# curioloop/rafting

Measured on AMD Instinct MI355X. Metric: raft-group decisions/sec (AppendEntries+vote), higher is better.
Workload: dtype int64

## Files before the change

### include/raftgpu.h

```cpp
#ifndef RAFTGPU_H
#define RAFTGPU_H

#include <stdint.h>
#include <stddef.h>

#ifdef __cplusplus
extern "C" {
#endif

#define RG_ABI_VERSION      6
#define RG_MIN_CLUSTER      2
#define RG_MAX_CLUSTER      15
#define RG_MAX_COMPACT_CLUSTER 7
#define RG_TERM_RUNS        4
#define RG_NO_NODE          (-1)

enum { RG_FOLLOWER = 0, RG_CANDIDATE = 1, RG_LEADER = 2 };

enum {
    RG_EV_NONE          = 0,
    RG_EV_AE_REQ        = 1,
    RG_EV_AE_ACK        = 2,
    RG_EV_IS_ACK        = 3,
    RG_EV_RV_REQ        = 4,
// ... 123 lines not shown
    uint32_t *elected_epoch;
    int64_t  *elected_term;
    int64_t  *commit_index;
    int64_t  *epoch_index;
    int64_t  *epoch_term;
    int64_t  *first_index;
    int64_t  *last_index;
    uint32_t *run_count;
    uint32_t *run_offset;
    int64_t  *run_start;
    int64_t  *run_term;
    int64_t  *peer_last_epoch;
    int64_t  *peer_next_index;
    int64_t  *peer_match_index;
    int32_t  *peer_rejection;
    uint8_t  *peer_pending;
} rg_group_state_t;

typedef struct rg_table rg_table_t;

int         rg_abi_version(void);
int         rg_table_create(int device, uint32_t groups, uint32_t cluster, uint32_t self_slot,
                            int pre_vote, rg_table_t **out);
int         rg_table_destroy(rg_table_t *t);
const char *rg_last_error(const rg_table_t *t);
enum { RG_OPT_REQUIRE_FENCED_TIMEOUTS = 1,
       RG_OPT_AUTO_INDEX_BASE = 2,
       RG_OPT_COMPACT_ANY_CLUSTER = 3,
       RG_OPT_DEVICE_IN_FLIGHT = 4 };
int         rg_table_option(rg_table_t *t, int option, int value);
uint32_t    rg_table_groups(const rg_table_t *t);
uint32_t    rg_table_cluster(const rg_table_t *t);

int rg_load_state(rg_table_t *t, uint32_t first, uint32_t count, const rg_group_state_t *src);
int rg_read_state(rg_table_t *t, uint32_t first, uint32_t count, rg_group_state_t *dst);

int rg_submit(rg_table_t *t, const rg_batch_t *in, const rg_outcome_t *out, int memspace);
int rg_sync(rg_table_t *t);

#define RG_PIPELINE_DEPTH 2
int rg_submit_async(rg_table_t *t, const rg_batch_t *in, const rg_outcome_t *out);
int rg_submit_wait(rg_table_t *t);

typedef struct { int32_t a, b, c, d; } rg_ev_quad32_t;
typedef struct {
    uint32_t              rounds, count;
    const uint32_t       *gid;
    const rg_ev_head_t   *head;
    const rg_ev_quad32_t *abcd;
    const int32_t        *entry_terms;
    uint64_t              entry_count;
} rg_batch32_t;
typedef struct {
    rg_reply_t   *reply;
    rg_logfx_t   *logfx;
    rg_persist_t *persist;
    uint32_t     *counts;
    uint32_t      logfx_cap, persist_cap;
} rg_outcome_packed_t;
int rg_submit_async_packed(rg_table_t *t, const rg_batch32_t *in, const rg_outcome_packed_t *out);

typedef struct rg_tick rg_tick_t;
int rg_tick_create(rg_table_t *t, const rg_batch32_t *in, const rg_outcome_packed_t *out, rg_tick_t **tick);
int rg_tick_launch(rg_tick_t *tick);
int rg_tick_wait(rg_tick_t *tick);
int rg_tick_destroy(rg_tick_t *tick);

int rg_submit32(rg_table_t *t, const rg_batch32_t *in, const rg_outcome_t *out, int memspace);
int64_t rg_batch32_pack(const rg_batch_t *in, rg_ev_head_t *head, rg_ev_quad32_t *abcd, int32_t *entry_terms);

int rg_index_base_set(rg_table_t *t, uint32_t first, uint32_t count, const int64_t *base);
int rg_index_base_get(rg_table_t *t, uint32_t first, uint32_t count, int64_t *base);
int rg_index_base_advance(const rg_batch_t *in, int32_t window, uint32_t groups, int64_t *index_base);
int rg_index_base_advance32(const rg_batch32_t *in, int32_t window, uint32_t groups, int64_t *index_base);
int64_t rg_batch32_pack_rel(const rg_batch_t *in, const int64_t *index_base, rg_ev_head_t *head, rg_ev_quad32_t *abcd, int32_t *entry_terms);
typedef struct { int32_t resp_term; uint32_t flags; int32_t commit_index; int32_t log_from; } rg_out32_t;
typedef struct { int32_t term; int32_t voted_for; uint32_t role_epoch; int32_t role; } rg_persist32_t;
typedef struct {
    rg_out32_t     *row;
    rg_persist32_t *persist;
    rg_outcome_t    wide;
} rg_outcome32_t;
int rg_submit32c(rg_table_t *t, const rg_batch32_t *in, const rg_outcome32_t *out, int memspace);
int rg_submit32c_sparse(rg_table_t *t, const rg_batch32_t *in, const rg_outcome32_t *out, int memspace);
int rg_submit32c_sparse_rounds(rg_table_t *t, const rg_batch32_t *in, const rg_outcome32_t *out, int memspace);
int rg_outcome32_unpack(const rg_outcome32_t *in, uint32_t rounds, uint32_t count, uint32_t *role_epoch, const rg_outcome_t *out);
int rg_outcome32_unpack_rel(const rg_outcome32_t *in, uint32_t rounds, uint32_t count, uint32_t *role_epoch, const int64_t *index_base, const rg_outcome_t *out);
const char *rg_step_kernel(rg_table_t *t, uint32_t count);

enum {
    RG_SEND_NONE      = 0,
    RG_SEND_APPEND    = 1,
    RG_SEND_SNAPSHOT  = 2,
    RG_SEND_GATED     = 3,
    RG_SEND_NEED_HOST = 4
};
#define RG_REPLICATE_LIMIT 50
#define RG_IN_FLIGHT_LIMIT 20

typedef struct {
    int64_t  term;
    int64_t  leader_commit;
    int64_t  epoch_index;
    int64_t  epoch_term;
    uint32_t role_epoch;
    uint32_t is_leader;
    uint64_t reserved;
} rg_send_head_t;

#define RG_SENT_TRIGGERED  1u
#define RG_SENT_HEARTBEAT  2u

typedef struct {
    int64_t  prev_index;
    int64_t  prev_term;
    int64_t  last_index;
    uint32_t count;
    uint32_t kind;
} rg_send_t;

int rg_replicate(rg_table_t *t, uint32_t count, const uint32_t *gid, const uint8_t *heartbeat, const uint16_t *in_flight,
                 rg_send_head_t *head, rg_send_t *send, int memspace);

int rg_timers_configure(rg_table_t *t, int64_t election_ms, int64_t heartbeat_ms, uint64_t seed);
int rg_timers_update(rg_table_t *t, uint32_t rounds, uint32_t count, const uint32_t *gid, const rg_reply_t *reply,
                     const int64_t *now, int memspace);
int rg_timers_expired(rg_table_t *t, int64_t now, uint32_t *out_gid, uint32_t capacity, uint32_t *out_count, int memspace);
int rg_timers_expired_epochs(rg_table_t *t, int64_t now, uint32_t *out_gid, uint32_t *out_epoch, uint32_t capacity, uint32_t *out_count,
                             int memspace);
int rg_timers_update32(rg_table_t *t, uint32_t rounds, const rg_out32_t *row, const rg_persist32_t *persist32, const int64_t *now, int memspace);
int rg_timers_arm(rg_table_t *t, int64_t now);
int rg_timers_read(rg_table_t *t, uint32_t first, uint32_t count, int64_t *deadline);

int rg_health_update(rg_table_t *t, uint32_t rounds, uint32_t count, const uint32_t *gid, const rg_ev_head_t *head,
                     const rg_reply_t *reply, const int64_t *now, int memspace);
int rg_health_update32(rg_table_t *t, uint32_t rounds, const rg_ev_head_t *head, const rg_out32_t *row, const int64_t *now, int memspace);
#define RG_HEALTH_NO_REQUEST 4u
int rg_health_failure(rg_table_t *t, uint32_t n, const uint32_t *gid, const uint8_t *slot, const uint8_t *flags, int64_t now);
int rg_ready(rg_table_t *t, int64_t now, int32_t critical_point, int64_t cool_down_ms, uint8_t *ready, int memspace);
int rg_health_read(rg_table_t *t, uint32_t first, uint32_t count, int64_t *request_success, int64_t *request_failure,
                   int32_t *recent_failure);
int rg_in_flight_read(rg_table_t *t, uint32_t first, uint32_t count, uint16_t *in_flight);
int rg_in_flight_set(rg_table_t *t, uint32_t first, uint32_t count, const uint16_t *in_flight);

typedef struct {
    uint32_t              rounds;
    const rg_ev_head_t   *head;
    const rg_ev_quad32_t *abcd;
    const int32_t        *entry_terms;
    uint64_t              entry_capacity;
    const int64_t        *now;
    const uint8_t        *heartbeat;
    const uint16_t       *in_flight;
    int32_t               critical_point;
    int64_t               cool_down_ms;
    rg_out32_t           *row;
    rg_persist32_t       *persist32;
    uint32_t             *expired_gid;
    uint32_t             *expired_epoch;
    uint32_t             *expired_count;
    uint32_t              expired_capacity;
    rg_send_head_t       *send_head;
    rg_send_t            *send;
    uint8_t              *ready;
} rg_tick2_io_t;
typedef struct rg_tick2 rg_tick2_t;
// ... 65 lines not shown
```

### rafting_amd/csrc/raftgpu.cpp

```cpp
#include <hip/hip_runtime.h>

#include <algorithm>
#include <cstdarg>
#include <cstdint>
#include <cstdio>
#include <cstdlib>
#include <cstring>
#include <string>
#include <unordered_map>
#include <vector>

#include "rg_device.hpp"
#include "rg_assemble.hpp"

using rg::DevTable;
using rg::I64x2;

struct Staging {
    void *ptr = nullptr;
    size_t cap = 0;
};

struct PipeSlot {
    Staging gid, head, ab, cd, hint, terms, reply, logfx, persist;
    Staging abcd32, terms32, counts;
    hipEvent_t up = nullptr, done = nullptr, down = nullptr;
};

struct rg_table {
    int device = 0;
    uint32_t G = 0, P = 0, self = 0, F = 0;
    int pre_vote = 0;
    hipStream_t stream = nullptr;
    DevTable dt{};
    unsigned long long *counters = nullptr;
    unsigned long long *wide_bodies = nullptr;
    size_t counter_slots = 0;
    int fast_paths = 1;
    int force_wide = 0;
    int require_fence = 0;
    int has_bases = 0;
    int auto_window = 0;
    int compact_any_cluster = 0;
    Staging st_abcd32, st_terms32, st_out32, st_persist32;
    int lanes = -1;
    uint32_t simds = 1024;
    Staging st_gid, st_head, st_ab, st_cd, st_hint, st_terms, st_reply, st_logfx, st_persist, st_hb, st_fl, st_sh, st_ss;
    bool timing = false;
    std::vector<std::pair<hipEvent_t, hipEvent_t>> ev_pool;
    size_t ev_used = 0;
    uint64_t t_launches = 0;
    double t_total_ms = 0.0;
    hipEvent_t region0 = nullptr, region1 = nullptr;
    int64_t *timer_deadline = nullptr;
    uint32_t *timer_epoch = nullptr;
    unsigned long long *tick_masks = nullptr;
    uint32_t *tick_ticket = nullptr;
    uint64_t config_gen = 0;
    std::vector<struct rg_tick *> ticks;
    std::vector<struct rg_tick2 *> ticks2;
    std::vector<struct rg_assembler *> assemblers;
    uint32_t *timer_counts = nullptr;
    int64_t election_ms = 900, heartbeat_ms = 300;
    uint64_t timer_seed = 0;
    Staging st_tgid, st_hgid, st_hslot, st_hflag, st_ready;
    int64_t *health_ok = nullptr, *health_fail = nullptr;
    int32_t *health_recent = nullptr;
    uint16_t *in_flight = nullptr;
    Staging st_hdone;
    hipStream_t s_in = nullptr, s_out = nullptr;
    PipeSlot pipe[RG_PIPELINE_DEPTH];
    uint64_t pipe_head = 0, pipe_tail = 0;
    std::string err;
};

static thread_local std::string g_create_err;

static int fail(rg_table *t, int code, const char *fmt, ...)
{
    char buf[512];
    va_list ap;
    va_start(ap, fmt);
    vsnprintf(buf, sizeof buf, fmt, ap);
    va_end(ap);
    if (t) t->err = buf; else g_create_err = buf;
    return code;
}

#define HIP_TRY(t, expr)                                                                              \
    do {                                                                                              \
        hipError_t e_ = (expr);                                                                       \
        if (e_ != hipSuccess) return fail((t), -2, "%s failed: %s", #expr, hipGetErrorString(e_));    \
    } while (0)

static int wait_oldest(rg_table *t)
{
    if (t->pipe_tail == t->pipe_head) return 1;
    HIP_TRY(t, hipEventSynchronize(t->pipe[t->pipe_tail % RG_PIPELINE_DEPTH].down));
    t->pipe_tail += 1;
    return 0;
}

static int bind(rg_table *t, bool drain = true)
{
    HIP_TRY(t, hipSetDevice(t->device));
    while (drain && t->pipe_tail != t->pipe_head)
        if (int rc = wait_oldest(t); rc < 0) return rc;
    return 0;
}

static int reserve(rg_table *t, Staging &s, size_t bytes)
{
    if (bytes <= s.cap) return 0;
    if (s.ptr) HIP_TRY(t, hipFree(s.ptr));
    s.ptr = nullptr; s.cap = 0;
    size_t cap = bytes + bytes / 4 + 4096;
    HIP_TRY(t, hipMalloc(&s.ptr, cap));
    s.cap = cap;
    return 0;
}

static int drain_timing(rg_table *t)
{
    if (t->ev_used == 0) return 0;
    HIP_TRY(t, hipStreamSynchronize(t->stream));
    for (size_t i = 0; i < t->ev_used; i++) {
        float ms = 0.f;
        HIP_TRY(t, hipEventElapsedTime(&ms, t->ev_pool[i].first, t->ev_pool[i].second));
        t->t_total_ms += ms;
        t->t_launches += 1;
    }
    t->ev_used = 0;
    return 0;
}

extern "C" {

int rg_abi_version(void) { return RG_ABI_VERSION; }

const char *rg_last_error(const rg_table_t *t) { return t ? t->err.c_str() : g_create_err.c_str(); }
uint32_t rg_table_groups(const rg_table_t *t) { return t ? t->G : 0; }
uint32_t rg_table_cluster(const rg_table_t *t) { return t ? t->P : 0; }

int rg_table_option(rg_table_t *t, int option, int value)
{
    if (!t) return -1;
    switch (option) {
    case RG_OPT_REQUIRE_FENCED_TIMEOUTS:
        if (t->require_fence != (value != 0)) t->config_gen += 1;
        t->require_fence = value != 0;
        return 0;
    case RG_OPT_AUTO_INDEX_BASE:
        if (value < 0 || value >= (1 << 30)) return fail(t, -1, "rg_table_option: RG_OPT_AUTO_INDEX_BASE window %d outside [0, 2^30)", value);
        if (t->auto_window != value) t->config_gen += 1;
        if (value != 0 && !t->has_bases) t->has_bases = 1;
        t->auto_window = value;
        return 0;
    case RG_OPT_COMPACT_ANY_CLUSTER:
        if (value != 0 && value != 1) return fail(t, -1, "rg_table_option: RG_OPT_COMPACT_ANY_CLUSTER takes 0 or 1 (%d given)", value);
        if (t->compact_any_cluster != value) t->config_gen += 1;
        t->compact_any_cluster = value;
        return 0;
    case RG_OPT_DEVICE_IN_FLIGHT: {
        if (value != 0 && value != 1) return fail(t, -1, "rg_table_option: RG_OPT_DEVICE_IN_FLIGHT takes 0 or 1 (%d given)", value);
        if ((t->in_flight != nullptr) == (value == 1)) return 0;
        if (bind(t)) return -2;
        HIP_TRY(t, hipStreamSynchronize(t->stream));
        if (value == 1) {
            const size_t bytes = (size_t)t->G * t->F * sizeof(uint16_t);
            uint16_t *c = nullptr;
            HIP_TRY(t, hipMalloc((void **)&c, bytes));
            if (hipError_t e = hipMemsetAsync(c, 0, bytes, t->stream); e != hipSuccess || (e = hipStreamSynchronize(t->stream)) != hipSuccess) {
                (void)hipFree(c);
                return fail(t, -2, "rg_table_option: RG_OPT_DEVICE_IN_FLIGHT: %s", hipGetErrorString(e));
            }
            t->in_flight = c;
        } else {
            HIP_TRY(t, hipFree(t->in_flight));
            t->in_flight = nullptr;
        }
        t->config_gen += 1;
        return 0;
    }
    default: return fail(t, -1, "rg_table_option: unknown option %d", option);
    }
}

static void tick_release(struct rg_tick *k);
static void tick2_release(struct rg_tick2 *k);
static void assembler_release(struct rg_assembler *a);

int rg_table_destroy(rg_table_t *t)
{
    if (!t) return 0;
    (void)hipSetDevice(t->device);
    if (t->stream) (void)hipStreamSynchronize(t->stream);
    for (struct rg_tick *k : t->ticks) tick_release(k);
    for (struct rg_tick2 *k : t->ticks2) tick2_release(k);
    for (struct rg_assembler *a : t->assemblers) assembler_release(a);
    t->ticks.clear(); t->ticks2.clear(); t->assemblers.clear();
    void *cols[] = {t->dt.term_commit, t->dt.epoch, t->dt.window, t->dt.ident, t->dt.elect, t->dt.runs,
                    t->dt.peer_en, t->dt.peer_m, t->dt.ibase, t->wide_bodies, t->counters, t->st_gid.ptr, t->st_head.ptr, t->st_ab.ptr,
                    t->st_cd.ptr, t->st_hint.ptr, t->st_terms.ptr, t->st_reply.ptr, t->st_logfx.ptr,
                    t->st_persist.ptr, t->st_hb.ptr, t->st_fl.ptr, t->st_sh.ptr, t->st_ss.ptr, t->timer_deadline, t->timer_epoch, t->tick_masks, t->tick_ticket,
                    t->timer_counts, t->st_tgid.ptr, t->st_hgid.ptr, t->st_hslot.ptr, t->st_hflag.ptr, t->st_ready.ptr, t->health_ok,
                    t->health_fail, t->health_recent, t->in_flight, t->st_hdone.ptr, t->st_abcd32.ptr, t->st_terms32.ptr, t->st_out32.ptr, t->st_persist32.ptr};
    for (void *c : cols) if (c) (void)hipFree(c);
    for (PipeSlot &sl : t->pipe) {
        if (sl.down) (void)hipEventSynchronize(sl.down);
        for (Staging *st : {&sl.gid, &sl.head, &sl.ab, &sl.cd, &sl.hint, &sl.terms, &sl.reply, &sl.logfx, &sl.persist, &sl.abcd32, &sl.terms32, &sl.counts})
            if (st->ptr) (void)hipFree(st->ptr);
        for (hipEvent_t ev : {sl.up, sl.done, sl.down}) if (ev) (void)hipEventDestroy(ev);
    }
    if (t->s_in) (void)hipStreamDestroy(t->s_in);
    if (t->s_out) (void)hipStreamDestroy(t->s_out);
    for (auto &e : t->ev_pool) { (void)hipEventDestroy(e.first); (void)hipEventDestroy(e.second); }
    if (t->region0) { (void)hipEventDestroy(t->region0); (void)hipEventDestroy(t->region1); }
    if (t->stream) (void)hipStreamDestroy(t->stream);
    delete t;
    return 0;
}

int rg_table_create(int device, uint32_t groups, uint32_t cluster, uint32_t self_slot, int pre_vote, rg_table_t **out)
{
    if (!out) return fail(nullptr, -1, "rg_table_create: out is NULL");
    *out = nullptr;
    if (groups == 0) return fail(nullptr, -1, "rg_table_create: groups must be > 0");
    if (cluster < RG_MIN_CLUSTER || cluster > RG_MAX_CLUSTER)
        return fail(nullptr, -1, "rg_table_create: cluster size %u outside [%d, %d]", cluster, RG_MIN_CLUSTER, RG_MAX_CLUSTER);
    if (self_slot >= cluster) return fail(nullptr, -1, "rg_table_create: self_slot %u >= cluster %u", self_slot, cluster);
    int ndev = 0;
    hipError_t e = hipGetDeviceCount(&ndev);
    if (e != hipSuccess || ndev == 0)
        return fail(nullptr, -2, "rg_table_create: no HIP device (%s) — libraftgpu has no CPU path", hipGetErrorString(e));
    if (device < 0 || device >= ndev) return fail(nullptr, -1, "rg_table_create: device %d of %d", device, ndev);

    rg_table *t = new rg_table();
    t->device = device; t->G = groups; t->P = cluster; t->self = self_slot; t->F = cluster - 1;
    t->pre_vote = pre_vote != 0;
#define CREATE_TRY(expr)                                                                   \
    do {                                                                                   \
        hipError_t e2_ = (expr);                                                           \
        if (e2_ != hipSuccess) {                                                           \
            fail(nullptr, -2, "%s failed: %s", #expr, hipGetErrorString(e2_));             \
            rg_table_destroy(t);                                                           \
            return -2;                                                                     \
        }                                                                                  \
    } while (0)
    CREATE_TRY(hipSetDevice(device));
    CREATE_TRY(hipStreamCreateWithFlags(&t->stream, hipStreamNonBlocking));
    const size_t G = groups, F = t->F;
    CREATE_TRY(hipMalloc((void **)&t->dt.term_commit, G * sizeof(I64x2)));
    CREATE_TRY(hipMalloc((void **)&t->dt.epoch, G * sizeof(I64x2)));
    CREATE_TRY(hipMalloc((void **)&t->dt.window, G * sizeof(I64x2)));
    CREATE_TRY(hipMalloc((void **)&t->dt.ident, G * sizeof(rg::Ident)));
    CREATE_TRY(hipMalloc((void **)&t->dt.elect, G * sizeof(rg::Elect)));
    CREATE_TRY(hipMalloc((void **)&t->dt.runs, G * rg::K * sizeof(I64x2)));
    CREATE_TRY(hipMalloc((void **)&t->dt.peer_en, G * F * sizeof(I64x2)));
    CREATE_TRY(hipMalloc((void **)&t->dt.peer_m, G * F * sizeof(rg::Match)));
    CREATE_TRY(hipMalloc((void **)&t->dt.ibase, G * sizeof(int64_t)));
    CREATE_TRY(hipMalloc((void **)&t->wide_bodies, sizeof(unsigned long long)));
    CREATE_TRY(hipMemsetAsync(t->wide_bodies, 0, sizeof(unsigned long long), t->stream));
    {
        hipDeviceProp_t prop;
        CREATE_TRY(hipGetDeviceProperties(&prop, device));
        t->simds = (uint32_t)prop.multiProcessorCount * 4u;
    }
    t->lanes = -1;
    if (const char *e = getenv("RG_SPLIT")) t->lanes = atoi(e) != 0 ? 0 : 64;
    if (const char *e = getenv("RG_FAST")) t->fast_paths = atoi(e) != 0;
    if (const char *e = getenv("RG_FORCE_WIDE")) t->force_wide = atoi(e) != 0;
    t->counter_slots = (G + 63) / 64 + 1;
    CREATE_TRY(hipMalloc((void **)&t->counters, t->counter_slots * RG_NUM_COUNTERS * sizeof(unsigned long long)));
    t->dt.groups = groups;
    CREATE_TRY(hipMalloc((void **)&t->timer_deadline, G * sizeof(int64_t)));
    CREATE_TRY(hipMalloc((void **)&t->timer_counts, ((G + 255) / 256 * 4 + 1) * sizeof(uint32_t)));
    CREATE_TRY(hipMemsetAsync(t->timer_deadline, 0, G * sizeof(int64_t), t->stream));
    CREATE_TRY(hipMalloc((void **)&t->tick_masks, ((G + 255) / 256 * 4) * sizeof(unsigned long long)));
    CREATE_TRY(hipMemsetAsync(t->tick_masks, 0, ((G + 255) / 256 * 4) * sizeof(unsigned long long), t->stream));
    CREATE_TRY(hipMalloc((void **)&t->tick_ticket, sizeof(uint32_t)));
    CREATE_TRY(hipMemsetAsync(t->tick_ticket, 0, sizeof(uint32_t), t->stream));
    CREATE_TRY(hipMalloc((void **)&t->timer_epoch, G * sizeof(uint32_t)));
    CREATE_TRY(hipMemsetAsync(t->timer_epoch, 0, G * sizeof(uint32_t), t->stream));
    CREATE_TRY(hipMalloc((void **)&t->health_ok, G * F * sizeof(int64_t)));
    CREATE_TRY(hipMalloc((void **)&t->health_fail, G * F * sizeof(int64_t)));
    CREATE_TRY(hipMalloc((void **)&t->health_recent, G * F * sizeof(int32_t)));
    CREATE_TRY(hipMemsetAsync(t->health_ok, 0, G * F * sizeof(int64_t), t->stream));
    CREATE_TRY(hipMemsetAsync(t->health_fail, 0, G * F * sizeof(int64_t), t->stream));
    CREATE_TRY(hipMemsetAsync(t->health_recent, 0, G * F * sizeof(int32_t), t->stream));
    CREATE_TRY(hipMemsetAsync(t->dt.term_commit, 0, G * sizeof(I64x2), t->stream));
    CREATE_TRY(hipMemsetAsync(t->dt.epoch, 0, G * sizeof(I64x2), t->stream));
    CREATE_TRY(hipMemsetAsync(t->dt.window, 0, G * sizeof(I64x2), t->stream));
    CREATE_TRY(hipMemsetAsync(t->dt.runs, 0, G * rg::K * sizeof(I64x2), t->stream));
    CREATE_TRY(hipMemsetAsync(t->dt.peer_en, 0, G * F * sizeof(I64x2), t->stream));
    CREATE_TRY(hipMemsetAsync(t->dt.peer_m, 0, G * F * sizeof(rg::Match), t->stream));
    CREATE_TRY(hipMemsetAsync(t->dt.ibase, 0, G * sizeof(int64_t), t->stream));
    CREATE_TRY(hipMemsetAsync(t->counters, 0, t->counter_slots * RG_NUM_COUNTERS * sizeof(unsigned long long), t->stream));
    {
        std::vector<rg::Ident> id(G, rg::Ident{RG_NO_NODE, RG_NO_NODE, 1u, 0u});
        std::vector<rg::Elect> el(G, rg::Elect{0, 0u, 1});
        CREATE_TRY(hipMemcpyAsync(t->dt.ident, id.data(), G * sizeof(rg::Ident), hipMemcpyHostToDevice, t->stream));
        CREATE_TRY(hipMemcpyAsync(t->dt.elect, el.data(), G * sizeof(rg::Elect), hipMemcpyHostToDevice, t->stream));
        CREATE_TRY(hipStreamSynchronize(t->stream));
    }
#undef CREATE_TRY
    *out = t;
    return 0;
}


static int step_lanes(const rg_table *t, uint32_t count)
{
    if (t->lanes >= 0) return t->lanes;
    const uint32_t wavefronts = (count + 63u) / 64u;
    return wavefronts <= t->simds ? 0 : 64;
}

static bool state_complete(const rg_group_state_t *s)
{
    return s->current_term && s->voted_for && s->role && s->current_leader && s->timeout_detected && s->repl_prepared &&
           s->role_epoch && s->votes && s->elected_epoch && s->elected_term && s->commit_index && s->epoch_index &&
           s->epoch_term && s->first_index && s->last_index && s->run_count && s->run_offset && s->run_start && s->run_term &&
           s->peer_last_epoch && s->peer_next_index && s->peer_match_index && s->peer_rejection && s->peer_pending;
}

int rg_load_state(rg_table_t *t, uint32_t first, uint32_t count, const rg_group_state_t *s)
{
    if (!t) return -1;
    if (!s || !state_complete(s)) return fail(t, -1, "rg_load_state: src or one of its columns is NULL");
    if ((uint64_t)first + count > t->G) return fail(t, -1, "rg_load_state: range [%u, %u) exceeds %u groups", first, first + count, t->G);
    if (count == 0) return 0;
    if (bind(t)) return -2;
    const size_t n = count, F = t->F, G = t->G;
    std::vector<I64x2> tc(n), ep(n), win(n), runs(n * rg::K), en(n * F);
    std::vector<rg::Ident> id(n);
    std::vector<rg::Elect> el(n);
    std::vector<rg::Match> pm(n * F);
    for (size_t i = 0; i < n; i++) {
        const int32_t role = s->role[i];
        if (role < RG_FOLLOWER || role > RG_LEADER) return fail(t, -1, "rg_load_state: group %zu role %d", first + i, role);
        if (s->voted_for[i] < RG_NO_NODE || s->voted_for[i] >= (int32_t)t->P || s->current_leader[i] < RG_NO_NODE ||
            s->current_leader[i] >= (int32_t)t->P)
            return fail(t, -1, "rg_load_state: group %zu node slot out of range", first + i);
        const uint32_t total = s->run_count[i], off = s->run_offset[i];
        const uint32_t rc = total > (uint32_t)rg::K ? (uint32_t)rg::K : total;
        int64_t fi = 0, la = 0;
        if (total) {
            fi = s->first_index[i]; la = s->last_index[i];
            if (s->run_start[off] != fi || la < s->run_start[off + total - 1])
                return fail(t, -1, "rg_load_state: group %zu runs do not span [first,last]", first + i);
            if (fi != s->epoch_index[i] && fi != s->epoch_index[i] + 1)
                return fail(t, -1, "rg_load_state: group %zu first index %lld is neither epoch.index nor epoch.index+1",
                            first + i, (long long)fi);
            for (uint32_t k = 1; k < total; k++)
// ... 247 lines not shown
    rg_batch_t wide{};
    wide.rounds = in->rounds; wide.count = in->count; wide.gid = in->gid; wide.head = in->head;
    wide.ab = wide.cd = reinterpret_cast<const rg_ev_pair_t *>(in->abcd);
    wide.entry_terms = reinterpret_cast<const int64_t *>(in->entry_terms); wide.entry_count = in->entry_count;
    rg_logfx_t dummy_l; rg_persist_t dummy_p;
    const rg_outcome_t shape{out->reply, &dummy_l, &dummy_p};
    if (int rc = check_batch(t, &wide, &shape, true)) return rc;
    if (in->count == 0) { out->counts[0] = out->counts[1] = 0; return 0; }
    const size_t rows64 = (size_t)in->rounds * in->count;
    if (rows64 >= (1ull << 31)) return fail(t, -1, "rg_submit_async_packed: %zu rows in one batch (limit 2^31 - 1)", rows64);
    if (bind(t, false)) return -2;
    void *d_logfx = nullptr, *d_persist = nullptr, *d_counts = nullptr;
    if (hipHostGetDevicePointer(&d_counts, out->counts, 0) != hipSuccess ||
        (out->logfx_cap && hipHostGetDevicePointer(&d_logfx, out->logfx, 0) != hipSuccess) ||
        (out->persist_cap && hipHostGetDevicePointer(&d_persist, out->persist, 0) != hipSuccess)) {
        (void)hipGetLastError();
        return fail(t, -1, "rg_submit_async_packed: counts / logfx / persist must be page-locked memory from rg_host_alloc");
    }
    if (int rc = pipeline_ready(t)) return rc;
    PipeSlot &sl = t->pipe[t->pipe_head % RG_PIPELINE_DEPTH];
    const bool sparse = in->gid != nullptr;
    const uint32_t rows = (uint32_t)rows64, waves = (rows + 63u) / 64u;
    rg::StepParams p = step_params(t, &wide);
    if (reserve(t, sl.head, rows64 * sizeof(rg_ev_head_t)) || reserve(t, sl.abcd32, rows64 * sizeof(rg_ev_quad32_t)) ||
        reserve(t, sl.reply, rows64 * sizeof(rg_reply_t)) || reserve(t, sl.logfx, rows64 * sizeof(I64x2)) ||
        reserve(t, sl.persist, rows64 * sizeof(rg_persist_t)) || reserve(t, sl.counts, (size_t)2 * waves * sizeof(uint32_t)))
        return -2;
    hipStream_t si = t->s_in, so = t->s_out;
    HIP_TRY(t, hipMemcpyAsync(sl.head.ptr, in->head, rows64 * sizeof(rg_ev_head_t), hipMemcpyHostToDevice, si));
    HIP_TRY(t, hipMemcpyAsync(sl.abcd32.ptr, in->abcd, rows64 * sizeof(rg_ev_quad32_t), hipMemcpyHostToDevice, si));
    if (sparse) {
        if (reserve(t, sl.gid, in->count * sizeof(uint32_t))) return -2;
        HIP_TRY(t, hipMemcpyAsync(sl.gid.ptr, in->gid, in->count * sizeof(uint32_t), hipMemcpyHostToDevice, si));
        p.gid = (const uint32_t *)sl.gid.ptr;
    }
    if (in->entry_count) {
        if (reserve(t, sl.terms32, in->entry_count * sizeof(int32_t))) return -2;
        HIP_TRY(t, hipMemcpyAsync(sl.terms32.ptr, in->entry_terms, in->entry_count * sizeof(int32_t), hipMemcpyHostToDevice, si));
    }
    HIP_TRY(t, hipEventRecord(sl.up, si));
    HIP_TRY(t, hipStreamWaitEvent(t->stream, sl.up, 0));
    p.head = (const rg_ev_head_t *)sl.head.ptr; p.abcd32 = (const rg::I32x4 *)sl.abcd32.ptr;
    p.hint = nullptr;
    p.entry_terms32 = in->entry_count ? (const int32_t *)sl.terms32.ptr : nullptr;
    p.reply = (rg_reply_t *)sl.reply.ptr; p.logfx = (I64x2 *)sl.logfx.ptr; p.persist = (rg_persist_t *)sl.persist.ptr;
    if (int rc = launch(t, p, sparse)) return rc;
    HIP_TRY(t, rg::launch_outcome_count(p.reply, rows, (uint32_t *)sl.counts.ptr, (uint32_t *)d_counts, t->stream));
    HIP_TRY(t, hipEventRecord(sl.done, t->stream));
    HIP_TRY(t, hipStreamWaitEvent(so, sl.done, 0));
    HIP_TRY(t, rg::launch_outcome_emit(p.reply, p.logfx, p.persist, rows, (const uint32_t *)sl.counts.ptr, (I64x2 *)d_logfx, out->logfx_cap,
                                       (rg_persist_t *)d_persist, out->persist_cap, so));
    HIP_TRY(t, hipMemcpyAsync(out->reply, sl.reply.ptr, rows64 * sizeof(rg_reply_t), hipMemcpyDeviceToHost, so));
    HIP_TRY(t, hipEventRecord(sl.down, so));
    t->pipe_head += 1;
    return 0;
}

struct rg_tick {
    rg_table *t = nullptr;
    hipGraph_t graph = nullptr;
    hipGraphExec_t exec = nullptr;
    Staging head, abcd, gid, terms, reply, logfx, persist, counts;
    uint64_t config_gen = 0;
    bool in_flight = false;
};

static void tick_release(struct rg_tick *k)
{
    if (k->exec) (void)hipGraphExecDestroy(k->exec);
    if (k->graph) (void)hipGraphDestroy(k->graph);
    k->exec = nullptr; k->graph = nullptr;
    for (Staging *st : {&k->head, &k->abcd, &k->gid, &k->terms, &k->reply, &k->logfx, &k->persist, &k->counts}) {
        if (st->ptr) (void)hipFree(st->ptr);
        st->ptr = nullptr; st->cap = 0;
    }
    k->t = nullptr;
}

int rg_tick_destroy(rg_tick_t *k)
{
    if (!k) return 0;
    if (rg_table *t = k->t) {
        (void)hipSetDevice(t->device);
        if (t->stream) (void)hipStreamSynchronize(t->stream);
        t->ticks.erase(std::remove(t->ticks.begin(), t->ticks.end(), k), t->ticks.end());
        tick_release(k);
    }
    delete k;
    return 0;
}

static bool page_locked(const void *p)
{
    void *d = nullptr;
    if (hipHostGetDevicePointer(&d, const_cast<void *>(p), 0) == hipSuccess) return true;
    (void)hipGetLastError();
    return false;
}

int rg_tick_create(rg_table_t *t, const rg_batch32_t *in, const rg_outcome_packed_t *out, rg_tick_t **tick)
{
    if (!t) return -1;
    if (int rc = compact_ok(t, "rg_tick_create")) return rc;
    if (!tick) return fail(t, -1, "rg_tick_create: tick is NULL");
    *tick = nullptr;
    if (!in || !out) return fail(t, -1, "rg_tick_create: null batch or outcome");
    if (!in->head || !in->abcd || !out->reply || !out->counts || (out->logfx_cap && !out->logfx) || (out->persist_cap && !out->persist))
        return fail(t, -1, "rg_tick_create: head, abcd, reply, counts and every list with a capacity are required");
    if (in->entry_count && !in->entry_terms) return fail(t, -1, "rg_tick_create: entry_count %llu without entry_terms", (unsigned long long)in->entry_count);
    rg_batch_t wide{};
    wide.rounds = in->rounds; wide.count = in->count; wide.gid = nullptr; wide.head = in->head;
    wide.ab = wide.cd = reinterpret_cast<const rg_ev_pair_t *>(in->abcd);
    wide.entry_terms = reinterpret_cast<const int64_t *>(in->entry_terms); wide.entry_count = in->entry_count;
    rg_logfx_t dummy_l; rg_persist_t dummy_p;
    const rg_outcome_t shape{out->reply, &dummy_l, &dummy_p};
    if (in->gid) {
        if (in->rounds != 1) return fail(t, -1, "rg_tick_create: sparse batches carry exactly one round");
        if (in->count > t->G || in->count == 0) return fail(t, -1, "rg_tick_create: %u rows for %u groups", in->count, t->G);
    } else if (int rc = check_batch(t, &wide, &shape, true)) return rc;
    if (in->rounds == 0 || in->count == 0) return fail(t, -1, "rg_tick_create: an empty shape");
    const size_t rows64 = (size_t)in->rounds * in->count;
    if (rows64 >= (1ull << 31)) return fail(t, -1, "rg_tick_create: %zu rows in one batch (limit 2^31 - 1)", rows64);
    if (bind(t)) return -2;
    void *d_logfx = nullptr, *d_persist = nullptr, *d_counts = nullptr;
    if (hipHostGetDevicePointer(&d_counts, out->counts, 0) != hipSuccess ||
        (out->logfx_cap && hipHostGetDevicePointer(&d_logfx, out->logfx, 0) != hipSuccess) ||
        (out->persist_cap && hipHostGetDevicePointer(&d_persist, out->persist, 0) != hipSuccess)) {
        (void)hipGetLastError();
        return fail(t, -1, "rg_tick_create: counts / logfx / persist must be page-locked memory from rg_host_alloc");
    }
    if (!page_locked(in->head) || !page_locked(in->abcd) || !page_locked(out->reply) || (in->gid && !page_locked(in->gid)) ||
        (in->entry_count && !page_locked(in->entry_terms)))
        return fail(t, -1, "rg_tick_create: head / abcd / gid / entry_terms / reply must be page-locked memory from rg_host_alloc (the recorded copies replay from them)");
    rg_tick *k = new rg_tick();
    k->t = t;
    k->config_gen = t->config_gen;
    const uint32_t rows = (uint32_t)rows64, waves = (rows + 63u) / 64u;
    const bool sparse = in->gid != nullptr;
    if (reserve(t, k->head, rows64 * sizeof(rg_ev_head_t)) || reserve(t, k->abcd, rows64 * sizeof(rg_ev_quad32_t)) || reserve(t, k->reply, rows64 * sizeof(rg_reply_t)) ||
        reserve(t, k->logfx, rows64 * sizeof(I64x2)) || reserve(t, k->persist, rows64 * sizeof(rg_persist_t)) || reserve(t, k->counts, (size_t)2 * waves * sizeof(uint32_t)) ||
        (sparse && reserve(t, k->gid, in->count * sizeof(uint32_t))) || (in->entry_count && reserve(t, k->terms, in->entry_count * sizeof(int32_t)))) {
        rg_tick_destroy(k);
        return -2;
    }
    rg::StepParams p = step_params(t, &wide);
    p.head = (const rg_ev_head_t *)k->head.ptr; p.abcd32 = (const rg::I32x4 *)k->abcd.ptr;
    p.gid = sparse ? (const uint32_t *)k->gid.ptr : nullptr;
    p.entry_terms32 = in->entry_count ? (const int32_t *)k->terms.ptr : nullptr;
    p.reply = (rg_reply_t *)k->reply.ptr; p.logfx = (I64x2 *)k->logfx.ptr; p.persist = (rg_persist_t *)k->persist.ptr;
    hipStream_t s = t->stream;
    hipError_t e = hipStreamBeginCapture(s, hipStreamCaptureModeThreadLocal);
    if (e == hipSuccess) e = hipMemcpyAsync(k->head.ptr, in->head, rows64 * sizeof(rg_ev_head_t), hipMemcpyHostToDevice, s);
    if (e == hipSuccess) e = hipMemcpyAsync(k->abcd.ptr, in->abcd, rows64 * sizeof(rg_ev_quad32_t), hipMemcpyHostToDevice, s);
    if (e == hipSuccess && sparse) e = hipMemcpyAsync(k->gid.ptr, in->gid, in->count * sizeof(uint32_t), hipMemcpyHostToDevice, s);
    if (e == hipSuccess && in->entry_count) e = hipMemcpyAsync(k->terms.ptr, in->entry_terms, in->entry_count * sizeof(int32_t), hipMemcpyHostToDevice, s);
    if (e == hipSuccess) e = rg::launch_step(p, (int)t->F, sparse, 32, s);
    if (e == hipSuccess) e = rg::launch_outcome_count(p.reply, rows, (uint32_t *)k->counts.ptr, (uint32_t *)d_counts, s);
    if (e == hipSuccess) e = rg::launch_outcome_emit(p.reply, p.logfx, p.persist, rows, (const uint32_t *)k->counts.ptr, (I64x2 *)d_logfx, out->logfx_cap,
                                                     (rg_persist_t *)d_persist, out->persist_cap, s);
    if (e == hipSuccess) e = hipMemcpyAsync(out->reply, k->reply.ptr, rows64 * sizeof(rg_reply_t), hipMemcpyDeviceToHost, s);
    hipGraph_t g = nullptr;
    const hipError_t e2 = hipStreamEndCapture(s, &g);
    k->graph = g;
    if (e == hipSuccess) e = e2;
    if (e == hipSuccess) e = hipGraphInstantiate(&k->exec, k->graph, nullptr, nullptr, 0);
    if (e != hipSuccess) {
        (void)hipGetLastError();
        rg_tick_destroy(k);
        return fail(t, -2, "rg_tick_create: %s", hipGetErrorString(e));
    }
    t->ticks.push_back(k);
    *tick = k;
    return 0;
}

int rg_tick_launch(rg_tick_t *k)
{
    if (!k || !k->t) return -1;
    rg_table *t = k->t;
    if (k->config_gen != t->config_gen)
        return fail(t, -1, "rg_tick_launch: the table's options or index bases changed after rg_tick_create (they are part of the recording): create the tick again");
    if (bind(t)) return -2;
    if (k->in_flight) { HIP_TRY(t, hipStreamSynchronize(t->stream)); k->in_flight = false; }
    HIP_TRY(t, hipGraphLaunch(k->exec, t->stream));
    k->in_flight = true;
    return 0;
}

int rg_tick_wait(rg_tick_t *k)
{
    if (!k || !k->t) return -1;
    rg_table *t = k->t;
    HIP_TRY(t, hipSetDevice(t->device));
    HIP_TRY(t, hipStreamSynchronize(t->stream));
    k->in_flight = false;
    return 0;
}

static rg::TimerParams timer_params(rg_table *t);
static rg::HealthParams health_params(rg_table *t);

struct rg_tick2 {
    rg_table *t = nullptr;
    hipGraph_t graph = nullptr;
    hipGraphExec_t exec = nullptr;
    uint64_t config_gen = 0;
    bool in_flight = false;
};

static void tick2_release(struct rg_tick2 *k)
{
    if (k->exec) (void)hipGraphExecDestroy(k->exec);
    if (k->graph) (void)hipGraphDestroy(k->graph);
    k->exec = nullptr; k->graph = nullptr;
    k->t = nullptr;
}

int rg_tick2_destroy(rg_tick2_t *k)
{
    if (!k) return 0;
    if (rg_table *t = k->t) {
        (void)hipSetDevice(t->device);
        if (t->stream) (void)hipStreamSynchronize(t->stream);
        t->ticks2.erase(std::remove(t->ticks2.begin(), t->ticks2.end(), k), t->ticks2.end());
        tick2_release(k);
    }
    delete k;
    return 0;
}

static int device_visible(rg_table *t, const char *who, const void *p, const char *what, void **out)
{
    *out = nullptr;
    if (!p) return 0;
    hipPointerAttribute_t a{};
    if (hipPointerGetAttributes(&a, p) != hipSuccess || a.type == hipMemoryTypeUnregistered) {
        (void)hipGetLastError();
        return fail(t, -1, "%s: %s is neither device memory (rg_dev_alloc) nor page-locked host memory (rg_host_alloc)", who, what);
    }
    if (a.type == hipMemoryTypeHost) {
        if (hipHostGetDevicePointer(out, const_cast<void *>(p), 0) != hipSuccess) {
            (void)hipGetLastError();
            return fail(t, -1, "%s: %s is host memory the device cannot address", who, what);
        }
        return 0;
    }
    *out = const_cast<void *>(p);
    return 0;
}

static int tick2_create(rg_table_t *t, const rg_tick2_io_t *io, const rg_tick2_rows_t *rows, rg_tick2_t **tick, const char *who, bool deep = false,
                        const uint32_t *depth_now = nullptr)
{
    if (!t) return -1;
    if (int rc = compact_ok(t, who)) return rc;
    if (!tick) return fail(t, -1, "%s: tick is NULL", who);
    *tick = nullptr;
    if (!io) return fail(t, -1, "%s: io is NULL", who);
    if (io->rounds == 0 || io->rounds > 64) return fail(t, -1, "%s: %u rounds (1 .. 64: one clock per round travels with the tick)", who, io->rounds);
    if (!io->head || !io->abcd || !io->now || !io->row || !io->persist32) return fail(t, -1, "%s: head, abcd, now, row and persist32 are required", who);
    if (io->entry_capacity && !io->entry_terms) return fail(t, -1, "%s: entry_capacity %llu without entry_terms", who, (unsigned long long)io->entry_capacity);
    if (io->expired_gid && (!io->expired_count || io->expired_capacity == 0)) return fail(t, -1, "%s: the expiry step needs expired_count and a capacity", who);
    if ((io->send_head == nullptr) != (io->send == nullptr)) return fail(t, -1, "%s: send_head and send come together", who);
    if (t->in_flight && (io->heartbeat || io->in_flight))
        return fail(t, -1, "%s: the table has RG_OPT_DEVICE_IN_FLIGHT: the send step derives heartbeat and in_flight from the tick's own rows, both columns must be NULL", who);
    if (rows) {
        if (io->rounds != 1 && !deep) return fail(t, -1, "%s: %u rounds (a list of groups carries exactly one round)", who, io->rounds);
        if (!rows->gid || !rows->count) return fail(t, -1, "%s: gid and count are required", who);
        if (rows->capacity == 0 || rows->capacity > t->G) return fail(t, -1, "%s: a capacity of %u rows for %u groups (1 .. groups)", who, rows->capacity, t->G);
    }
    const uint32_t R = rows ? rows->capacity : t->G;
    rg_batch_t wide{};
    wide.rounds = io->rounds; wide.count = R; wide.gid = rows ? rows->gid : nullptr; wide.head = io->head;
    wide.ab = wide.cd = reinterpret_cast<const rg_ev_pair_t *>(io->abcd);
    wide.entry_terms = reinterpret_cast<const int64_t *>(io->entry_terms); wide.entry_count = io->entry_capacity;
    rg_reply_t dummy_r; rg_logfx_t dummy_l; rg_persist_t dummy_p;
    const rg_outcome_t shape{&dummy_r, &dummy_l, &dummy_p};
    if (int rc = check_batch(t, &wide, &shape, false, deep)) return rc;
    if (bind(t)) return -2;
    const auto visible = [t](const void *p, const char *what, void **out) { return device_visible(t, "rg_tick2_create", p, what, out); };
    void *d_head, *d_abcd, *d_terms, *d_now, *d_hb, *d_fl, *d_row, *d_per, *d_egid, *d_eep, *d_ecnt, *d_sh, *d_ss, *d_ready, *d_gid = nullptr, *d_cnt = nullptr, *d_depth = nullptr;
    if ((rows && (visible(rows->gid, "gid", &d_gid) || visible(rows->count, "count", &d_cnt) || visible(depth_now, "rounds", &d_depth))) ||
        visible(io->head, "head", &d_head) || visible(io->abcd, "abcd", &d_abcd) || visible(io->entry_terms, "entry_terms", &d_terms) ||
        visible(io->now, "now", &d_now) || visible(io->heartbeat, "heartbeat", &d_hb) || visible(io->in_flight, "in_flight", &d_fl) ||
        visible(io->row, "row", &d_row) || visible(io->persist32, "persist32", &d_per) || visible(io->expired_gid, "expired_gid", &d_egid) ||
        visible(io->expired_epoch, "expired_epoch", &d_eep) || visible(io->expired_count, "expired_count", &d_ecnt) ||
        visible(io->send_head, "send_head", &d_sh) || visible(io->send, "send", &d_ss) || visible(io->ready, "ready", &d_ready))
        return -1;
    rg_tick2 *k = new rg_tick2();
    k->t = t;
    k->config_gen = t->config_gen;
    rg::StepParams sp = step_params(t, &wide);
    sp.gid = (const uint32_t *)d_gid;
    sp.head = (const rg_ev_head_t *)d_head; sp.abcd32 = (const rg::I32x4 *)d_abcd;
    sp.entry_terms32 = io->entry_capacity ? (const int32_t *)d_terms : nullptr;
    sp.out32 = (rg::I32x4 *)d_row; sp.persist32 = (rg::I32x4 *)d_per;
    rg::TimerParams tp = timer_params(t);
    tp.rounds = io->rounds; tp.count = R; tp.out32 = (const rg::I32x4 *)d_row; tp.persist32 = (const rg::I32x4 *)d_per; tp.now_mem = (const int64_t *)d_now;
    rg::HealthParams hp = health_params(t);
    hp.rounds = io->rounds; hp.count = R; hp.head = (const rg_ev_head_t *)d_head; hp.out32 = (const rg::I32x4 *)d_row; hp.now_mem = (const int64_t *)d_now;
    const int64_t *now_last = (const int64_t *)d_now + (io->rounds - 1);
    rg::HealthParams rp = health_params(t);
    rp.now_mem = now_last;
    rg::ReplicateParams qp{};
    qp.t = t->dt; qp.count = R; qp.gid = (const uint32_t *)d_gid; qp.heartbeat = (const uint8_t *)d_hb; qp.in_flight = (const uint16_t *)d_fl; qp.head = (rg_send_head_t *)d_sh; qp.send = (rg_send_t *)d_ss;
    if (t->in_flight) {
        qp.counts = t->in_flight; qp.ev_head = (const rg_ev_head_t *)d_head; qp.ev_out32 = (const rg::I32x4 *)d_row; qp.ev_stride = R; qp.self = t->self;
    }
    hipStream_t s = t->stream;
    rg::TickFoldParams fp{};
    fp.tp = tp; fp.hp = hp; fp.now_last = now_last;
    fp.masks = (unsigned long long *)t->tick_masks; fp.ticket = t->tick_ticket;
    fp.out_gid = (uint32_t *)d_egid; fp.out_epoch = (uint32_t *)d_eep; fp.out_count = (uint32_t *)d_ecnt; fp.capacity = io->expired_capacity;
    fp.expire = io->expired_gid != nullptr;
    fp.rounds_now = (const uint32_t *)d_depth;
    rg::TickTailParams tt{};
    tt.fp = fp; tt.qp = qp; tt.rp = rp; tt.critical_point = io->critical_point; tt.cool_down = io->cool_down_ms; tt.ready = (uint8_t *)d_ready;
    const char *nodes_env = getenv("RG_TICK_NODES");
    int nodes = (nodes_env && (nodes_env[0] == '2' || nodes_env[0] == '4')) ? nodes_env[0] - '0' : (sp.force_wide != 0 ? 2 : 1);
    if (nodes == 4 && t->in_flight) nodes = 2;
    hipError_t e = hipStreamBeginCapture(s, hipStreamCaptureModeThreadLocal);
    if (rows) {
        if (e == hipSuccess) e = rg::launch_tick_sparse(sp, tt, (const uint32_t *)d_cnt, (int)t->F, s);
        if (e == hipSuccess && fp.expire) e = rg::launch_tick_expire(fp, s);
    } else if (nodes == 1) {
        if (e == hipSuccess) e = rg::launch_tick(sp, tt, (int)t->F, s);
    } else {
        if (e == hipSuccess) e = rg::launch_step(sp, (int)t->F, false, 32, s);
        if (nodes == 2) {
            if (e == hipSuccess) e = rg::launch_tick_tail(tt, (int)t->F, s);
        } else {
            if (e == hipSuccess) e = rg::launch_tick_fold(fp, s);
            if (e == hipSuccess && io->send_head) e = rg::launch_replicate(qp, (int)t->F, s);
            if (e == hipSuccess && io->ready) e = rg::launch_ready(rp, 0, io->critical_point, io->cool_down_ms, (uint8_t *)d_ready, s);
        }
    }
    hipGraph_t g = nullptr;
    const hipError_t e2 = hipStreamEndCapture(s, &g);
    k->graph = g;
    if (e == hipSuccess) e = e2;
    if (e == hipSuccess) e = hipGraphInstantiate(&k->exec, k->graph, nullptr, nullptr, 0);
    if (e != hipSuccess) {
        (void)hipGetLastError();
        rg_tick2_destroy(k);
        return fail(t, -2, "%s: %s", who, hipGetErrorString(e));
    }
    t->ticks2.push_back(k);
    *tick = k;
    return 0;
}

int rg_tick2_create(rg_table_t *t, const rg_tick2_io_t *io, rg_tick2_t **tick)
{
    return tick2_create(t, io, nullptr, tick, "rg_tick2_create");
}

int rg_tick2_create_sparse(rg_table_t *t, const rg_tick2_io_t *io, const rg_tick2_rows_t *rows, rg_tick2_t **tick)
{
    if (t && !rows) return fail(t, -1, "rg_tick2_create_sparse: rows is NULL");
    return tick2_create(t, io, rows, tick, "rg_tick2_create_sparse");
}

int rg_tick2_create_sparse_rounds(rg_table_t *t, const rg_tick2_io_t *io, const rg_tick2_rounds_t *rows, rg_tick2_t **tick)
{
    if (t && !rows) return fail(t, -1, "rg_tick2_create_sparse_rounds: rows is NULL");
    if (!t) return -1;
    const rg_tick2_rows_t list{rows->gid, rows->count, rows->capacity};
    return tick2_create(t, io, &list, tick, "rg_tick2_create_sparse_rounds", true, rows->rounds);
}

int rg_tick2_launch(rg_tick2_t *k)
{
    if (!k || !k->t) return -1;
    rg_table *t = k->t;
    if (k->config_gen != t->config_gen)
        return fail(t, -1, "rg_tick2_launch: the table's options or index bases changed after rg_tick2_create (they are part of the recording): create the tick again");
    if (bind(t)) return -2;
    HIP_TRY(t, hipGraphLaunch(k->exec, t->stream));
    k->in_flight = true;
    return 0;
}

int rg_tick2_wait(rg_tick2_t *k)
{
    if (!k || !k->t) return -1;
    rg_table *t = k->t;
    HIP_TRY(t, hipSetDevice(t->device));
    HIP_TRY(t, hipStreamSynchronize(t->stream));
    k->in_flight = false;
    return 0;
}

struct rg_assembler {
    rg_table *t = nullptr;
    uint32_t max_events = 0, max_expired = 0;
    rg::AsmParams sc{};
    Staging in_words, in_gid, in_head, in_abcd, ex_gid, ex_epoch;
    Staging out_gid, out_words, out_head, out_abcd, out_origin, out_deferred;
};

static void assembler_release(struct rg_assembler *a)
{
    void *cols[] = {a->sc.cnt, a->sc.bitmap, a->sc.rowof, a->sc.wordoff, a->sc.rowcnt, a->sc.segoff, a->sc.seg, a->sc.flag, a->sc.dcounts, a->sc.big, a->sc.scalars,
                    a->in_words.ptr, a->in_gid.ptr, a->in_head.ptr, a->in_abcd.ptr, a->ex_gid.ptr, a->ex_epoch.ptr,
                    a->out_gid.ptr, a->out_words.ptr, a->out_head.ptr, a->out_abcd.ptr, a->out_origin.ptr, a->out_deferred.ptr};
    for (void *c : cols) if (c) (void)hipFree(c);
    *a = rg_assembler{};
}

int rg_assembler_destroy(rg_assembler_t *a)
{
    if (!a) return 0;
    if (rg_table *t = a->t) {
        (void)hipSetDevice(t->device);
        if (t->stream) (void)hipStreamSynchronize(t->stream);
        t->assemblers.erase(std::remove(t->assemblers.begin(), t->assemblers.end(), a), t->assemblers.end());
        assembler_release(a);
    }
    delete a;
    return 0;
}

int rg_assembler_create(rg_table_t *t, uint32_t max_events, uint32_t max_expired, rg_assembler_t **out)
{
    if (!t) return -1;
    if (!out) return fail(t, -1, "rg_assembler_create: a is NULL");
    *out = nullptr;
    if ((uint64_t)max_events + max_expired >= (1ull << 31))
        return fail(t, -1, "rg_assembler_create: %u + %u events: a run holds fewer than 2^31 (the ids of the expired source carry bit 31)", max_events, max_expired);
    if (bind(t)) return -2;
    rg_assembler *a = new rg_assembler();
    a->t = t; a->max_events = max_events; a->max_expired = max_expired;
    rg::AsmParams &p = a->sc;
    const size_t G = t->G, words = (G + 63) / 64, events = (size_t)max_events + max_expired, eb = events ? (events + 255) / 256 : 1;
    p.groups = t->G; p.words = (uint32_t)words;
    p.seg_cap = (uint32_t)events;
    p.rows_cap = (uint32_t)(G < events ? G : events);
    p.big_cap = (uint32_t)(events / (rg::ASM_SMALL + 1) + 1);
    struct { void **ptr; size_t bytes; bool zero; } cols[] = {
        {(void **)&p.cnt, G * sizeof(uint32_t), true}, {(void **)&p.bitmap, words * sizeof(unsigned long long), true}, {(void **)&p.rowof, G * sizeof(uint32_t), true},
        {(void **)&p.wordoff, (words + 1) * sizeof(uint32_t), false}, {(void **)&p.rowcnt, ((size_t)p.rows_cap + 1) * sizeof(uint32_t), false},
        {(void **)&p.segoff, ((size_t)p.rows_cap + 1) * sizeof(uint32_t), false}, {(void **)&p.seg, (events + 1) * sizeof(uint32_t), false},
        {(void **)&p.flag, events + 1, false}, {(void **)&p.dcounts, (eb * 4 + 1) * sizeof(uint32_t), false}, {(void **)&p.big, (size_t)p.big_cap * sizeof(uint32_t), false},
        {(void **)&p.scalars, rg::ASM_SCALARS * sizeof(uint32_t), true}};
    for (auto &c : cols) {
        hipError_t e = hipMalloc(c.ptr, c.bytes);
        if (e == hipSuccess && c.zero) e = hipMemsetAsync(*c.ptr, 0, c.bytes, t->stream);
        if (e != hipSuccess) {
            assembler_release(a);
            delete a;
            return fail(t, -2, "rg_assembler_create: %zu bytes of scratch: %s", c.bytes, hipGetErrorString(e));
        }
    }
    if (hipStreamSynchronize(t->stream) != hipSuccess) { assembler_release(a); delete a; return fail(t, -2, "rg_assembler_create: hipStreamSynchronize failed"); }
    t->assemblers.push_back(a);
    *out = a;
    return 0;
}

int rg_assemble32(rg_assembler_t *a, const rg_arrivals_t *in, const rg_assembled_t *out, int memspace)
{
    if (!a || !a->t) return -1;
    rg_table *t = a->t;
    const char *who = "rg_assemble32";
    if (!in || !out) return fail(t, -1, "%s: NULL arrivals or batch", who);
    if (!in->count || (in->capacity && (!in->gid || !in->head || !in->abcd))) return fail(t, -1, "%s: count, gid, head and abcd of the arrival log are required", who);
    if (!out->gid || !out->count || !out->rounds || !out->head || !out->abcd || !out->origin || !out->stats || (out->deferred_capacity && !out->deferred))
        return fail(t, -1, "%s: gid, count, rounds, head, abcd, origin and stats of the batch are required (and deferred, unless deferred_capacity is 0)", who);
    if (out->capacity == 0 || out->capacity > t->G) return fail(t, -1, "%s: capacity %u outside 1 .. %u groups", who, out->capacity, t->G);
    if (out->max_rounds < 1 || out->max_rounds > 64) return fail(t, -1, "%s: max_rounds %u outside 1 .. 64", who, out->max_rounds);
    if (in->capacity > a->max_events) return fail(t, -1, "%s: an arrival log of %u events, the assembler was created for %u", who, in->capacity, a->max_events);
    const int sources = (in->expired_gid != nullptr) + (in->expired_epoch != nullptr) + (in->expired_count != nullptr);
    if (sources != 0 && sources != 3) return fail(t, -1, "%s: the expired source comes as all three columns or none", who);
    const bool expired = sources == 3;
    if (expired && in->expired_capacity > a->max_expired)
        return fail(t, -1, "%s: an expired source of %u entries, the assembler was created for %u", who, in->expired_capacity, a->max_expired);
    if (memspace != RG_MEM_DEVICE && memspace != RG_MEM_HOST) return fail(t, -1, "%s: unknown memspace %d", who, memspace);
    const uint32_t C = out->capacity, D = out->max_rounds, ex_cap = expired ? in->expired_capacity : 0u;
    const size_t cells = (size_t)C * D;
    rg::AsmParams p = a->sc;
    p.in_cap = in->capacity; p.ex_cap = ex_cap; p.C = C; p.D = D; p.deferred_cap = out->deferred_capacity;
    if (memspace == RG_MEM_DEVICE) {
        void *v[16] = {};
        const struct { const void *ptr; const char *what; } cols[] = {
            {in->count, "count"}, {in->gid, "gid"}, {in->head, "head"}, {in->abcd, "abcd"}, {in->expired_gid, "expired_gid"}, {in->expired_epoch, "expired_epoch"},
            {in->expired_count, "expired_count"}, {out->gid, "the batch's gid"}, {out->count, "the batch's count"}, {out->rounds, "rounds"}, {out->head, "the batch's head"},
            {out->abcd, "the batch's abcd"}, {out->origin, "origin"}, {out->deferred, "deferred"}, {out->stats, "stats"}};
        int k = 0;
        for (const auto &c : cols) if (int rc = device_visible(t, "rg_assemble32", c.ptr, c.what, &v[k++])) return rc;
        p.in_count = (const uint32_t *)v[0]; p.in_gid = (const uint32_t *)v[1]; p.in_head = (const rg::U32x2 *)v[2]; p.in_abcd = (const rg::I32x4 *)v[3];
        p.ex_gid = (const uint32_t *)v[4]; p.ex_epoch = (const uint32_t *)v[5]; p.ex_count = (const uint32_t *)v[6];
        p.gid = (uint32_t *)v[7]; p.count = (uint32_t *)v[8]; p.rounds = (uint32_t *)v[9]; p.head = (rg::U32x2 *)v[10]; p.abcd = (rg::I32x4 *)v[11];
        p.origin = (uint32_t *)v[12]; p.deferred = (uint32_t *)v[13]; p.stats = (uint32_t *)v[14];
        if (bind(t)) return -2;
        HIP_TRY(t, rg::launch_assemble(p, t->stream));
        return 0;
    }
// ... 100 lines not shown
    }
    p.reply = (rg_reply_t *)t->st_reply.ptr; p.logfx = (I64x2 *)t->st_logfx.ptr; p.persist = (rg_persist_t *)t->st_persist.ptr;
    HIP_TRY(t, hipMemsetAsync(t->st_logfx.ptr, 0, rows * sizeof(I64x2), s));
    HIP_TRY(t, hipMemsetAsync(t->st_persist.ptr, 0, rows * sizeof(rg_persist_t), s));
    if (int rc = launch(t, p, sparse)) return rc;
    HIP_TRY(t, hipMemcpyAsync(out->reply, t->st_reply.ptr, rows * sizeof(rg_reply_t), hipMemcpyDeviceToHost, s));
    HIP_TRY(t, hipMemcpyAsync(out->logfx, t->st_logfx.ptr, rows * sizeof(I64x2), hipMemcpyDeviceToHost, s));
    HIP_TRY(t, hipMemcpyAsync(out->persist, t->st_persist.ptr, rows * sizeof(rg_persist_t), hipMemcpyDeviceToHost, s));
    HIP_TRY(t, hipStreamSynchronize(s));
    return 0;
}

int rg_submit32(rg_table_t *t, const rg_batch32_t *in, const rg_outcome_t *out, int memspace)
{
    if (!t) return -1;
    if (int rc = compact_ok(t, "rg_submit32")) return rc;
    if (!in || !out) return fail(t, -1, "rg_submit32: NULL batch or outcome");
    if (!in->head || !in->abcd) return fail(t, -1, "rg_submit32: head and abcd are required");
    rg_batch_t wide{};
    wide.rounds = in->rounds; wide.count = in->count; wide.gid = in->gid; wide.head = in->head;
    wide.ab = wide.cd = reinterpret_cast<const rg_ev_pair_t *>(in->abcd);
    wide.entry_terms = reinterpret_cast<const int64_t *>(in->entry_terms); wide.entry_count = in->entry_count;
    if (int rc = check_batch(t, &wide, out, memspace == RG_MEM_HOST)) return rc;
    if (in->count == 0) return 0;
    if (bind(t)) return -2;
    const bool sparse = in->gid != nullptr;
    const size_t rows = (size_t)in->rounds * in->count;
    rg::StepParams p = step_params(t, &wide);
    if (memspace == RG_MEM_DEVICE) {
        p.gid = in->gid; p.head = in->head; p.abcd32 = (const rg::I32x4 *)in->abcd;
        p.entry_terms32 = in->entry_count ? in->entry_terms : nullptr;
        p.reply = out->reply; p.logfx = (I64x2 *)out->logfx; p.persist = out->persist;
        return launch(t, p, sparse);
    }
    if (memspace != RG_MEM_HOST) return fail(t, -1, "rg_submit32: unknown memspace %d", memspace);
    hipStream_t s = t->stream;
    if (reserve(t, t->st_head, rows * sizeof(rg_ev_head_t)) || reserve(t, t->st_abcd32, rows * sizeof(rg_ev_quad32_t)) ||
        reserve(t, t->st_reply, rows * sizeof(rg_reply_t)) || reserve(t, t->st_logfx, rows * sizeof(I64x2)) ||
        reserve(t, t->st_persist, rows * sizeof(rg_persist_t)))
        return -2;
    HIP_TRY(t, hipMemcpyAsync(t->st_head.ptr, in->head, rows * sizeof(rg_ev_head_t), hipMemcpyHostToDevice, s));
    HIP_TRY(t, hipMemcpyAsync(t->st_abcd32.ptr, in->abcd, rows * sizeof(rg_ev_quad32_t), hipMemcpyHostToDevice, s));
    p.head = (const rg_ev_head_t *)t->st_head.ptr; p.abcd32 = (const rg::I32x4 *)t->st_abcd32.ptr;
    if (sparse) {
        if (reserve(t, t->st_gid, in->count * sizeof(uint32_t))) return -2;
        HIP_TRY(t, hipMemcpyAsync(t->st_gid.ptr, in->gid, in->count * sizeof(uint32_t), hipMemcpyHostToDevice, s));
        p.gid = (const uint32_t *)t->st_gid.ptr;
    }
    if (in->entry_count) {
        if (reserve(t, t->st_terms32, in->entry_count * sizeof(int32_t))) return -2;
        HIP_TRY(t, hipMemcpyAsync(t->st_terms32.ptr, in->entry_terms, in->entry_count * sizeof(int32_t), hipMemcpyHostToDevice, s));
        p.entry_terms32 = (const int32_t *)t->st_terms32.ptr;
    }
    p.reply = (rg_reply_t *)t->st_reply.ptr; p.logfx = (I64x2 *)t->st_logfx.ptr; p.persist = (rg_persist_t *)t->st_persist.ptr;
    HIP_TRY(t, hipMemsetAsync(t->st_logfx.ptr, 0, rows * sizeof(I64x2), s));
    HIP_TRY(t, hipMemsetAsync(t->st_persist.ptr, 0, rows * sizeof(rg_persist_t), s));
    if (int rc = launch(t, p, sparse)) return rc;
    HIP_TRY(t, hipMemcpyAsync(out->reply, t->st_reply.ptr, rows * sizeof(rg_reply_t), hipMemcpyDeviceToHost, s));
    HIP_TRY(t, hipMemcpyAsync(out->logfx, t->st_logfx.ptr, rows * sizeof(I64x2), hipMemcpyDeviceToHost, s));
    HIP_TRY(t, hipMemcpyAsync(out->persist, t->st_persist.ptr, rows * sizeof(rg_persist_t), hipMemcpyDeviceToHost, s));
    HIP_TRY(t, hipStreamSynchronize(s));
    return 0;
}

int rg_wide_body_workgroups(rg_table_t *t, uint64_t *count, int reset)
{
    if (!t || !count) return -1;
    if (bind(t)) return -2;
    unsigned long long v = 0;
    HIP_TRY(t, hipMemcpyAsync(&v, t->wide_bodies, sizeof v, hipMemcpyDeviceToHost, t->stream));
    if (reset) HIP_TRY(t, hipMemsetAsync(t->wide_bodies, 0, sizeof v, t->stream));
    HIP_TRY(t, hipStreamSynchronize(t->stream));
    *count = v;
    return 0;
}

int rg_index_base_set(rg_table_t *t, uint32_t first, uint32_t count, const int64_t *base)
{
    if (!t) return -1;
    if (!base) return fail(t, -1, "rg_index_base_set: NULL base");
    if ((uint64_t)first + count > t->G) return fail(t, -1, "rg_index_base_set: groups [%u, %u) of %u", first, first + count, t->G);
    for (uint32_t i = 0; i < count; i++)
        if (base[i] < 0) return fail(t, -1, "rg_index_base_set: base[%u] = %lld is negative", i, (long long)base[i]);
    for (uint32_t i = 0; i < count; i++)
        if (base[i] != 0 && !t->has_bases) { t->has_bases = 1; t->config_gen += 1; }
    if (count == 0) return 0;
    if (bind(t)) return -2;
    HIP_TRY(t, hipMemcpyAsync(t->dt.ibase + first, base, (size_t)count * sizeof(int64_t), hipMemcpyHostToDevice, t->stream));
    HIP_TRY(t, hipStreamSynchronize(t->stream));
    return 0;
}

int rg_index_base_get(rg_table_t *t, uint32_t first, uint32_t count, int64_t *base)
{
    if (!t) return -1;
    if (!base) return fail(t, -1, "rg_index_base_get: NULL base");
    if ((uint64_t)first + count > t->G) return fail(t, -1, "rg_index_base_get: groups [%u, %u) of %u", first, first + count, t->G);
    if (count == 0) return 0;
    if (bind(t)) return -2;
    HIP_TRY(t, hipMemcpyAsync(base, t->dt.ibase + first, (size_t)count * sizeof(int64_t), hipMemcpyDeviceToHost, t->stream));
    HIP_TRY(t, hipStreamSynchronize(t->stream));
    return 0;
}

extern "C++" template <class Flush>
int advance_bases(uint32_t rounds, uint32_t count, const uint32_t *gid, const rg_ev_head_t *head, int32_t window, uint32_t groups, int64_t *index_base,
                         Flush flush)
{
    if (!head || !index_base || window < 1 || window >= (1 << 30)) return -1;
    if (gid ? count > groups : count != groups) return -2;
    if (gid)
        for (uint32_t i = 0; i < count; i++)
            if (gid[i] >= groups) return -2;
    std::vector<int64_t> top(gid ? count : groups, 0);
    for (uint32_t r = 0; r < rounds; r++)
        for (uint32_t i = 0; i < count; i++) {
            const size_t row = (size_t)r * count + i;
            if (RG_HDR_KIND(head[row].hdr) != RG_EV_LOG_FLUSH) continue;
            const int64_t a = flush(row, gid ? gid[i] : i);
            if (a > top[i]) top[i] = a;
        }
    for (uint32_t i = 0; i < (uint32_t)top.size(); i++) {
        int64_t &base = index_base[gid ? gid[i] : i];
        if (top[i] - window > base) base = top[i] - window;
    }
    return 0;
}

int rg_index_base_advance(const rg_batch_t *in, int32_t window, uint32_t groups, int64_t *index_base)
{
    if (!in || !in->ab) return -1;
    return advance_bases(in->rounds, in->count, in->gid, in->head, window, groups, index_base, [&](size_t row, uint32_t) { return (int64_t)in->ab[row].x; });
}

int rg_index_base_advance32(const rg_batch32_t *in, int32_t window, uint32_t groups, int64_t *index_base)
{
    if (!in || !in->abcd) return -1;
    return advance_bases(in->rounds, in->count, in->gid, in->head, window, groups, index_base, [&](size_t row, uint32_t g) {
        const int32_t a = in->abcd[row].a;
        return a <= 0 ? (int64_t)0 : (int64_t)a + index_base[g];
    });
}

static uint32_t host_index_fields(uint32_t kind)
{
    switch (kind) {
    case RG_EV_AE_REQ: return 0xAu;
    case RG_EV_AE_ACK: return 0x6u;
    case RG_EV_IS_ACK: case RG_EV_RV_REQ: case RG_EV_PV_REQ: case RG_EV_IS_REQ: return 0x2u;
    case RG_EV_LOG_FLUSH: return 0x1u;
    default: return 0u;
    }
}

static int submit32c(rg_table_t *t, const rg_batch32_t *in, const rg_outcome32_t *out, int memspace, bool sparse, const char *who, bool list_rounds = false)
{
    if (!t) return -1;
    if (int rc = compact_ok(t, who)) return rc;
    if (!in || !out) return fail(t, -1, "%s: NULL batch or outcome", who);
    if (!in->head || !in->abcd || !out->row || !out->persist) return fail(t, -1, "%s: head, abcd, row and persist are required", who);
    if (!sparse && in->gid) return fail(t, -1, "rg_submit32c: dense batches only (gid must be NULL); a list of groups goes through rg_submit32c_sparse");
    if (sparse && !in->gid) return fail(t, -1, "%s: gid is required (dense batches go through rg_submit32c)", who);
    const int wides = (out->wide.reply != nullptr) + (out->wide.logfx != nullptr) + (out->wide.persist != nullptr);
    if (wides != 0 && wides != 3) return fail(t, -1, "%s: the overflow columns come as all three or none", who);
    rg_batch_t wide{};
    wide.rounds = in->rounds; wide.count = in->count; wide.gid = in->gid; wide.head = in->head;
    wide.ab = wide.cd = reinterpret_cast<const rg_ev_pair_t *>(in->abcd);
    wide.entry_terms = reinterpret_cast<const int64_t *>(in->entry_terms); wide.entry_count = in->entry_count;
    rg_reply_t dummy_r; rg_logfx_t dummy_l; rg_persist_t dummy_p;
    const rg_outcome_t shape{&dummy_r, &dummy_l, &dummy_p};
    if (int rc = check_batch(t, &wide, &shape, memspace == RG_MEM_HOST, list_rounds)) return rc;
    if (in->count == 0) return 0;
    if (bind(t)) return -2;
    const size_t rows = (size_t)in->rounds * in->count;
    rg::StepParams p = step_params(t, &wide);
    if (memspace == RG_MEM_DEVICE) {
        p.gid = in->gid; p.head = in->head; p.abcd32 = (const rg::I32x4 *)in->abcd;
        p.entry_terms32 = in->entry_count ? in->entry_terms : nullptr;
        p.out32 = (rg::I32x4 *)out->row; p.persist32 = (rg::I32x4 *)out->persist;
        p.reply = out->wide.reply; p.logfx = (I64x2 *)out->wide.logfx; p.persist = out->wide.persist;
        return launch(t, p, sparse);
    }
    if (memspace != RG_MEM_HOST) return fail(t, -1, "%s: unknown memspace %d", who, memspace);
    hipStream_t s = t->stream;
    if (reserve(t, t->st_head, rows * sizeof(rg_ev_head_t)) || reserve(t, t->st_abcd32, rows * sizeof(rg_ev_quad32_t)) ||
        reserve(t, t->st_out32, rows * sizeof(rg_out32_t)) || reserve(t, t->st_persist32, rows * sizeof(rg_persist32_t)))
        return -2;
    if (wides && (reserve(t, t->st_reply, rows * sizeof(rg_reply_t)) || reserve(t, t->st_logfx, rows * sizeof(I64x2)) ||
                  reserve(t, t->st_persist, rows * sizeof(rg_persist_t))))
        return -2;
    HIP_TRY(t, hipMemcpyAsync(t->st_head.ptr, in->head, rows * sizeof(rg_ev_head_t), hipMemcpyHostToDevice, s));
    HIP_TRY(t, hipMemcpyAsync(t->st_abcd32.ptr, in->abcd, rows * sizeof(rg_ev_quad32_t), hipMemcpyHostToDevice, s));
    p.head = (const rg_ev_head_t *)t->st_head.ptr; p.abcd32 = (const rg::I32x4 *)t->st_abcd32.ptr;
    if (sparse) {
        if (reserve(t, t->st_gid, in->count * sizeof(uint32_t))) return -2;
        HIP_TRY(t, hipMemcpyAsync(t->st_gid.ptr, in->gid, in->count * sizeof(uint32_t), hipMemcpyHostToDevice, s));
        p.gid = (const uint32_t *)t->st_gid.ptr;
    }
    if (in->entry_count) {
        if (reserve(t, t->st_terms32, in->entry_count * sizeof(int32_t))) return -2;
        HIP_TRY(t, hipMemcpyAsync(t->st_terms32.ptr, in->entry_terms, in->entry_count * sizeof(int32_t), hipMemcpyHostToDevice, s));
        p.entry_terms32 = (const int32_t *)t->st_terms32.ptr;
    }
    p.out32 = (rg::I32x4 *)t->st_out32.ptr; p.persist32 = (rg::I32x4 *)t->st_persist32.ptr;
    HIP_TRY(t, hipMemsetAsync(t->st_persist32.ptr, 0, rows * sizeof(rg_persist32_t), s));
    if (wides) {
        p.reply = (rg_reply_t *)t->st_reply.ptr; p.logfx = (I64x2 *)t->st_logfx.ptr; p.persist = (rg_persist_t *)t->st_persist.ptr;
        HIP_TRY(t, hipMemsetAsync(t->st_reply.ptr, 0, rows * sizeof(rg_reply_t), s));
        HIP_TRY(t, hipMemsetAsync(t->st_logfx.ptr, 0, rows * sizeof(I64x2), s));
        HIP_TRY(t, hipMemsetAsync(t->st_persist.ptr, 0, rows * sizeof(rg_persist_t), s));
    }
    if (int rc = launch(t, p, sparse)) return rc;
    HIP_TRY(t, hipMemcpyAsync(out->row, t->st_out32.ptr, rows * sizeof(rg_out32_t), hipMemcpyDeviceToHost, s));
    HIP_TRY(t, hipMemcpyAsync(out->persist, t->st_persist32.ptr, rows * sizeof(rg_persist32_t), hipMemcpyDeviceToHost, s));
    if (wides) {
        HIP_TRY(t, hipMemcpyAsync(out->wide.reply, t->st_reply.ptr, rows * sizeof(rg_reply_t), hipMemcpyDeviceToHost, s));
        HIP_TRY(t, hipMemcpyAsync(out->wide.logfx, t->st_logfx.ptr, rows * sizeof(I64x2), hipMemcpyDeviceToHost, s));
        HIP_TRY(t, hipMemcpyAsync(out->wide.persist, t->st_persist.ptr, rows * sizeof(rg_persist_t), hipMemcpyDeviceToHost, s));
    }
    HIP_TRY(t, hipStreamSynchronize(s));
    return 0;
}

int rg_submit32c(rg_table_t *t, const rg_batch32_t *in, const rg_outcome32_t *out, int memspace)
{
    return submit32c(t, in, out, memspace, false, "rg_submit32c");
}

int rg_submit32c_sparse(rg_table_t *t, const rg_batch32_t *in, const rg_outcome32_t *out, int memspace)
{
    return submit32c(t, in, out, memspace, true, "rg_submit32c_sparse");
}

int rg_submit32c_sparse_rounds(rg_table_t *t, const rg_batch32_t *in, const rg_outcome32_t *out, int memspace)
{
    return submit32c(t, in, out, memspace, true, "rg_submit32c_sparse_rounds", true);
}

int rg_outcome32_unpack(const rg_outcome32_t *in, uint32_t rounds, uint32_t count, uint32_t *role_epoch, const rg_outcome_t *out)
{
    return rg_outcome32_unpack_rel(in, rounds, count, role_epoch, nullptr, out);
}

int rg_outcome32_unpack_rel(const rg_outcome32_t *in, uint32_t rounds, uint32_t count, uint32_t *role_epoch, const int64_t *index_base, const rg_outcome_t *out)
{
    if (!in || !in->row || !in->persist || !role_epoch || !out || !out->reply || !out->logfx || !out->persist) return -1;
    auto absolute = [&](int32_t v, uint32_t i) { return v == 0 ? (int64_t)0 : (int64_t)v + (index_base ? index_base[i] : 0); };
    for (uint32_t r = 0; r < rounds; r++) {
        for (uint32_t i = 0; i < count; i++) {
            const size_t row = (size_t)r * count + i;
            const rg_out32_t c = in->row[row];
            const uint32_t flags = c.flags & ~RG_F_WIDE_VALUES;
            const bool has_lfx = (flags & (RG_F_COMMIT | RG_F_LOG_APPEND | RG_F_LOG_TRUNC)) != 0 || RG_F_STATUS(flags) == RG_NEED_HOST;
            const bool has_from = (flags & (RG_F_LOG_APPEND | RG_F_LOG_TRUNC)) != 0 || RG_F_STATUS(flags) == RG_NEED_HOST;
            const bool has_per = (flags & RG_F_PERSIST) != 0;
// ... 417 lines not shown
    if (out)
        for (size_t i = 0; i < n; i++)
            for (size_t j = 0; j < F; j++) out[i * F + j] = col[j * n + i];
    return 0;
}

int rg_in_flight_read(rg_table_t *t, uint32_t first, uint32_t count, uint16_t *in_flight)
{
    return in_flight_copy(t, first, count, in_flight, nullptr, "rg_in_flight_read");
}

int rg_in_flight_set(rg_table_t *t, uint32_t first, uint32_t count, const uint16_t *in_flight)
{
    return in_flight_copy(t, first, count, nullptr, in_flight, "rg_in_flight_set");
}

const char *rg_step_kernel(rg_table_t *t, uint32_t count)
{
    if (!t) return "";
    return step_lanes(t, count) == 0 ? "rg::step_split_kernel" : "rg::step_kernel";
}

int rg_sync(rg_table_t *t)
{
    if (!t) return -1;
    if (bind(t)) return -2;
    HIP_TRY(t, hipStreamSynchronize(t->stream));
    return 0;
}


int rg_host_alloc(rg_table_t *t, size_t bytes, void **hptr)
{
    if (!t || !hptr) return -1;
    if (bind(t)) return -2;
    HIP_TRY(t, hipHostMalloc(hptr, bytes ? bytes : 16, hipHostMallocDefault));
    return 0;
}

int rg_host_free(rg_table_t *t, void *hptr)
{
    if (!t) return -1;
    if (bind(t)) return -2;
    HIP_TRY(t, hipStreamSynchronize(t->stream));
    HIP_TRY(t, hipHostFree(hptr));
    return 0;
}

int rg_dev_alloc(rg_table_t *t, size_t bytes, void **dptr)
{
    if (!t || !dptr) return -1;
    if (bind(t)) return -2;
    HIP_TRY(t, hipMalloc(dptr, bytes ? bytes : 16));
    return 0;
}

int rg_dev_free(rg_table_t *t, void *dptr)
{
    if (!t) return -1;
    if (bind(t)) return -2;
    HIP_TRY(t, hipStreamSynchronize(t->stream));
    HIP_TRY(t, hipFree(dptr));
    return 0;
}

int rg_copy_to_device(rg_table_t *t, void *dst, const void *src, size_t bytes)
{
    if (!t) return -1;
    if (bind(t)) return -2;
    HIP_TRY(t, hipMemcpyAsync(dst, src, bytes, hipMemcpyHostToDevice, t->stream));
    HIP_TRY(t, hipStreamSynchronize(t->stream));
    return 0;
}

int rg_copy_to_host(rg_table_t *t, void *dst, const void *src, size_t bytes)
{
    if (!t) return -1;
    if (bind(t)) return -2;
    HIP_TRY(t, hipMemcpyAsync(dst, src, bytes, hipMemcpyDeviceToHost, t->stream));
    HIP_TRY(t, hipStreamSynchronize(t->stream));
    return 0;
}

void *rg_stream(rg_table_t *t) { return t ? (void *)t->stream : nullptr; }


int rg_timing_enable(rg_table_t *t, int on)
{
    if (!t) return -1;
    if (bind(t)) return -2;
    if (drain_timing(t)) return -2;
    t->timing = on != 0;
    return 0;
}

int rg_timing_read(rg_table_t *t, uint64_t *launches, double *total_ms, int reset)
{
    if (!t) return -1;
    if (bind(t)) return -2;
    if (drain_timing(t)) return -2;
    if (launches) *launches = t->t_launches;
    if (total_ms) *total_ms = t->t_total_ms;
    if (reset) { t->t_launches = 0; t->t_total_ms = 0.0; }
    return 0;
}

int rg_timing_begin(rg_table_t *t)
{
    if (!t) return -1;
    if (bind(t)) return -2;
    if (!t->region0) { HIP_TRY(t, hipEventCreate(&t->region0)); HIP_TRY(t, hipEventCreate(&t->region1)); }
    HIP_TRY(t, hipEventRecord(t->region0, t->stream));
    return 0;
}

int rg_timing_end(rg_table_t *t, double *elapsed_ms)
{
    if (!t || !elapsed_ms) return -1;
    if (bind(t)) return -2;
    if (!t->region0) return fail(t, -1, "rg_timing_end without rg_timing_begin");
    HIP_TRY(t, hipEventRecord(t->region1, t->stream));
    HIP_TRY(t, hipEventSynchronize(t->region1));
    float ms = 0.f;
    HIP_TRY(t, hipEventElapsedTime(&ms, t->region0, t->region1));
    *elapsed_ms = ms;
    return 0;
}

int rg_counters_read(rg_table_t *t, uint64_t counters[RG_NUM_COUNTERS], int reset)
{
    if (!t || !counters) return -1;
    if (bind(t)) return -2;
    const size_t n = t->counter_slots * RG_NUM_COUNTERS;
    std::vector<unsigned long long> host(n);
    HIP_TRY(t, hipMemcpyAsync(host.data(), t->counters, n * sizeof(unsigned long long), hipMemcpyDeviceToHost, t->stream));
    if (reset) HIP_TRY(t, hipMemsetAsync(t->counters, 0, n * sizeof(unsigned long long), t->stream));
    HIP_TRY(t, hipStreamSynchronize(t->stream));
#ifdef RG_PROBE_HWID
    if (const char *path = getenv("RG_DUMP_COUNTERS")) {
        if (FILE *f = fopen(path, "wb")) { fwrite(host.data(), sizeof(unsigned long long), n, f); fclose(f); }
    }
#endif
    for (int i = 0; i < RG_NUM_COUNTERS; i++) counters[i] = 0;
    for (size_t s = 0; s < t->counter_slots; s++)
        for (int i = 0; i < RG_NUM_COUNTERS; i++) counters[i] += host[s * RG_NUM_COUNTERS + i];
    return 0;
}

int rg_copy_bandwidth(rg_table_t *t, size_t bytes, int iters, double *gbps)
{
    if (!t || !gbps || iters < 1) return -1;
    if (bind(t)) return -2;
    bytes &= ~(size_t)15;
    if (bytes == 0) return fail(t, -1, "rg_copy_bandwidth: bytes must be >= 16");
    void *src = nullptr, *dst = nullptr;
    HIP_TRY(t, hipMalloc(&src, bytes));
    HIP_TRY(t, hipMalloc(&dst, bytes));
    HIP_TRY(t, hipMemsetAsync(src, 1, bytes, t->stream));
    hipEvent_t a, b;
    HIP_TRY(t, hipEventCreate(&a));
    HIP_TRY(t, hipEventCreate(&b));
    HIP_TRY(t, rg::launch_copy(src, dst, bytes, t->stream));
    HIP_TRY(t, hipEventRecord(a, t->stream));
    for (int i = 0; i < iters; i++) HIP_TRY(t, rg::launch_copy(src, dst, bytes, t->stream));
    HIP_TRY(t, hipEventRecord(b, t->stream));
    HIP_TRY(t, hipStreamSynchronize(t->stream));
    float ms = 0.f;
// ... 9 lines not shown
```

### rafting_amd/csrc/rg_device.hpp

```cpp
#pragma once

#include <hip/hip_runtime.h>
#include <stdint.h>
#include <type_traits>

#include "../../include/raftgpu.h"

namespace rg {

constexpr int K = RG_TERM_RUNS;
constexpr int BLOCK = 64;

struct alignas(16) I64x2 { int64_t x, y; };
struct alignas(16) I32x4 { int32_t x, y, z, w; };
struct alignas(8) U32x2 { uint32_t x, y; };
struct alignas(16) Ident { int32_t voted_for, leader; uint32_t role_epoch, meta; };
struct alignas(16) Elect { int64_t elected_term; uint32_t elected_epoch; int32_t votes; };
struct alignas(16) Match { int64_t match_index; int32_t rejection; int32_t pad; };

constexpr uint32_t META_ROLE = 3u, META_TD = 1u << 2, META_PREP = 1u << 3;
constexpr int META_RC_SHIFT = 4, META_PEND_SHIFT = 8;
constexpr uint32_t META_PEND_MASK = (1u << (RG_MAX_CLUSTER - 1)) - 1u;

struct DevTable {
    I64x2 *term_commit;
    I64x2 *epoch;
    I64x2 *window;
    Ident *ident;
    Elect *elect;
    I64x2 *runs;
    I64x2 *peer_en;
    Match *peer_m;
    int64_t *ibase;
    uint32_t groups;
};

struct StepParams {
    DevTable t;
    uint32_t rounds, count;
    const uint32_t *gid;
    const rg_ev_head_t *head;
    const I64x2 *ab, *cd, *hint;
    const int64_t *entry_terms;
    const I32x4 *abcd32;
    const int32_t *entry_terms32;
    uint64_t entry_count;
    rg_reply_t *reply;
    I64x2 *logfx;
    rg_persist_t *persist;
    I32x4 *out32, *persist32;
    unsigned long long *counters;
    unsigned long long *wide_bodies;
    int32_t self, cluster, majority, pre_vote;
    int32_t fast_paths;
    int32_t force_wide;
    int32_t require_fence;
    int32_t has_bases;
    int32_t auto_window;
    uint32_t stride;
};

struct ReplicateParams {
    DevTable t;
    uint32_t count;
    const uint32_t *gid;
    const uint8_t *heartbeat;
    const uint16_t *in_flight;
    rg_send_head_t *head;
    rg_send_t *send;
    uint16_t *counts;
    const rg_ev_head_t *ev_head;
    const I32x4 *ev_out32;
    uint32_t ev_stride, self;
};

struct TimerParams {
    int64_t *deadline;
    uint32_t *epoch;
    const Ident *ident;
    uint32_t groups, rounds, count;
    const uint32_t *gid;
    const rg_reply_t *reply;
    const I32x4 *out32, *persist32;
    const int64_t *now_mem;
    int64_t now[64];
    int64_t election_ms, heartbeat_ms;
    uint64_t seed;
};

struct HealthParams {
    int64_t *ok, *fail;
    int32_t *recent;
    DevTable t;
    uint32_t rounds, count, followers, self;
    const uint32_t *gid;
    const rg_ev_head_t *head;
    const rg_reply_t *reply;
    const I32x4 *out32;
    const int64_t *now_mem;
    int64_t now[64];
    uint16_t *counts;
};

struct TickFoldParams {
    TimerParams tp;
    HealthParams hp;
    const int64_t *now_last;
    unsigned long long *masks;
    uint32_t *ticket;
    uint32_t *out_gid, *out_epoch, *out_count;
    uint32_t capacity;
    int expire;
    const uint32_t *rounds_now;
};
struct TickTailParams {
    TickFoldParams fp;
    ReplicateParams qp;
    HealthParams rp;
    int32_t critical_point;
    int64_t cool_down;
    uint8_t *ready;
};

hipError_t launch_step(const StepParams &p, int followers, bool sparse, int shape, hipStream_t s);
hipError_t launch_copy(const void *src, void *dst, size_t bytes, hipStream_t s);
hipError_t launch_replicate(const ReplicateParams &p, int followers, hipStream_t s);
hipError_t launch_health_update(const HealthParams &p, hipStream_t s);
hipError_t launch_health_failure(const HealthParams &p, uint32_t n, const uint32_t *gid, const uint8_t *slot, const uint8_t *flags, const uint16_t *done, hipStream_t s);
hipError_t launch_ready(const HealthParams &p, int64_t now, int32_t cp, int64_t cd, uint8_t *ready, hipStream_t s);
hipError_t launch_timers_update(const TimerParams &p, hipStream_t s);
hipError_t launch_tick_fold(const TickFoldParams &p, hipStream_t s);
hipError_t launch_tick_tail(const TickTailParams &p, int followers, hipStream_t s);
hipError_t launch_tick(const StepParams &p, const TickTailParams &tp, int followers, hipStream_t s);
hipError_t launch_tick_sparse(const StepParams &p, const TickTailParams &tp, const uint32_t *rows_now, int followers, hipStream_t s);
hipError_t launch_tick_expire(const TickFoldParams &p, hipStream_t s);
hipError_t launch_timers_arm(const TimerParams &p, hipStream_t s);
hipError_t launch_timers_expired(int64_t *deadline, const Ident *ident, uint32_t groups, int64_t now, const int64_t *now_mem, uint32_t *counts, uint32_t *total,
                                 uint32_t *out_gid, uint32_t *out_epoch, uint32_t capacity, hipStream_t s);
hipError_t launch_outcome_count(const rg_reply_t *reply, uint32_t rows, uint32_t *counts, uint32_t *totals, hipStream_t s);
hipError_t launch_outcome_emit(const rg_reply_t *reply, const I64x2 *logfx, const rg_persist_t *persist, uint32_t rows, const uint32_t *counts,
                               I64x2 *out_logfx, uint32_t cap_logfx, rg_persist_t *out_persist, uint32_t cap_persist, hipStream_t s);

__device__ __forceinline__ int64_t wadd(int64_t a, int64_t b) { return (int64_t)((uint64_t)a + (uint64_t)b); }
__device__ __forceinline__ int64_t wsub(int64_t a, int64_t b) { return (int64_t)((uint64_t)a - (uint64_t)b); }
__device__ __forceinline__ int64_t max64(int64_t a, int64_t b) { return a > b ? a : b; }
__device__ __forceinline__ int64_t min64(int64_t a, int64_t b) { return a < b ? a : b; }
template <class V> __device__ __forceinline__ V vadd(V x, V y) { typedef typename std::make_unsigned<V>::type U; return (V)((U)x + (U)y); }
template <class V> __device__ __forceinline__ V vmin(V x, V y) { return x < y ? x : y; }
template <class V> __device__ __forceinline__ V vmax(V x, V y) { return x > y ? x : y; }

constexpr uint32_t EV_LIMIT = 1u << 30;
constexpr uint32_t STATE_LIMIT = (1u << 30) + (1u << 29);

template <class V>
__device__ __forceinline__ void cmp_exchange(V &a, V &b)
{
    const bool sw = a > b;
    const V lo = sw ? b : a, hi = sw ? a : b;
    a = lo; b = hi;
}
template <int F, class V>
__device__ __forceinline__ void major_indices(V (&m)[F], V &full, V &major)
{
    if constexpr (F == 4 && sizeof(V) == 4) {
        const V lo1 = vmin(m[0], m[1]), hi1 = vmax(m[0], m[1]), lo2 = vmin(m[2], m[3]), hi2 = vmax(m[2], m[3]);
        full = vmin(lo1, lo2);
        major = vmax(vmax(lo1, lo2), vmin(hi1, hi2));
    } else if constexpr (F == 4) {
        cmp_exchange(m[0], m[1]); cmp_exchange(m[2], m[3]);
        cmp_exchange(m[0], m[2]); cmp_exchange(m[1], m[3]);
        full = m[0]; major = m[1] > m[2] ? m[1] : m[2];
    } else {
#pragma unroll
        for (int a = 1; a < F; a++) {
#pragma unroll
            for (int b = a; b > 0; b--) cmp_exchange(m[b - 1], m[b]);
        }
        full = m[0]; major = m[F / 2];
    }
}

__device__ __forceinline__ int64_t rejection_step(int32_t r)
{
    if (r < 0) return r == -1 ? 1 : 0;
    int64_t s = 1;
    s += r >= 2; s += r >= 10; s += r >= 31; s += r >= 88; s += r >= 242; s += r >= 663; s += r >= 1806;
    s += r >= 4913; s += r >= 13358; s += r >= 36313; s += r >= 98714; s += r >= 268335; s += r >= 729414;
    s += r >= 1982757; s += r >= 5389696; s += r >= 14650717; s += r >= 39824782; s += r >= 108254986;
    s += r >= 294267564; s += r >= 799902175;
    return s;
}

template <class V>
struct FxT {
    uint32_t flags;
    uint32_t status;
    V resp_term;
    V log_from;
};
typedef FxT<int64_t> Fx;

constexpr uint32_t HDR_AE_OK = 1u << 10, HDR_PEER_OK = 1u << 11, HDR_WIDE = 1u << 9;

template <class V>
struct GroupT {
    V term, commit, epoch_index, epoch_term, first, last, elected_term;
    V s0, s1, s2, s3;
// ... 897 lines not shown
```

### rafting_amd/csrc/rg_kernels.hip

```cpp
#include "rg_device.hpp"
#include "rg_step.hpp"

namespace rg {

__device__ __forceinline__ void wave_lds_sync()
{
    __builtin_amdgcn_s_waitcnt(0xC07F);
    __builtin_amdgcn_wave_barrier();
}
__device__ __forceinline__ void stream_store(uint4 *dst, const uint4 v)
{
    const u32x4 q = {v.x, v.y, v.z, v.w};
    __builtin_nontemporal_store(q, reinterpret_cast<u32x4 *>(dst));
}

template <int F>
__device__ __forceinline__ void replicate_wave(const ReplicateParams &p, uint4 *st, const uint32_t i0, const uint32_t lane, const uint32_t stride, const uint32_t rounds)
{
    const uint32_t i = i0 + lane;
    const bool active = i < p.count;
    const uint32_t ir = active ? i : p.count - 1u;
    const uint32_t gi = p.gid ? p.gid[ir] : ir;
    const uint32_t G = p.t.groups;
    const I64x2 tc = p.t.term_commit[gi], ep = p.t.epoch[gi], w = p.t.window[gi];
// ... 664 lines not shown
{
    if (n == 0) return hipSuccess;
    hipLaunchKernelGGL(health_failure_kernel, dim3((n + 255) / 256), dim3(256), 0, s, p, n, gid, slot, flags, done);
    return hipGetLastError();
}
hipError_t launch_ready(const HealthParams &p, int64_t now, int32_t cp, int64_t cd, uint8_t *ready, hipStream_t s)
{
    hipLaunchKernelGGL(ready_kernel, dim3((p.t.groups + 255) / 256), dim3(256), 0, s, p, now, cp, cd, ready);
    return hipGetLastError();
}

constexpr int COPY_UNROLL = 4;
__global__ __launch_bounds__(256) void copy_kernel(const u32x4 *__restrict__ src, u32x4 *__restrict__ dst, size_t n)
{
    const size_t per = (n + gridDim.x - 1) / gridDim.x;
    const size_t lo = (size_t)blockIdx.x * per, hi = lo + per < n ? lo + per : n;
    size_t i = lo + threadIdx.x;
    for (; i + (COPY_UNROLL - 1) * 256 < hi; i += COPY_UNROLL * 256) {
        u32x4 v[COPY_UNROLL];
#pragma unroll
        for (int k = 0; k < COPY_UNROLL; k++) v[k] = __builtin_nontemporal_load(src + i + k * 256);
#pragma unroll
        for (int k = 0; k < COPY_UNROLL; k++) __builtin_nontemporal_store(v[k], dst + i + k * 256);
    }
    for (; i < hi; i += 256) dst[i] = src[i];
}

__device__ __forceinline__ bool row_has_logfx(uint32_t fa)
{
    return ((fa & (RG_F_COMMIT | RG_F_LOG_APPEND | RG_F_LOG_TRUNC)) != 0u) | (RG_F_STATUS(fa) == (uint32_t)RG_NEED_HOST);
}
__global__ __launch_bounds__(256) void outcome_count_kernel(const rg_reply_t *__restrict__ reply, uint32_t rows, uint32_t *n_logfx, uint32_t *n_persist)
{
    const uint32_t i = blockIdx.x * 256u + threadIdx.x;
    const uint32_t fa = i < rows ? reply[i].flags : 0u;
    const unsigned long long ml = __ballot(row_has_logfx(fa)), mp = __ballot((fa & RG_F_PERSIST) != 0u);
    if ((threadIdx.x & 63u) == 0u && i < rows) { n_logfx[i >> 6] = (uint32_t)__popcll(ml); n_persist[i >> 6] = (uint32_t)__popcll(mp); }
}
__global__ __launch_bounds__(256) void outcome_emit_kernel(const rg_reply_t *__restrict__ reply, const I64x2 *__restrict__ logfx,
                                                           const rg_persist_t *__restrict__ persist, uint32_t rows, const uint32_t *off_logfx,
                                                           const uint32_t *off_persist, I64x2 *out_logfx, uint32_t cap_logfx,
                                                           rg_persist_t *out_persist, uint32_t cap_persist)
{
    const uint32_t i = blockIdx.x * 256u + threadIdx.x;
    const uint32_t fa = i < rows ? reply[i].flags : 0u;
    const bool hl = row_has_logfx(fa), hp = (fa & RG_F_PERSIST) != 0u;
    const unsigned long long ml = __ballot(hl), mp = __ballot(hp);
    const unsigned long long below = (1ull << (threadIdx.x & 63u)) - 1ull;
    if (hl) {
        const uint32_t pos = off_logfx[i >> 6] + (uint32_t)__popcll(ml & below);
        if (pos < cap_logfx) out_logfx[pos] = logfx[i];
    }
    if (hp) {
        const uint32_t pos = off_persist[i >> 6] + (uint32_t)__popcll(mp & below);
        if (pos < cap_persist) out_persist[pos] = persist[i];
    }
}

hipError_t launch_outcome_count(const rg_reply_t *reply, uint32_t rows, uint32_t *counts, uint32_t *totals, hipStream_t s)
{
    const uint32_t blocks = (rows + 255u) / 256u, waves = (rows + 63u) / 64u;
    hipLaunchKernelGGL(outcome_count_kernel, dim3(blocks), dim3(256), 0, s, reply, rows, counts, counts + waves);
    hipLaunchKernelGGL(timers_scan_kernel, dim3(1), dim3(1024), 0, s, counts, waves, totals);
    hipLaunchKernelGGL(timers_scan_kernel, dim3(1), dim3(1024), 0, s, counts + waves, waves, totals + 1);
    return hipGetLastError();
}
hipError_t launch_outcome_emit(const rg_reply_t *reply, const I64x2 *logfx, const rg_persist_t *persist, uint32_t rows, const uint32_t *counts,
                               I64x2 *out_logfx, uint32_t cap_logfx, rg_persist_t *out_persist, uint32_t cap_persist, hipStream_t s)
{
    const uint32_t blocks = (rows + 255u) / 256u, waves = (rows + 63u) / 64u;
    hipLaunchKernelGGL(outcome_emit_kernel, dim3(blocks), dim3(256), 0, s, reply, logfx, persist, rows, counts, counts + waves, out_logfx, cap_logfx,
                       out_persist, cap_persist);
    return hipGetLastError();
}

hipError_t launch_copy(const void *src, void *dst, size_t bytes, hipStream_t s)
{
    hipLaunchKernelGGL(copy_kernel, dim3(2048), dim3(256), 0, s, (const u32x4 *)src, (u32x4 *)dst, bytes / 16);
    return hipGetLastError();
}

#endif

#define RG_FOLLOWER_LAUNCHERS(X) X(StepLaunch) X(TickLaunch) X(TickSparseLaunch) X(TickTailLaunch)
#if defined(RG_TU) && RG_TU == 1
#define RG_PER_UNIT(L) extern template hipError_t launch_range<L, 7>(const L &, int); extern template hipError_t launch_range<L, 11>(const L &, int);
#elif defined(RG_TU)
#define RG_PER_UNIT(L) template hipError_t launch_range<L, RG_TU>(const L &, int);
#else
#define RG_PER_UNIT(L)
#endif
RG_FOLLOWER_LAUNCHERS(RG_PER_UNIT)
#undef RG_PER_UNIT
#ifdef RG_TU_MAIN
hipError_t launch_step(const StepParams &p, int followers, bool sparse, int shape, hipStream_t s) { return launch_followers(StepLaunch{p, sparse, shape, s}, followers); }
hipError_t launch_replicate(const ReplicateParams &p, int followers, hipStream_t s) { return launch_followers(ReplicateLaunch{p, s}, followers); }
hipError_t launch_tick(const StepParams &p, const TickTailParams &tp, int followers, hipStream_t s) { return launch_followers(TickLaunch{p, tp, s}, followers); }
hipError_t launch_tick_sparse(const StepParams &p, const TickTailParams &tp, const uint32_t *rows_now, int followers, hipStream_t s)
{
    return launch_followers(TickSparseLaunch{p, tp, rows_now, s}, followers);
}
hipError_t launch_tick_tail(const TickTailParams &p, int followers, hipStream_t s) { return launch_followers(TickTailLaunch{p, s}, followers); }
#endif

}

#ifdef RG_TU_MAIN
#define RG_ASSEMBLE_KERNELS 1
#endif
#include "rg_assemble.hpp"
```

### rafting_amd/csrc/rg_step.hpp

```cpp
#pragma once
#include "rg_device.hpp"
#include "rg_tier1n.hpp"

namespace rg {

typedef uint32_t u32x2 __attribute__((vector_size(8)));
typedef uint32_t u32x4 __attribute__((vector_size(16)));

template <class T> __device__ __forceinline__ T nt_load16(const T *p)
{
    static_assert(sizeof(T) == 16, "16-byte row");
    const u32x4 v = __builtin_nontemporal_load(reinterpret_cast<const u32x4 *>(p));
    T r; __builtin_memcpy(&r, &v, 16); return r;
}
template <class T> __device__ __forceinline__ T nt_load8(const T *p)
{
    static_assert(sizeof(T) == 8, "8-byte row");
    const u32x2 v = __builtin_nontemporal_load(reinterpret_cast<const u32x2 *>(p));
    T r; __builtin_memcpy(&r, &v, 8); return r;
}
template <class T> __device__ __forceinline__ void nt_store16(T *p, const T &x)
{
    static_assert(sizeof(T) == 16, "16-byte row");
    u32x4 v; __builtin_memcpy(&v, &x, 16);
// ... 61 lines not shown
    e.hdr = h.hdr; e.aux = h.aux;
    if constexpr (EV32) {
        const I32x4 q = nt_load16(p.abcd32 + row);
        e.a = q.x; e.b = q.y; e.c = q.z; e.d = q.w;
    } else {
        const I64x2 ab = nt_load16(p.ab + row), cd = nt_load16(p.cd + row);
        e.a = ab.x; e.b = ab.y; e.c = cd.x; e.d = cd.y;
    }
}

template <bool EV32>
__device__ __forceinline__ void load_event_tail(const StepParams &p, size_t row, const EventRow &e, EventTail &t)
{
    if constexpr (EV32) {
        t.hx = 0; t.hy = 0;
        t.e0 = (int64_t)(int32_t)e.aux; t.e1 = t.e0; t.e2 = t.e0; t.e3 = t.e0;
    } else {
        if (p.hint != nullptr && RG_HDR_HINT(e.hdr)) { const I64x2 hh = p.hint[row]; t.hx = hh.x; t.hy = hh.y; }
        const uint32_t n = RG_HDR_N(e.hdr);
        const bool have_terms = (p.entry_terms != nullptr) & (p.entry_count != 0);
        const char *base = have_terms ? reinterpret_cast<const char *>(p.entry_terms) : reinterpret_cast<const char *>(p.head);
        const bool ae = (RG_HDR_KIND(e.hdr) == RG_EV_AE_REQ) & (n > 0) & have_terms & ((uint64_t)e.aux + n <= p.entry_count);
        const uint32_t o = e.aux * 8u;
        const uint32_t o0 = ae ? o : 0u, o1 = (ae & (n > 1u)) ? o + 8u : 0u, o2 = (ae & (n > 2u)) ? o + 16u : 0u,
                       o3 = (ae & (n > 3u)) ? o + 24u : 0u;
        t.e0 = *reinterpret_cast<const int64_t *>(base + o0); t.e1 = *reinterpret_cast<const int64_t *>(base + o1);
        t.e2 = *reinterpret_cast<const int64_t *>(base + o2); t.e3 = *reinterpret_cast<const int64_t *>(base + o3);
    }
}

template <bool EV32>
__device__ __forceinline__ uint32_t decorate(const StepParams &p, const EventRow &e, const EventTail &t, bool mark_out_of_domain)
{
    const uint32_t hdr = e.hdr, kind = RG_HDR_KIND(hdr), slot = RG_HDR_SLOT(hdr), n = RG_HDR_N(hdr);
    const uint32_t P = (uint32_t)p.cluster, self = (uint32_t)p.self;
    const bool peer_ok = (slot < P) & (slot != self);
    bool one_term;
    uint32_t keep;
    if constexpr (EV32) {
        const bool same = (hdr & RG_HDR_SAME_TERM) != 0;
        one_term = (n == 0) | same;
        keep = (hdr & ~(7u << 9)) | (same ? HDR_SAME_IN : 0u);
    } else {
        const bool readable = (n <= 4u) & (p.entry_terms != nullptr) & ((uint64_t)e.aux + n <= p.entry_count);
        const bool same = ((n < 2u) | (t.e1 == t.e0)) & ((n < 3u) | (t.e2 == t.e0)) & ((n < 4u) | (t.e3 == t.e0));
        one_term = (n == 0) | (readable & same);
        keep = hdr & ~(3u << 10);
    }
    const bool ae_ok = (kind == RG_EV_AE_REQ) & (slot < P) & (e.c != 0) & (n <= RG_MAX_AE_ENTRIES) & one_term;
    uint32_t out = keep | (ae_ok ? HDR_AE_OK : 0u) | (peer_ok ? HDR_PEER_OK : 0u);
    if constexpr (EV32) {
        if (mark_out_of_domain) {
            const uint32_t w = (uint32_t)(int32_t)e.a | (uint32_t)(int32_t)e.b | (uint32_t)(int32_t)e.c | (uint32_t)(int32_t)e.d |
                               (((kind == RG_EV_AE_REQ) & ((hdr & RG_HDR_SAME_TERM) != 0)) ? e.aux : 0u);
            out = (w >= EV_LIMIT) ? (out | KIND_OUT_OF_DOMAIN) : out;
        }
    }
    return out;
}

template <bool EV32>
__device__ __forceinline__ Entries entries_of(const StepParams &p, uint32_t hdr_in, uint32_t aux, int64_t e0, int64_t e1, int64_t e2, int64_t e3)
{
    Entries en;
    if constexpr (EV32) {
        en.t64 = nullptr;
        en.t32 = p.entry_terms32 ? p.entry_terms32 + aux : nullptr;
        en.same = ((hdr_in & HDR_SAME_IN) != 0) & (RG_HDR_KIND(hdr_in) == RG_EV_AE_REQ);
        en.prefetched = false;
        en.e0 = (int64_t)(int32_t)aux; en.e1 = en.e0; en.e2 = en.e0; en.e3 = en.e0;
    } else {
        en.t64 = p.entry_terms ? p.entry_terms + aux : nullptr;
        en.t32 = nullptr;
        en.same = false;
        en.prefetched = true;
        en.e0 = e0; en.e1 = e1; en.e2 = e2; en.e3 = e3;
    }
    return en;
}
__device__ __forceinline__ bool entries_readable(const StepParams &p, const Entries &en, uint32_t aux, uint32_t n)
{
    return en.same | (((en.t64 != nullptr) | (en.t32 != nullptr)) & ((uint64_t)aux + n <= p.entry_count));
}

__device__ __forceinline__ void load_group(const DevTable &t, uint32_t gi, Group &g)
{
    const uint32_t G = t.groups;
    const I64x2 tc = t.term_commit[gi], ep = t.epoch[gi], w = t.window[gi];
    const Ident id = t.ident[gi];
    const Elect el = t.elect[gi];
    g.term = tc.x; g.commit = tc.y; g.epoch_index = ep.x; g.epoch_term = ep.y; g.first = w.x; g.last = w.y;
    g.voted_for = id.voted_for; g.leader = id.leader; g.role_epoch = id.role_epoch;
    g.role = (int32_t)(id.meta & META_ROLE);
    g.td = (id.meta & META_TD) != 0; g.prepared = (id.meta & META_PREP) != 0;
    g.rc = (int32_t)((id.meta >> META_RC_SHIFT) & 7u);
    g.pending = (id.meta >> META_PEND_SHIFT) & META_PEND_MASK;
    g.elected_term = el.elected_term; g.elected_epoch = el.elected_epoch; g.votes = el.votes;
    const I64x2 r0 = t.runs[gi], r1 = t.runs[(size_t)G + gi], r2 = t.runs[(size_t)2 * G + gi], r3 = t.runs[(size_t)3 * G + gi];
    g.s0 = r0.x; g.t0 = r0.y; g.s1 = r1.x; g.t1 = r1.y; g.s2 = r2.x; g.t2 = r2.y; g.s3 = r3.x; g.t3 = r3.y;
    g.log_dirty = false; g.peers_dirty = false;
    g.refresh_tail();
}

template <int F>
__device__ __forceinline__ void stage_peers(const DevTable &t, uint32_t gi, const Group &g, PeersWide<F> &pe)
{
    if (!g.prepared) return;
    const uint32_t G = t.groups;
#pragma unroll
    for (int j = 0; j < F; j++) {
        const I64x2 en = t.peer_en[(size_t)j * G + gi];
        const Match m = t.peer_m[(size_t)j * G + gi];
        pe.set_last_epoch(j, en.x); pe.set_next_index(j, en.y);
        pe.set_match_index(j, m.match_index); pe.set_rejection(j, m.rejection);
    }
}
template <int F>
__device__ __forceinline__ bool stage_peers(const DevTable &t, uint32_t gi, bool prepared, PeersNarrow<F> &pe)
{
    if (!prepared) return true;
    const uint32_t G = t.groups;
    const int64_t base = pe.base;
    uint64_t w = 0;
#pragma unroll
    for (int j = 0; j < F; j++) {
        const I64x2 en = t.peer_en[(size_t)j * G + gi];
        const Match m = t.peer_m[(size_t)j * G + gi];
        const int64_t ep = to_rel(en.x, base), nx = to_rel(en.y, base), mt = to_rel(m.match_index, base);
        w |= (uint64_t)ep | (uint64_t)nx | (uint64_t)mt;
        pe.rec[j * BLOCK] = I32x4{(int32_t)ep, (int32_t)nx, (int32_t)mt, m.rejection};
        *pe.mslot(j) = (int32_t)mt;
    }
    return w < (uint64_t)EV_LIMIT;
}

template <class PE>
__device__ __forceinline__ void store_group(const DevTable &t, uint32_t gi, const Group &g, const PE &pe, int followers)
{
    const uint32_t G = t.groups;
    t.term_commit[gi] = I64x2{g.term, g.commit};
    t.epoch[gi] = I64x2{g.epoch_index, g.epoch_term};
    t.window[gi] = I64x2{g.first, g.last};
    Ident id;
    id.voted_for = g.voted_for; id.leader = g.leader; id.role_epoch = g.role_epoch;
    id.meta = (uint32_t)g.role | (g.td ? META_TD : 0u) | (g.prepared ? META_PREP : 0u) |
              ((uint32_t)g.rc << META_RC_SHIFT) | (g.pending << META_PEND_SHIFT);
    t.ident[gi] = id;
    Elect el;
    el.elected_term = g.elected_term; el.elected_epoch = g.elected_epoch; el.votes = g.votes;
    t.elect[gi] = el;
    if (g.log_dirty) {
        t.runs[gi] = I64x2{g.s0, g.t0};
        t.runs[(size_t)G + gi] = I64x2{g.s1, g.t1};
        t.runs[(size_t)2 * G + gi] = I64x2{g.s2, g.t2};
        t.runs[(size_t)3 * G + gi] = I64x2{g.s3, g.t3};
    }
    if (g.peers_dirty) {
        for (int j = 0; j < followers; j++) {
            t.peer_en[(size_t)j * G + gi] = I64x2{pe.last_epoch(j), pe.next_index(j)};
            Match m;
            m.match_index = pe.match_index(j); m.rejection = pe.rejection(j); m.pad = 0;
            t.peer_m[(size_t)j * G + gi] = m;
        }
    }
}

// ... 96 lines not shown
    load_event_tail<false>(p, ir, cur, cur_t);
    for (uint32_t r = 0; r < p.rounds; r++) {
        const size_t row = (size_t)r * round_rows + ir;
        __builtin_amdgcn_s_waitcnt(0x0F70);
        if (r > 0) {
            if (active) nt_store16(p.reply + (row - round_rows), pend_rep);
            if (pend_w_lfx) nt_store16(p.logfx + (row - round_rows), pend_lfx);
            if (pend_w_per) nt_store16(p.persist + (row - round_rows), pend_per);
        }
        const uint32_t r1 = r + 1u < p.rounds ? r + 1u : last_round, r2 = r + 2u < p.rounds ? r + 2u : last_round;
        load_event<false>(p, (size_t)r2 * round_rows + ir, far);
        load_event_tail<false>(p, (size_t)r1 * round_rows + ir, near, near_t);

        {
            const uint32_t kind = RG_HDR_KIND(cur.hdr);
            const bool skip = blocked & (kind != RG_EV_NONE);
            flush_max = ((kind == RG_EV_LOG_FLUSH) & (cur.a > flush_max)) ? cur.a : flush_max;
            const uint32_t hdr = decorate<false>(p, cur, cur_t, false);
            const bool done = tier1<F, int64_t, PeersWide<F>>(p, g, pe, st.fx, FAST & !skip, hdr, cur.aux, cur.a, cur.b, cur.c, cur.d, cur_t.e0);
            bool slow = !done & !skip;
            if (skip) st.fx = Fx{0u, RG_SKIPPED_AFTER_NEED_HOST, 0, 0};
            if (__builtin_amdgcn_ballot_w64(slow) != 0) {
                if (slow) slow = !tier15w<F, int64_t, PeersWide<F>>(p, g, pe, st.fx, FAST, hdr, cur.aux, (RG_HDR_HINT(cur.hdr) != 0) & (p.hint != nullptr), cur.a, cur.b, cur.c, cur.d, cur_t.e0);
                if (slow) {
                    const Entries en = entries_of<false>(p, cur.hdr, cur.aux, cur_t.e0, cur_t.e1, cur_t.e2, cur_t.e3);
                    st.run(cur.hdr, cur.aux, cur.a, cur.b, cur.c, cur.d, (RG_HDR_HINT(cur.hdr) != 0) & (p.hint != nullptr), cur_t.hx, cur_t.hy, en,
                           entries_readable(p, en, cur.aux, RG_HDR_N(cur.hdr)));
                }
            }
            const uint32_t status = st.fx.status, flags = st.fx.flags;
            if (status == RG_NEED_HOST) blocked = true;
            pend_rep.resp_term = (flags & RG_F_REPLIED) ? st.fx.resp_term : 0;
            pend_rep.flags = flags | ((uint32_t)g.role << RG_F_ROLE_SHIFT) | (status << RG_F_STATUS_SHIFT);
            pend_rep.role_epoch = g.role_epoch;
            pend_w_lfx = active & (((flags & (RG_F_COMMIT | RG_F_LOG_APPEND | RG_F_LOG_TRUNC)) != 0) | (status == RG_NEED_HOST));
            pend_lfx = I64x2{g.commit, st.fx.log_from};
            pend_w_per = active & ((flags & RG_F_PERSIST) != 0);
            pend_per.term = g.term; pend_per.voted_for = g.voted_for; pend_per.role = g.role;
            tally.add(kind, flags, status);
        }
        cur = near; cur_t = near_t;
        near = far;
    }
    if (active) {
        const size_t row = (size_t)(p.rounds - 1) * round_rows + ir;
        nt_store16(p.reply + row, pend_rep);
        if (pend_w_lfx) nt_store16(p.logfx + row, pend_lfx);
        if (pend_w_per) nt_store16(p.persist + row, pend_per);
    }

    if (active) {
        store_group(p.t, gi, g, pe, F);
        if (p.auto_window != 0) advance_base(p, gi, p.t.ibase[gi], flush_max);
    }
    tally.flush(p, lane, active);
}

enum { EV_HEAD = 0, EV_A, EV_B, EV_C, EV_D, EV_E0, EV_HX, EV_HY, EV_E1, EV_E2, EV_E3, EV_FIELDS };
enum { OUT_RESP = 0, OUT_FLAGS, OUT_COMMIT, OUT_FROM, OUT_TERM, OUT_VOTE, OUT_FIELDS };

__device__ __forceinline__ void lds_barrier()
{
    __builtin_amdgcn_s_waitcnt(0xC07F);
    __builtin_amdgcn_s_barrier();
    asm volatile("" ::: "memory");
}

template <int F, bool EV32, int NO = 2>
struct SplitLds {
    static constexpr int EVF = EV32 ? (int)EV_D + 1 : (int)EV_FIELDS;
    static constexpr size_t W_EPOCH = 0, W_NEXT = W_EPOCH + F * BLOCK * 8, W_MATCH = W_NEXT + F * BLOCK * 8, W_REJ = W_MATCH + F * BLOCK * 8,
                            W_EV = W_REJ + F * BLOCK * 4, W_OUT = W_EV + 2 * EVF * BLOCK * 8, W_AUTO = W_OUT + 2 * OUT_FIELDS * BLOCK * 8,
                            W_END = W_AUTO + BLOCK * 24;
    static constexpr int MV = (F + 3) / 4;
    static constexpr int NEV = 4;
    static constexpr size_t N_REC = 0, N_MV = N_REC + F * BLOCK * 16, N_EVH = N_MV + MV * BLOCK * 16, N_EVQ = N_EVH + NEV * BLOCK * 16,
                            N_O0 = N_EVQ + NEV * BLOCK * 16, N_O1 = N_O0 + NO * BLOCK * 16, N_BAIL = N_O1 + NO * BLOCK * 16,
                            N_LUTC = N_BAIL + 16, N_LUTM = N_LUTC + 256 * 4, N_LUTE = N_LUTM + 128 * 4,
                            N_BASE = N_LUTE + 128 * 2, N_LUTS = N_BASE + BLOCK * 8,
                            N_END = N_LUTS + 64 * 4;
    static constexpr size_t BYTES = EV32 ? (W_END > N_END ? W_END : N_END) : W_END;
};

template <int F, bool SPARSE, bool EV32, bool OUT32 = false>
__device__ __forceinline__ void split_body(const StepParams &p, unsigned char *smem)
{
    static_assert(EV32 || !OUT32, "compact outcome rows belong to the compact-row kernels");
    typedef SplitLds<F, EV32> L;
    int64_t *sh_epoch = reinterpret_cast<int64_t *>(smem + L::W_EPOCH), *sh_next = reinterpret_cast<int64_t *>(smem + L::W_NEXT),
            *sh_match = reinterpret_cast<int64_t *>(smem + L::W_MATCH);
    int32_t *sh_rej = reinterpret_cast<int32_t *>(smem + L::W_REJ);
    uint64_t (*sh_ev)[L::EVF][BLOCK] = reinterpret_cast<uint64_t (*)[L::EVF][BLOCK]>(smem + L::W_EV);
    uint64_t (*sh_out)[OUT_FIELDS][BLOCK] = reinterpret_cast<uint64_t (*)[OUT_FIELDS][BLOCK]>(smem + L::W_OUT);

    const uint32_t lane = threadIdx.x & (BLOCK - 1);
    const bool io_wave = __builtin_amdgcn_readfirstlane(threadIdx.x) >= (uint32_t)BLOCK;
    const uint32_t i = blockIdx.x * BLOCK + lane;
    const bool active = i < p.count;
    const uint32_t ir = active ? i : p.count - 1u;
    const uint32_t last_round = p.rounds - 1u;
    const uint32_t round_rows = SPARSE ? p.stride : p.count;

    if (io_wave) {
        auto row_of = [&](uint32_t r) { return (size_t)(r < p.rounds ? r : last_round) * round_rows + ir; };
        int64_t io_base = 0;
        if constexpr (EV32) io_base = (p.has_bases != 0) ? p.t.ibase[SPARSE ? p.gid[ir] : ir] : 0;
        const bool io_rel = EV32 && __builtin_amdgcn_ballot_w64(io_base != 0) != 0;
        auto publish = [&](uint32_t slot, const EventRow &e, const EventTail &t) {
            sh_ev[slot][EV_HEAD][lane] = (uint64_t)decorate<EV32>(p, e, t, false) | ((uint64_t)e.aux << 32);
            if (io_rel) {
                const uint32_t ix = index_fields(RG_HDR_KIND(e.hdr));
                sh_ev[slot][EV_A][lane] = (uint64_t)((ix & 1u) ? to_abs(e.a, io_base) : e.a); sh_ev[slot][EV_B][lane] = (uint64_t)((ix & 2u) ? to_abs(e.b, io_base) : e.b);
                sh_ev[slot][EV_C][lane] = (uint64_t)((ix & 4u) ? to_abs(e.c, io_base) : e.c); sh_ev[slot][EV_D][lane] = (uint64_t)((ix & 8u) ? to_abs(e.d, io_base) : e.d);
            } else {
                sh_ev[slot][EV_A][lane] = (uint64_t)e.a; sh_ev[slot][EV_B][lane] = (uint64_t)e.b; sh_ev[slot][EV_C][lane] = (uint64_t)e.c; sh_ev[slot][EV_D][lane] = (uint64_t)e.d;
            }
            if constexpr (!EV32) {
                sh_ev[slot][EV_E0][lane] = (uint64_t)t.e0;
                sh_ev[slot][EV_HX][lane] = (uint64_t)t.hx; sh_ev[slot][EV_HY][lane] = (uint64_t)t.hy;
                sh_ev[slot][EV_E1][lane] = (uint64_t)t.e1;
                sh_ev[slot][EV_E2][lane] = (uint64_t)t.e2; sh_ev[slot][EV_E3][lane] = (uint64_t)t.e3;
            }
        };
        Tally tally;
        auto retire = [&](uint32_t r, uint32_t hdr) {
            const uint32_t slot = r & 1u;
            const size_t row = (size_t)r * round_rows + ir;
            const uint64_t fe = sh_out[slot][OUT_FLAGS][lane];
            const uint32_t flags_all = (uint32_t)fe, flags = flags_all & 0xFFFFu, status = RG_F_STATUS(flags_all);
            rg_reply_t rep;
            rep.resp_term = (int64_t)sh_out[slot][OUT_RESP][lane]; rep.flags = flags_all; rep.role_epoch = (uint32_t)(fe >> 32);
            const bool w_lfx = active & (((flags & (RG_F_COMMIT | RG_F_LOG_APPEND | RG_F_LOG_TRUNC)) != 0) | (status == RG_NEED_HOST));
            const bool w_per = active & ((flags & RG_F_PERSIST) != 0);
            const I64x2 lfx{(int64_t)sh_out[slot][OUT_COMMIT][lane], (int64_t)sh_out[slot][OUT_FROM][lane]};
            const uint64_t v = sh_out[slot][OUT_VOTE][lane];
            rg_persist_t per;
            per.term = (int64_t)sh_out[slot][OUT_TERM][lane]; per.voted_for = (int32_t)(uint32_t)v; per.role = (int32_t)(uint32_t)(v >> 32);
            if constexpr (OUT32) {
                const int64_t commit_r = io_rel ? to_rel(lfx.x, io_base) : lfx.x, from_r = io_rel ? to_rel(lfx.y, io_base) : lfx.y;
                const uint64_t bits = (uint64_t)rep.resp_term | (uint64_t)commit_r | (w_lfx ? (uint64_t)from_r : 0ull) | (w_per ? (uint64_t)per.term : 0ull);
                const bool wide = bits >= (1ull << 31);
                if (active) {
                    nt_store16(p.out32 + row, I32x4{(int32_t)rep.resp_term, (int32_t)(flags_all | (wide ? RG_F_WIDE_VALUES : 0u)), (int32_t)commit_r, (int32_t)from_r});
                    if (w_per) nt_store16(p.persist32 + row, I32x4{(int32_t)per.term, per.voted_for, (int32_t)rep.role_epoch, per.role});
                    if (wide & (p.reply != nullptr)) {
                        nt_store16(p.reply + row, rep);
                        if (w_lfx) nt_store16(p.logfx + row, lfx);
                        if (w_per) nt_store16(p.persist + row, per);
                    }
                }
            } else {
                if (active) nt_store16(p.reply + row, rep);
                if (w_lfx) nt_store16(p.logfx + row, lfx);
                if (w_per) nt_store16(p.persist + row, per);
            }
            tally.add(RG_HDR_KIND(hdr), flags, status);
        };

        EventRow n1{}, n2{}, n3{}, n4{};
        EventTail t1{}, t2{};
        uint32_t hdr_cur, hdr_prev = 0u;
        {
            EventRow first{};
            EventTail first_t{};
            load_event<EV32>(p, row_of(0), first);
            load_event<EV32>(p, row_of(1), n1);
            load_event<EV32>(p, row_of(2), n2);
            load_event<EV32>(p, row_of(3), n3);
            load_event<EV32>(p, row_of(4), n4);
            load_event_tail<EV32>(p, row_of(0), first, first_t);
            load_event_tail<EV32>(p, row_of(1), n1, t1);
            load_event_tail<EV32>(p, row_of(2), n2, t2);
            publish(0u, first, first_t);
            hdr_cur = first.hdr;
        }
        lds_barrier();
        for (uint32_t r = 0; r < p.rounds; r++) {
            publish((r + 1u) & 1u, n1, t1);
            if (r > 0) retire(r - 1u, hdr_prev);
            hdr_prev = hdr_cur; hdr_cur = n1.hdr;
            n1 = n2; t1 = t2;
            n2 = n3;
            n3 = n4;
            load_event_tail<EV32>(p, row_of(r + 3u), n2, t2);
            load_event<EV32>(p, row_of(r + 5u), n4);
            lds_barrier();
        }
        retire(last_round, hdr_prev);
        tally.flush(p, lane, active);
        return;
    }

    __builtin_amdgcn_s_setprio(3);
    const uint32_t gi = SPARSE ? p.gid[ir] : ir;
    Group g;
    load_group(p.t, gi, g);
    PeersWide<F> pe;
    pe.e = sh_epoch + lane; pe.n = sh_next + lane; pe.m = sh_match + lane; pe.r = sh_rej + lane; pe.overflow = false;
    stage_peers<F>(p.t, gi, g, pe);
    Stepper<F, PeersWide<F>> st(p, g, pe);
    const bool FAST = p.fast_paths != 0;
    bool blocked = false;
    int64_t *sh_flush = reinterpret_cast<int64_t *>(smem + L::W_AUTO) + 3 * lane;
    sh_flush[0] = 0;
    sh_flush[1] = (active & (p.auto_window != 0)) ? (int64_t)reinterpret_cast<uint64_t>(p.t.ibase + gi) : 0;
    sh_flush[2] = p.auto_window;
    lds_barrier();
    for (uint32_t r = 0; r < p.rounds; r++) {
        const uint32_t slot = r & 1u;
        const uint64_t head = sh_ev[slot][EV_HEAD][lane];
        const uint32_t hdr = (uint32_t)head, aux = (uint32_t)(head >> 32);
        const int64_t a = (int64_t)sh_ev[slot][EV_A][lane], b = (int64_t)sh_ev[slot][EV_B][lane],
                      c = (int64_t)sh_ev[slot][EV_C][lane], d = (int64_t)sh_ev[slot][EV_D][lane];
        int64_t e0 = (int64_t)(int32_t)aux;
        if constexpr (!EV32) e0 = (int64_t)sh_ev[slot][EV_E0][lane];
        const uint32_t kind = RG_HDR_KIND(hdr);
        { const int64_t top = *sh_flush; *sh_flush = ((kind == RG_EV_LOG_FLUSH) & (a > top)) ? a : top; }
        const bool skip = blocked & (kind != RG_EV_NONE);
        const bool done = tier1<F, int64_t, PeersWide<F>>(p, g, pe, st.fx, FAST & !skip, hdr, aux, a, b, c, d, e0);
        bool slow = !done & !skip;
        if (skip) st.fx = Fx{0u, RG_SKIPPED_AFTER_NEED_HOST, 0, 0};
        if (__builtin_amdgcn_ballot_w64(slow) != 0) {
            if (slow) slow = !tier15w<F, int64_t, PeersWide<F>>(p, g, pe, st.fx, FAST, hdr, aux, EV32 ? false : ((RG_HDR_HINT(hdr) != 0) & (p.hint != nullptr)), a, b, c, d, e0);
            if (slow) {
                int64_t hx = 0, hy = 0, e1 = e0, e2 = e0, e3 = e0;
                if constexpr (!EV32) {
                    hx = (int64_t)sh_ev[slot][EV_HX][lane]; hy = (int64_t)sh_ev[slot][EV_HY][lane];
                    e1 = (int64_t)sh_ev[slot][EV_E1][lane]; e2 = (int64_t)sh_ev[slot][EV_E2][lane]; e3 = (int64_t)sh_ev[slot][EV_E3][lane];
                }
                const Entries en = entries_of<EV32>(p, hdr, aux, e0, e1, e2, e3);
                const bool hinted = EV32 ? false : ((RG_HDR_HINT(hdr) != 0) & (p.hint != nullptr));
                st.run(hdr, aux, a, b, c, d, hinted, hx, hy, en, entries_readable(p, en, aux, RG_HDR_N(hdr)));
            }
        }
        const uint32_t status = st.fx.status, flags = st.fx.flags;
        if (status == RG_NEED_HOST) blocked = true;
        const uint32_t flags_all = flags | ((uint32_t)g.role << RG_F_ROLE_SHIFT) | (status << RG_F_STATUS_SHIFT);
        sh_out[slot][OUT_RESP][lane] = (flags & RG_F_REPLIED) ? (uint64_t)st.fx.resp_term : 0ull;
        sh_out[slot][OUT_FLAGS][lane] = (uint64_t)flags_all | ((uint64_t)g.role_epoch << 32);
        sh_out[slot][OUT_COMMIT][lane] = (uint64_t)g.commit;
        sh_out[slot][OUT_FROM][lane] = (uint64_t)st.fx.log_from;
        sh_out[slot][OUT_TERM][lane] = (uint64_t)g.term;
        sh_out[slot][OUT_VOTE][lane] = (uint64_t)(uint32_t)g.voted_for | ((uint64_t)(uint32_t)g.role << 32);
        lds_barrier();
    }
    uint32_t gi_out = gi;
    RG_FRESH_VGPR(gi_out);
    if (active) store_group(p.t, gi_out, g, pe, F);
    if (const int64_t at = sh_flush[1]; at != 0) {
        RG_GLOBAL_AS int64_t *slot = reinterpret_cast<RG_GLOBAL_AS int64_t *>((uint64_t)at);
        const int64_t top = sh_flush[0], window = sh_flush[2];
        if (top - window > *slot) *slot = top - window;
    }
}

template <int F, bool SPARSE>
__global__ __launch_bounds__(2 * BLOCK) void step_split_kernel(const StepParams p)
{
    __shared__ alignas(16) unsigned char smem[SplitLds<F, false>::BYTES];
    split_body<F, SPARSE, false>(p, smem);
}

struct Row32 { U32x2 h; I32x4 q; };

constexpr int CW_AUXC = 18;
template <int F = 0>
__device__ __forceinline__ uint32_t class_entry(const StepParams &p, uint32_t idx)
{
    const uint32_t kind = idx & 15u, slot = idx >> 4;
    const uint32_t P = (uint32_t)p.cluster, self = (uint32_t)p.self;
    const bool peer_ok = (slot < P) & (slot != self);
    const bool ack = (kind == RG_EV_AE_ACK) & peer_ok, vreq = (kind == RG_EV_RV_REQ) | (kind == RG_EV_PV_REQ),
               vrep = (kind == RG_EV_RV_REPLY) | (kind == RG_EV_PV_REPLY);
    const uint32_t j = ack ? (slot < self ? slot : slot - 1u) : 0u;
    const uint32_t cls = (ack ? 1u << CW_ACK : 0u) | (((kind == RG_EV_AE_REQ) & (slot < P)) ? 1u << CW_AE : 0u) | ((kind == RG_EV_CLIENT_APPEND) ? 1u << CW_CLIENT : 0u) |
                         (((ack | (kind == RG_EV_IS_ACK)) & peer_ok) ? 1u << CW_ACKANY : 0u) |
                         ((kind - (uint32_t)RG_EV_RV_REQ <= (uint32_t)(RG_EV_TIMEOUT - RG_EV_RV_REQ)) ? 1u << CW_ELK : 0u) |
                         ((vrep & peer_ok) ? 1u << CW_VR : 0u) | ((kind == RG_EV_PV_REPLY) ? 1u << CW_PV : 0u) | ((kind == RG_EV_TIMEOUT) ? 1u << CW_TO : 0u) |
                         ((vreq & (slot < P)) ? 1u << CW_VQ : 0u) | ((kind == RG_EV_PV_REQ) ? 1u << CW_PVQ : 0u) | ((kind == RG_EV_NONE) ? 1u << CW_NONE : 0u) |
                         ((((0x1CCu >> kind) & 1u) != 0) ? 1u << CW_AUXC : 0u);
    const uint32_t j4 = F > 6 ? (j & 15u) : j;
    return cls | (j4 << 10) | (slot << 5) | (31u - j);
}
__device__ __forceinline__ I32x4 class_word(const uint32_t *lutc, const Row32 &x)
{
    const uint32_t hdr = x.h.x, aux = x.h.y;
    const uint32_t e = lutc[hdr & 0xFFu];
    const int32_t n = (int32_t)(hdr >> 12);
    const sw same = (int32_t)(hdr << (31 - 10));
    const int32_t n_lim = (same >> 31) & (int32_t)RG_MAX_AE_ENTRIES;
    const sw ae_bad = ~s_pos(x.q.z) | s_lt(n_lim, n), cli_bad = s_lt(n, 1);
    const uint32_t auxm = (uint32_t)(((int32_t)(e << (31 - CW_AUXC)) | ((int32_t)(e << (31 - CW_AE)) & same)) >> 31);
    const uint32_t w = (uint32_t)x.q.x | (uint32_t)x.q.y | (uint32_t)x.q.z | (uint32_t)x.q.w | (aux & auxm);
    const uint32_t ood = (uint32_t)((int32_t)(w | (w << 1)) >> 31);
    const uint32_t off = (((uint32_t)ae_bad & 0x80000000u) >> (31 - CW_AE)) | (((uint32_t)cli_bad & 0x80000000u) >> (31 - CW_CLIENT)) | (1u << CW_AUXC) |
                         (ood & 0xFFF80000u);
    const uint32_t cw = (e & ~off) | ((hdr & 0x100u) << (CW_FLAG - 8));
    return I32x4{(int32_t)cw, (int32_t)aux, n, (int32_t)(hdr | (ood & KIND_OUT_OF_DOMAIN))};
}
__device__ __forceinline__ uint32_t expand_by_table(const uint32_t *lutm, const uint16_t *lute, uint32_t w)
{
    const uint32_t fast = lutm[w & 127u] | (uint32_t)lute[(w >> 7) & 127u];
    return ((int32_t)w < 0) ? (w & 0x00FFFFFFu) : fast;
}

template <int F, bool SPARSE, bool OUT32, int IOW = 1, int RPB = 1>
__device__ __forceinline__ bool narrow_body(const StepParams &p, unsigned char *smem)
{
    static_assert(RPB == 1 || (RPB == 2 && IOW == 1), "two rounds per hand-over: the two-wavefront workgroup only");
    constexpr int NO = 2 * RPB;
    typedef SplitLds<F, true, NO> L;
    I32x4 *sh_rec = reinterpret_cast<I32x4 *>(smem + L::N_REC);
    int32_t *sh_mv = reinterpret_cast<int32_t *>(smem + L::N_MV);
    I32x4 (*sh_evh)[BLOCK] = reinterpret_cast<I32x4 (*)[BLOCK]>(smem + L::N_EVH);
    I32x4 (*sh_evq)[BLOCK] = reinterpret_cast<I32x4 (*)[BLOCK]>(smem + L::N_EVQ);
    I32x4 (*sh_o0)[BLOCK] = reinterpret_cast<I32x4 (*)[BLOCK]>(smem + L::N_O0);
    I32x4 (*sh_o1)[BLOCK] = reinterpret_cast<I32x4 (*)[BLOCK]>(smem + L::N_O1);
    uint32_t *sh_bail = reinterpret_cast<uint32_t *>(smem + L::N_BAIL);
    uint32_t *sh_lutc = reinterpret_cast<uint32_t *>(smem + L::N_LUTC), *sh_lutm = reinterpret_cast<uint32_t *>(smem + L::N_LUTM);
    uint16_t *sh_lute = reinterpret_cast<uint16_t *>(smem + L::N_LUTE);
    uint32_t *sh_luts = reinterpret_cast<uint32_t *>(smem + L::N_LUTS);

    const uint32_t lane = threadIdx.x & (BLOCK - 1);
    const bool io_wave = __builtin_amdgcn_readfirstlane(threadIdx.x) >= (uint32_t)BLOCK;
    const uint32_t i = blockIdx.x * BLOCK + lane;
    const bool active = i < p.count;
    const uint32_t ir = active ? i : p.count - 1u;
    const uint32_t last_round = p.rounds - 1u;

    if (io_wave) {
        RG_HWID_BEGIN(1);
        const bool do_pub = IOW == 1 || __builtin_amdgcn_readfirstlane(threadIdx.x) < 2u * BLOCK;
        const bool do_ret = IOW == 1 || !do_pub;
        uint64_t b_head = reinterpret_cast<uint64_t>(p.head), b_q = reinterpret_cast<uint64_t>(p.abcd32),
                 b_reply = OUT32 ? reinterpret_cast<uint64_t>(p.out32) : reinterpret_cast<uint64_t>(p.reply),
                 b_logfx = reinterpret_cast<uint64_t>(p.logfx),
                 b_persist = OUT32 ? reinterpret_cast<uint64_t>(p.persist32) : reinterpret_cast<uint64_t>(p.persist);
        RG_OWN_SGPRS(b_head); RG_OWN_SGPRS(b_q); RG_OWN_SGPRS(b_reply); RG_OWN_SGPRS(b_logfx); RG_OWN_SGPRS(b_persist);
        const uint64_t round_rows = SPARSE ? p.stride : p.count;
        const uint32_t irm = ir & 0x0FFFFFFFu;
        int64_t io_base = 0;
        if constexpr (!OUT32) io_base = (p.has_bases != 0) ? p.t.ibase[SPARSE ? p.gid[ir] : ir] : 0;
        auto fetch = [&](uint32_t r, Row32 &x) {
            const uint64_t rb = (uint64_t)(r < p.rounds ? r : last_round) * round_rows;
            x.h = nt_load_at<U32x2>(b_head + rb * 8u, irm);
            x.q = nt_load_at<I32x4>(b_q + rb * 16u, irm);
        };
#pragma unroll
        for (int k = 0; k < 4; k++) sh_lutc[lane + 64u * k] = class_entry<F>(p, lane + 64u * k);
#pragma unroll
        for (int k = 0; k < 2; k++) {
            const uint32_t i7 = lane + 64u * k;
            sh_lutm[i7] = expand_predicates(i7);
            sh_lute[i7] = (uint16_t)(expand_predicates((i7 << 7) | 0x42u) & 0xFFFFu);
        }
        sh_luts[lane] = Tally::status_entry(lane);
        __builtin_amdgcn_wave_barrier();
        auto publish = [&](uint32_t slot, const Row32 &x) {
            sh_evh[slot][lane] = class_word(sh_lutc, x);
            sh_evq[slot][lane] = x.q;
        };
        Tally tally;
        auto retire = [&](uint32_t r, uint32_t hdr) {
            const uint32_t slot = r & (uint32_t)(NO - 1);
            const uint64_t rb16 = (uint64_t)r * round_rows * 16u;
            const I32x4 o0 = sh_o0[slot][lane], o1 = sh_o1[slot][lane];
            const uint32_t flags_all = expand_by_table(sh_lutm, sh_lute, (uint32_t)o0.y) | ((uint32_t)o1.w << RG_F_ROLE_SHIFT), flags = flags_all & 0xFFFFu, status = RG_F_STATUS(flags_all);
            if constexpr (OUT32) {
                nt_store_at(b_reply + rb16, irm, I32x4{(flags & RG_F_REPLIED) ? o0.x : 0, (int32_t)flags_all, o0.w, o1.x});
                if ((flags & RG_F_PERSIST) != 0) nt_store_at(b_persist + rb16, irm, I32x4{o1.y, o1.z, o0.z, o1.w});
            } else {
                rg_reply_t rep;
                rep.resp_term = (flags & RG_F_REPLIED) ? (int64_t)(uint32_t)o0.x : 0; rep.flags = flags_all; rep.role_epoch = (uint32_t)o0.z;
                nt_store_at(b_reply + rb16, irm, rep);
                const bool w_lfx = ((flags & (RG_F_COMMIT | RG_F_LOG_APPEND | RG_F_LOG_TRUNC)) != 0) | (status == RG_NEED_HOST);
                if (w_lfx) nt_store_at(b_logfx + rb16, irm, I64x2{to_abs((int64_t)(uint32_t)o0.w, io_base), to_abs((int64_t)(uint32_t)o1.x, io_base)});
                if ((flags & RG_F_PERSIST) != 0) {
                    rg_persist_t per;
                    per.term = (int64_t)(uint32_t)o1.y; per.voted_for = o1.z; per.role = o1.w;
                    nt_store_at(b_persist + rb16, irm, per);
                }
            }
            tally.add_packed_lut(RG_HDR_KIND(hdr), flags, status, sh_luts);
        };
        Row32 buf[4];
        uint32_t hdr_m1 = 0u, hdr_0, hdr_1;
        if (do_pub) {
            Row32 e0, e1;
            fetch(0, e0); fetch(1, e1); fetch(2, buf[2]); fetch(3, buf[3]); fetch(4, buf[0]); fetch(5, buf[1]);
            publish(0u, e0); publish(1u, e1);
            hdr_0 = e0.h.x; hdr_1 = e1.h.x;
        } else {
            hdr_0 = hdr_1 = 0u;
            for (int k = 0; k < 4; k++) { buf[k].h = U32x2{0u, 0u}; buf[k].q = I32x4{0, 0, 0, 0}; }
        }
        lds_barrier();
        { const uint32_t seen0 = *sh_bail; if (__builtin_amdgcn_readfirstlane(seen0) == 1u) return false; }
        bool bailed = false;
        uint32_t seen = 0u;
        RG_PROBE_BEGIN();
        if constexpr (RPB == 2) {
            uint32_t hk[4] = {hdr_0, hdr_1, 0u, 0u};
            for (uint32_t r0 = 0; r0 < p.rounds && !bailed; r0 += 4u) {
                if ((r0 & 127u) == 124u) tally.spill();
#pragma unroll
                for (int k = 0; k < 4; k++) {
                    const uint32_t r = r0 + (uint32_t)k;
                    if (r >= p.rounds) break;
                    Row32 &x = buf[(k + 2) & 3];
                    publish((r + 2u) & 3u, x);
                    RG_PROBE_MARK(0);
                    if (r >= 2u) retire(r - 2u, hk[(k + 2) & 3]);
                    hk[(k + 2) & 3] = x.h.x;
                    fetch(r + 6u, x);
                    RG_PROBE_MARK(1);
                    if ((k & 1) != 0 || r == last_round) {
                        const uint32_t mark = __builtin_amdgcn_readfirstlane(seen), pair = r >> 1;
                        if ((mark != 0u) & (mark <= pair + 1u)) { bailed = true; break; }
                        lds_barrier();
                        RG_PROBE_MARK(2);
                        seen = *sh_bail;
                    }
                }
            }
            if (bailed) return false;
            { const uint32_t mark = __builtin_amdgcn_readfirstlane(seen); if (mark != 0u) return false; }
            for (uint32_t q = p.rounds >= 2u ? p.rounds - 2u : 0u; q < p.rounds; q++) {
                const uint32_t i = q & 3u;
                retire(q, i == 0u ? hk[0] : (i == 1u ? hk[1] : (i == 2u ? hk[2] : hk[3])));
            }
            tally.spill();
#if defined(RG_PROBE)
            RG_PROBE_FLUSH(0);
#elif defined(RG_PROBE_HWID)
            RG_HWID_END(1);
#else
            tally.flush(p, lane, active);
#endif
            return true;
        }
        for (uint32_t r0 = 0; r0 < p.rounds && !bailed; r0 += 4u) {
            if ((r0 & 127u) == 124u) tally.spill();
#pragma unroll
            for (int k = 0; k < 4; k++) {
                const uint32_t r = r0 + (uint32_t)k;
                if (r >= p.rounds) break;
                Row32 &x = buf[(k + 2) & 3];
                if (do_pub) publish((r + 2u) & 3u, x);
// ... 45 lines not shown
        Group g64;
        load_group(p.t, gi, g64);
        g64.s1 = g64.rc > 1 ? g64.s1 : 0; g64.s2 = g64.rc > 2 ? g64.s2 : 0; g64.s3 = g64.rc > 3 ? g64.s3 : 0;
        if (any_base) g64 = group_to_rel(g64, base);
        in_domain = fits32(g64, EV_LIMIT) & small_fields_fit(g64) & (p.force_wide == 0) & (p.rounds < (1u << 24)) & ((base == 0) | (g64.epoch_index > 0)) & (base >= 0);
        narrow_into(g, g64);
        g.nallow = FAST ? 0 : -1;
        g.recache();
        in_domain = in_domain & stage_peers<F>(p.t, gi, g64.prepared, pe);
    }
    bool bailed = __builtin_amdgcn_ballot_w64(!in_domain) != 0;
    if (lane == 0) *sh_bail = bailed ? 1u : 0u;
    bool blocked = false;
    int32_t flush_max = 0;
    lds_barrier();
    if (bailed) return false;
    RG_PROBE_BEGIN();
#ifdef RG_EVENT_PREFETCH
    I32x4 h_next = sh_evh[0][lane], q_next = sh_evq[0][lane];
#endif
    auto round = [&](const uint32_t r) {
#ifdef RG_EVENT_PREFETCH
        const I32x4 h = h_next, q = q_next;
#else
        const I32x4 h = sh_evh[r & 3u][lane], q = sh_evq[r & 3u][lane];
#endif
        RG_PROBE_MARK(0);
        OutN out;
        const sw done = tier1n<F>(p, g, pe, out, h.x, (uint32_t)h.y, h.z, q.x, q.y, q.z, q.w);
        const bool open = done >= 0;
        RG_PROBE_MARK(1);
        const uint64_t b_open = __builtin_amdgcn_ballot_w64(open);
        const uint32_t slot = r & (uint32_t)(NO - 1);
        sh_o0[slot][lane] = I32x4{out.resp, (int32_t)out.pw, (int32_t)g.role_epoch, g.commit};
        sh_o1[slot][lane] = I32x4{out.log_from, g.term, g.voted_for, g.role};
        if (b_open != 0) {
            const uint32_t hdr = ((uint32_t)h.w & ~(7u << 9)) | ((((uint32_t)h.w & RG_HDR_SAME_TERM) != 0) ? HDR_SAME_IN : 0u), aux = (uint32_t)h.y, kind = RG_HDR_KIND(hdr);
            const bool skip = open & blocked & (kind != RG_EV_NONE);
            flush_max = (open & (kind == RG_EV_LOG_FLUSH) & (q.x > flush_max)) ? q.x : flush_max;
            bool park;
            const bool slow = open & !skip & !tier15<F>(p, g, pe, out, park, open & !skip, h.x, h.y, h.z, q.x, q.y, q.z, q.w);
            if (park) { blocked = true; g.nallow = -1; g.recache(); }
            RG_NOTE_SLOW(slow, lane == 0);
            bool bail = (slow | (skip & (p.auto_window != 0))) & (kind == KIND_OUT_OF_DOMAIN);
            if (slow & !bail) {
                const int64_t base = any_base ? *sh_base : 0;
                pe.base = base;
                Group g64 = group_to_abs(widen(g), base);
                Stepper<F, PeersNarrow<F>> st(p, g64, pe);
                const Entries en = entries_of<true>(p, hdr, aux, 0, 0, 0, 0);
                const uint32_t ix = index_fields(kind);
                st.run(hdr, aux, (ix & 1u) ? to_abs(q.x, base) : (int64_t)q.x, (ix & 2u) ? to_abs(q.y, base) : (int64_t)q.y,
                       (ix & 4u) ? to_abs(q.z, base) : (int64_t)q.z, (ix & 8u) ? to_abs(q.w, base) : (int64_t)q.w, false, 0, 0, en, entries_readable(p, en, aux, RG_HDR_N(hdr)));
                g64 = group_to_rel(g64, base);
                st.fx.log_from = to_rel(st.fx.log_from, base);
                bail = !fits32(g64, STATE_LIMIT) | !small_fields_fit(g64) | pe.overflow | ((base != 0) & (g64.epoch_index <= 0)) |
                       (((uint64_t)st.fx.resp_term | (uint64_t)st.fx.log_from) >= (uint64_t)STATE_LIMIT);
                narrow_into(g, g64);
                if (st.fx.status == RG_NEED_HOST) blocked = true;
                g.nallow = (FAST & !blocked) ? 0 : -1;
                g.recache();
                out.pw = PW_SLOW | st.fx.flags | (st.fx.status << RG_F_STATUS_SHIFT);
                out.resp = (int32_t)st.fx.resp_term; out.log_from = (int32_t)st.fx.log_from;
            }
            if (skip) { out.pw = PW_SLOW | ((uint32_t)RG_SKIPPED_AFTER_NEED_HOST << RG_F_STATUS_SHIFT); out.resp = 0; out.log_from = 0; }
            if (__builtin_amdgcn_ballot_w64(bail) != 0) {
                if (lane == 0) *sh_bail = r / (uint32_t)RPB + 2u;
                bailed = true;
            }
            sh_o0[slot][lane] = I32x4{out.resp, (int32_t)out.pw, (int32_t)g.role_epoch, g.commit};
            sh_o1[slot][lane] = I32x4{out.log_from, g.term, g.voted_for, g.role};
        } else {
            RG_NOTE_SLOW(false, lane == 0);
        }
        RG_PROBE_MARK(2);
#ifdef RG_EVENT_PREFETCH
        h_next = sh_evh[(r + 1u) & 3u][lane]; q_next = sh_evq[(r + 1u) & 3u][lane];
#endif
        if constexpr (RPB == 1) {
            lds_barrier();
            RG_PROBE_MARK(3);
        }
    };
    if constexpr (RPB == 2) {
        for (uint32_t r = 0; r < p.rounds; r++) {
            round(r);
            if (bailed) break;
            if ((r & 1u) != 0u || r == last_round) {
                lds_barrier();
                RG_PROBE_MARK(3);
            }
        }
        if (bailed) lds_barrier();
    } else {
#ifdef RG_EVENT_PREFETCH
    { uint32_t r = 0; do { round(r); r++; } while (!bailed & (r < p.rounds)); }
#else
    for (uint32_t r = 0; r < p.rounds; r++) {
        round(r);
        if (bailed) break;
    }
#endif
    }
    if (bailed) return false;
    RG_PROBE_FLUSH(4);
    RG_HWID_END(0);
    if (active) {
        Group g64 = widen(g);
        pe.base = 0;
        if (any_base) {
            const int64_t base = *sh_base;
            pe.base = base;
            g64 = group_to_abs(g64, base);
        }
        uint32_t gi_out = gi;
        RG_FRESH_VGPR(gi_out);
        store_group(p.t, gi_out, g64, pe, F);
        if (p.auto_window != 0) {
            const int64_t base = *sh_base;
            advance_base(p, gi_out, base, to_abs(flush_max, base));
        }
    }
    return true;
}

#ifndef RG_NOTE_FALLBACK
#define RG_NOTE_FALLBACK() ((void)0)
#endif

#ifndef RG_ROUNDS_PER_HANDOVER
#define RG_ROUNDS_PER_HANDOVER 1
#endif
template <int F, bool SPARSE, int WAVES, bool OUT32, int IOW = 1>
__global__ __launch_bounds__((1 + IOW) * BLOCK) __attribute__((amdgpu_waves_per_eu(WAVES, 8))) void step32_kernel(const StepParams p)
{
    constexpr int RPB = (WAVES == 1 && IOW == 1) ? RG_ROUNDS_PER_HANDOVER : 1;
    __shared__ alignas(16) unsigned char smem[SplitLds<F, true, 2 * RPB>::BYTES];
    if (narrow_body<F, SPARSE, OUT32, IOW, RPB>(p, smem)) return;
    if (threadIdx.x == 0) { RG_NOTE_FALLBACK(); atomicAdd(p.wide_bodies, 1ull); }
    if constexpr (IOW == 2) {
        if (__builtin_amdgcn_readfirstlane(threadIdx.x) >= 2u * BLOCK) {
            for (uint32_t k = 0; k < p.rounds + 2u; k++) lds_barrier();
            return;
        }
    }
    lds_barrier();
    split_body<F, SPARSE, true, OUT32>(p, smem);
}

template <int F, bool SPARSE, int WAVES, bool OUT32>
__global__ __launch_bounds__(2 * BLOCK) __attribute__((amdgpu_waves_per_eu(WAVES, 8))) void step32_wide_kernel(const StepParams p)
{
    __shared__ alignas(16) unsigned char smem[SplitLds<F, true>::BYTES];
    if (threadIdx.x == 0) { RG_NOTE_FALLBACK(); atomicAdd(p.wide_bodies, 1ull); }
    split_body<F, SPARSE, true, OUT32>(p, smem);
}

#if !defined(RG_BUILD_ONLY_F4)
#define RG_F_MASK 0x7FFEu
#elif defined(RG_BUILD_ALSO_F)
#define RG_F_MASK ((1u << 4) | (RG_BUILD_ALSO_F))
#else
#define RG_F_MASK (1u << 4)
#endif

#if !defined(RG_TU) || RG_TU == 1
#define RG_TU_MAIN 1
#endif

template <class L, int F>
static hipError_t launch_one(const L &l)
{
    if constexpr (((RG_F_MASK) >> F) & 1u) return l.template run<F>();
    else return hipErrorInvalidValue;
}
template <class L, int LO>
hipError_t launch_range(const L &l, int followers)
{
    switch (followers - LO) {
    case 0: return launch_one<L, LO>(l);
    case 1: return launch_one<L, LO + 1>(l);
    case 2: return launch_one<L, LO + 2>(l);
    case 3: return launch_one<L, LO + 3>(l);
    default: return hipErrorInvalidValue;
    }
}
template <class L>
static hipError_t launch_followers(const L &l, int followers)
{
    switch (followers) {
    case 1: return launch_one<L, 1>(l);
    case 2: return launch_one<L, 2>(l);
    case 3: return launch_one<L, 3>(l);
    case 4: return launch_one<L, 4>(l);
    case 5: return launch_one<L, 5>(l);
    case 6: return launch_one<L, 6>(l);
    case 7: case 8: case 9: case 10: return launch_range<L, 7>(l, followers);
    case 11: case 12: case 13: case 14: return launch_range<L, 11>(l, followers);
    default: return hipErrorInvalidValue;
    }
}

template <class Fn>
static hipError_t lift(bool b, Fn fn) { return b ? fn(std::true_type{}) : fn(std::false_type{}); }

template <int F> constexpr int WAVES_MANY = F <= 6 ? 4 : 1;
constexpr uint32_t MANY_BLOCKS = 1024u;
#ifdef RG_IOW2
constexpr int SMALL_IOW = 2;
#else
constexpr int SMALL_IOW = 1;
#endif

template <int F, bool SPARSE, bool OUT32>
static hipError_t launch_compact(const StepParams &p, hipStream_t s)
{
    const uint32_t blocks = (p.count + BLOCK - 1) / BLOCK;
    if (p.count >= (1u << 28)) return hipErrorInvalidValue;
    constexpr int MANY = WAVES_MANY<F>, IOW = (F <= 6 && OUT32 && !SPARSE) ? SMALL_IOW : 1;
    const bool many = blocks > MANY_BLOCKS;
    const dim3 grid(blocks), wg(2 * BLOCK);
    if (p.force_wide != 0) {
        if (many) hipLaunchKernelGGL((step32_wide_kernel<F, SPARSE, MANY, OUT32>), grid, wg, 0, s, p);
        else      hipLaunchKernelGGL((step32_wide_kernel<F, SPARSE, 1, OUT32>), grid, wg, 0, s, p);
    } else {
        if (many) hipLaunchKernelGGL((step32_kernel<F, SPARSE, MANY, OUT32>), grid, wg, 0, s, p);
        else      hipLaunchKernelGGL((step32_kernel<F, SPARSE, 1, OUT32, IOW>), grid, dim3((1 + IOW) * BLOCK), 0, s, p);
    }
    return hipGetLastError();
}

struct StepLaunch {
    const StepParams &p;
    bool sparse;
    int shape;
    hipStream_t s;
    template <int F> hipError_t run() const
    {
        if (shape != 0 && shape != 64 && shape != 32) return hipErrorInvalidValue;
        const StepParams &p = this->p;
        const hipStream_t s = this->s;
        const dim3 grid((p.count + BLOCK - 1) / BLOCK);
        if (grid.x == 0) return hipSuccess;
        return lift(sparse, [&](auto sp) {
            constexpr bool SPARSE = decltype(sp)::value;
            if (shape == 32) return lift(p.out32 != nullptr, [&](auto o) { return launch_compact<F, SPARSE, decltype(o)::value>(p, s); });
            if (shape == 64) hipLaunchKernelGGL((step_kernel<F, SPARSE>), grid, dim3(BLOCK), 0, s, p);
            else             hipLaunchKernelGGL((step_split_kernel<F, SPARSE>), grid, dim3(2 * BLOCK), 0, s, p);
            return hipGetLastError();
        });
    }
};

}
```

### rafting_amd/engine.py

```python
import ctypes as C
import os

import numpy as np

from . import abi

_HERE = os.path.dirname(os.path.abspath(__file__))
LIB_PATH = os.environ.get("RG_LIB") or os.path.join(_HERE, "libraftgpu.so")
_LIB = None


class EngineError(RuntimeError):
    pass


def library_sha16():
    import hashlib
    with open(LIB_PATH, "rb") as f:
        return hashlib.sha256(f.read()).hexdigest()[:16]


def exported_symbols():
    return [
        "rg_abi_version", "rg_table_create", "rg_table_destroy", "rg_last_error", "rg_table_groups",
        "rg_table_cluster", "rg_table_option", "rg_load_state", "rg_read_state", "rg_submit", "rg_submit32", "rg_submit32c", "rg_submit32c_sparse", "rg_submit32c_sparse_rounds", "rg_outcome32_unpack", "rg_outcome32_unpack_rel", "rg_index_base_set", "rg_index_base_get", "rg_index_base_advance", "rg_index_base_advance32", "rg_batch32_pack_rel", "rg_batch32_pack", "rg_submit_async", "rg_submit_async_packed", "rg_submit_wait", "rg_tick_create", "rg_tick_launch", "rg_tick_wait", "rg_tick_destroy", "rg_tick2_create", "rg_tick2_create_sparse", "rg_tick2_create_sparse_rounds", "rg_tick2_launch", "rg_tick2_wait", "rg_tick2_destroy", "rg_assembler_create", "rg_assemble32", "rg_assembler_destroy", "rg_timers_update32", "rg_health_update32", "rg_sync", "rg_step_kernel", "rg_host_alloc", "rg_host_free", "rg_dev_alloc",
        "rg_dev_free", "rg_copy_to_device", "rg_copy_to_host", "rg_stream", "rg_replicate", "rg_timers_configure", "rg_timers_update",
        "rg_timers_expired", "rg_timers_expired_epochs", "rg_timers_arm", "rg_timers_read", "rg_health_update", "rg_health_failure", "rg_ready", "rg_health_read", "rg_in_flight_read", "rg_in_flight_set",
        "rg_timing_enable",
        "rg_timing_read", "rg_timing_begin", "rg_timing_end", "rg_counters_read", "rg_wide_body_workgroups", "rg_copy_bandwidth",
    ]


def _share_hip_runtime_with_torch():
    import importlib.util
    import sys
    if "torch" in sys.modules:
        return
    try:
        spec = importlib.util.find_spec("torch")
    except (ImportError, ValueError):
        spec = None
    if spec is None or not spec.submodule_search_locations:
        return
    cand = os.path.join(list(spec.submodule_search_locations)[0], "lib", "libamdhip64.so")
    if os.path.exists(cand):
        try:
            C.CDLL(cand, mode=C.RTLD_GLOBAL)
        except OSError:
            pass


def lib():
    global _LIB
    if _LIB is None:
        if not os.path.exists(LIB_PATH):
            raise EngineError(
                "%s is missing — build it with `make -C rafting_amd/csrc` (or __graft_entry__.build()); "
                "there is no CPU fallback for the decision path" % LIB_PATH)
        _share_hip_runtime_with_torch()
        L = C.CDLL(LIB_PATH)
        if hasattr(L, "rg_is_host_emulation") and os.environ.get("RG_ALLOW_HOST_EMULATION") != "1":
            raise EngineError("%s is the test-only host emulation of the kernels (tests/devemu), not libraftgpu.so; "
                              "the decision path has no CPU fallback" % LIB_PATH)
        vp, u32, i32 = C.c_void_p, C.c_uint32, C.c_int
        L.rg_abi_version.restype = i32
        L.rg_table_create.argtypes = [i32, u32, u32, u32, i32, C.POINTER(vp)]
        L.rg_table_destroy.argtypes = [vp]
        L.rg_last_error.restype = C.c_char_p
        L.rg_last_error.argtypes = [vp]
        L.rg_table_groups.restype = u32
        L.rg_table_groups.argtypes = [vp]
        L.rg_table_cluster.restype = u32
        L.rg_table_cluster.argtypes = [vp]
        L.rg_table_option.argtypes = [vp, i32, i32]
        L.rg_load_state.argtypes = [vp, u32, u32, C.POINTER(abi.CGroupState)]
        L.rg_read_state.argtypes = [vp, u32, u32, C.POINTER(abi.CGroupState)]
        L.rg_submit.argtypes = [vp, C.POINTER(abi.CBatch), C.POINTER(abi.COutcome), i32]
        L.rg_submit32.argtypes = [vp, C.POINTER(abi.CBatch32), C.POINTER(abi.COutcome), i32]
        if os.environ.get("RG_LIB"):
            class _Tolerant:
                def __init__(self, lib_):
                    object.__setattr__(self, "_lib", lib_)

                def __getattr__(self, name):
                    try:
                        return getattr(self._lib, name)
                    except AttributeError:
                        class _Missing:
                            def __call__(self, *a):
                                raise EngineError("%s is not exported by %s" % (name, LIB_PATH))
                        return _Missing()
            real, L = L, _Tolerant(L)
        L.rg_submit32c.argtypes = [vp, C.POINTER(abi.CBatch32), C.POINTER(abi.COutcome32), i32]
        L.rg_submit32c_sparse.argtypes = [vp, C.POINTER(abi.CBatch32), C.POINTER(abi.COutcome32), i32]
        L.rg_submit32c_sparse_rounds.argtypes = [vp, C.POINTER(abi.CBatch32), C.POINTER(abi.COutcome32), i32]
        L.rg_outcome32_unpack.argtypes = [C.POINTER(abi.COutcome32), u32, u32, vp, C.POINTER(abi.COutcome)]
        L.rg_outcome32_unpack_rel.argtypes = [C.POINTER(abi.COutcome32), u32, u32, vp, vp, C.POINTER(abi.COutcome)]
        L.rg_index_base_set.argtypes = [vp, u32, u32, vp]
        L.rg_index_base_get.argtypes = [vp, u32, u32, vp]
        L.rg_index_base_advance.argtypes = [C.POINTER(abi.CBatch), i32, u32, vp]
        L.rg_index_base_advance32.argtypes = [C.POINTER(abi.CBatch32), i32, u32, vp]
        L.rg_batch32_pack_rel.restype = C.c_int64
        L.rg_batch32_pack_rel.argtypes = [C.POINTER(abi.CBatch), vp, vp, vp, vp]
        L.rg_batch32_pack.restype = C.c_int64
        L.rg_batch32_pack.argtypes = [C.POINTER(abi.CBatch), vp, vp, vp]
        L.rg_submit_async.argtypes = [vp, C.POINTER(abi.CBatch), C.POINTER(abi.COutcome)]
        L.rg_submit_wait.argtypes = [vp]
        L.rg_submit_async_packed.argtypes = [vp, vp, vp]
        L.rg_sync.argtypes = [vp]
        L.rg_tick_create.argtypes = [vp, vp, vp, C.POINTER(vp)]
        L.rg_tick_launch.argtypes = [vp]
        L.rg_tick_wait.argtypes = [vp]
        L.rg_tick_destroy.argtypes = [vp]
        L.rg_tick2_create.argtypes = [vp, C.POINTER(abi.CTick2Io), C.POINTER(vp)]
        L.rg_tick2_create_sparse.argtypes = [vp, C.POINTER(abi.CTick2Io), C.POINTER(abi.CTick2Rows), C.POINTER(vp)]
        L.rg_tick2_create_sparse_rounds.argtypes = [vp, C.POINTER(abi.CTick2Io), C.POINTER(abi.CTick2Rounds), C.POINTER(vp)]
        L.rg_tick2_launch.argtypes = [vp]
        L.rg_tick2_wait.argtypes = [vp]
        L.rg_tick2_destroy.argtypes = [vp]
        L.rg_assembler_create.argtypes = [vp, u32, u32, C.POINTER(vp)]
        L.rg_assemble32.argtypes = [vp, C.POINTER(abi.CArrivals), C.POINTER(abi.CAssembled), i32]
        L.rg_assembler_destroy.argtypes = [vp]
        L.rg_timers_update32.argtypes = [vp, u32, vp, vp, vp, i32]
        L.rg_health_update32.argtypes = [vp, u32, vp, vp, vp, i32]
        L.rg_replicate.argtypes = [vp, u32, vp, vp, vp, vp, vp, i32]
        L.rg_step_kernel.restype = C.c_char_p
        L.rg_step_kernel.argtypes = [vp, u32]
        L.rg_timers_configure.argtypes = [vp, C.c_int64, C.c_int64, C.c_uint64]
        L.rg_timers_update.argtypes = [vp, u32, u32, vp, vp, vp, i32]
        L.rg_timers_expired.argtypes = [vp, C.c_int64, vp, u32, C.POINTER(u32), i32]
        L.rg_timers_expired_epochs.argtypes = [vp, C.c_int64, vp, vp, u32, C.POINTER(u32), i32]
        L.rg_timers_arm.argtypes = [vp, C.c_int64]
        L.rg_timers_read.argtypes = [vp, u32, u32, vp]
        L.rg_health_update.argtypes = [vp, u32, u32, vp, vp, vp, vp, i32]
        L.rg_health_failure.argtypes = [vp, u32, vp, vp, vp, C.c_int64]
        L.rg_ready.argtypes = [vp, C.c_int64, i32, C.c_int64, vp, i32]
        L.rg_health_read.argtypes = [vp, u32, u32, vp, vp, vp]
        L.rg_in_flight_read.argtypes = [vp, u32, u32, vp]
        L.rg_in_flight_set.argtypes = [vp, u32, u32, vp]
        L.rg_host_alloc.argtypes = [vp, C.c_size_t, C.POINTER(vp)]
        L.rg_host_free.argtypes = [vp, vp]
        L.rg_dev_alloc.argtypes = [vp, C.c_size_t, C.POINTER(vp)]
        L.rg_dev_free.argtypes = [vp, vp]
        L.rg_copy_to_device.argtypes = [vp, vp, vp, C.c_size_t]
        L.rg_copy_to_host.argtypes = [vp, vp, vp, C.c_size_t]
        L.rg_stream.restype = vp
        L.rg_stream.argtypes = [vp]
        L.rg_timing_enable.argtypes = [vp, i32]
        L.rg_timing_read.argtypes = [vp, C.POINTER(C.c_uint64), C.POINTER(C.c_double), i32]
        L.rg_timing_begin.argtypes = [vp]
        L.rg_timing_end.argtypes = [vp, C.POINTER(C.c_double)]
        L.rg_counters_read.argtypes = [vp, C.POINTER(C.c_uint64), i32]
        L.rg_wide_body_workgroups.argtypes = [vp, C.POINTER(C.c_uint64), i32]
        L.rg_copy_bandwidth.argtypes = [vp, C.c_size_t, i32, C.POINTER(C.c_double)]
        if L.rg_abi_version() != abi.ABI_VERSION:
            raise EngineError("libraftgpu.so ABI %d != binding ABI %d" % (L.rg_abi_version(), abi.ABI_VERSION))
        _LIB = L
    return _LIB


def _replicate(call, groups, cluster, gid, heartbeat, in_flight):
    F = cluster - 1
    gid = None if gid is None else np.ascontiguousarray(gid, dtype=np.uint32)
    count = groups if gid is None else len(gid)
    hb = None if heartbeat is None else np.ascontiguousarray(np.broadcast_to(heartbeat, (count,)), dtype=np.uint8)
    fl = None if in_flight is None else np.ascontiguousarray(np.asarray(in_flight, dtype=np.uint16).reshape(count, F).T).reshape(count * F)
    head = np.zeros(count, dtype=abi.SEND_HEAD_DT)
    send = np.zeros(count * F, dtype=abi.SEND_DT)
    ptr = lambda a: None if a is None else a.ctypes.data
    call(count, ptr(gid), ptr(hb), ptr(fl), head.ctypes.data, send.ctypes.data)
    return head, np.ascontiguousarray(send.reshape(F, count).T)


def advance_index_base(batch, base, window):
    if not (isinstance(base, np.ndarray) and base.dtype == np.int64 and base.flags["C_CONTIGUOUS"]):
        raise EngineError("advance_index_base: base must be a contiguous int64 array (it is updated in place)")
    b = batch.as_struct()
    fn = lib().rg_index_base_advance32 if isinstance(batch, abi.Batch32) else lib().rg_index_base_advance
    rc = fn(C.byref(b), int(window), len(base), base.ctypes.data)
    if rc != 0:
        raise EngineError("advance_index_base: %d (%s)" % (rc, {-1: "missing column or window outside [1, 2^30)", -2: "batch shape does not fit the groups"}.get(rc, "?")))
    return base


def pack32(batch, index_base=None):
    rows = batch.rounds * batch.count
    head = np.zeros(rows, dtype=abi.HEAD_DT)
    abcd = np.zeros(rows, dtype=abi.QUAD32_DT)
    terms = np.zeros(max(batch.entry_count, 1), dtype=np.int32)
    b = batch.as_struct()
    if index_base is None:
        n = lib().rg_batch32_pack(C.byref(b), head.ctypes.data, abcd.ctypes.data, terms.ctypes.data)
    else:
        ib = np.ascontiguousarray(index_base, dtype=np.int64)
        n = lib().rg_batch32_pack_rel(C.byref(b), ib.ctypes.data, head.ctypes.data, abcd.ctypes.data, terms.ctypes.data)
    if n < 0:
        raise EngineError("rg_batch32_pack: %d (%s)" % (n, {-1: "missing column", -2: "the batch carries hints", -3: "a value outside [0, 2^31)",
                                                             -4: "entry_terms needed"}.get(n, "?")))
    return abi.Batch32(batch.rounds, batch.count, batch.gid, head, abcd, terms, n)


def pinned_like(table, array):
    a = np.ascontiguousarray(array)
    p = C.c_void_p()
    table._check(lib().rg_host_alloc(table._h, max(a.nbytes, 16), C.byref(p)))
    buf = (C.c_char * max(a.nbytes, 16)).from_address(p.value)
    view = np.frombuffer(buf, dtype=a.dtype, count=a.size).reshape(a.shape)
    view[...] = a

    class _Owner:
        ptr = p.value

        def free(self):
            if self.ptr:
                lib().rg_host_free(table._h, self.ptr)
                self.ptr = None
    return view, _Owner()


class PackedBatch:

    def __init__(self, table, batch, logfx_cap=None, persist_cap=None, entry_cap=0):
        assert abi.batch_fits_32(batch), "a value outside [0, 2^31) or a hint column: use submit_async for this batch"
        rows = batch.rounds * batch.count
        self.rows, self.table, self._owners = rows, table, []
        b32 = pack32(batch)
        self.head, self.abcd = self._pin(b32.head), self._pin(b32.abcd)
        et = np.zeros(max(entry_cap, b32.entry_count, 1), dtype=np.int32)
        et[:b32.entry_count] = b32.entry_terms[:b32.entry_count]
        self.entry_terms = self._pin(et)
        self.gid = None if batch.gid is None else self._pin(batch.gid)
        self.logfx_cap = rows if logfx_cap is None else logfx_cap
        self.persist_cap = rows if persist_cap is None else persist_cap
        self.reply = self._pin(np.zeros(rows, dtype=abi.REPLY_DT))
        self.logfx = self._pin(np.zeros(max(self.logfx_cap, 1), dtype=abi.LOGFX_DT))
        self.persist = self._pin(np.zeros(max(self.persist_cap, 1), dtype=abi.PERSIST_DT))
# ... 618 lines not shown
        self._check(lib().rg_timers_expired(self._h, now, out.ctypes.data, capacity, C.byref(n), abi.MEM_HOST))
        return out[: min(n.value, capacity)], n.value

    def timers_expired_epochs(self, now, capacity=None):
        capacity = self.groups if capacity is None else capacity
        out, ep = np.zeros(max(capacity, 1), dtype=np.uint32), np.zeros(max(capacity, 1), dtype=np.uint32)
        n = C.c_uint32()
        self._check(lib().rg_timers_expired_epochs(self._h, now, out.ctypes.data, ep.ctypes.data, capacity, C.byref(n), abi.MEM_HOST))
        k = min(n.value, capacity)
        return out[:k], ep[:k], n.value

    def timers_read(self, first=0, count=None):
        count = self.groups - first if count is None else count
        out = np.zeros(count, dtype=np.int64)
        self._check(lib().rg_timers_read(self._h, first, count, out.ctypes.data))
        return out

    def health_update(self, batch, reply, now):
        now = np.ascontiguousarray(now, dtype=np.int64)
        reply = np.ascontiguousarray(reply)
        assert len(now) == batch.rounds and len(reply) == batch.rounds * batch.count
        self._check(lib().rg_health_update(self._h, batch.rounds, batch.count, None if batch.gid is None else batch.gid.ctypes.data,
                                           batch.head.ctypes.data, reply.ctypes.data, now.ctypes.data, abi.MEM_HOST))

    def submit_timed(self, batch, now, fill=0):
        out = self.submit(batch, fill=fill)
        self.health_update(batch, out.reply, now)
        return out

    def submit_and_update_timers(self, batch, now, fill=0):
        out = self.submit(batch, fill=fill)
        self.timers_update(batch.rounds, batch.count, out.reply, now, gid=batch.gid)
        return out

    def health_failure(self, gid, slot, flags, now):
        gid = np.ascontiguousarray(gid, dtype=np.uint32)
        slot = np.ascontiguousarray(slot, dtype=np.uint8)
        flags = np.ascontiguousarray(flags, dtype=np.uint8)
        assert len(gid) == len(slot) == len(flags)
        self._check(lib().rg_health_failure(self._h, len(gid), gid.ctypes.data, slot.ctypes.data, flags.ctypes.data, now))

    def ready(self, now, critical_point, cool_down_ms):
        out = np.zeros(self.groups, dtype=np.uint8)
        self._check(lib().rg_ready(self._h, now, critical_point, cool_down_ms, out.ctypes.data, abi.MEM_HOST))
        return out

    def health_read(self, first=0, count=None):
        count = self.groups - first if count is None else count
        F = self.cluster - 1
        ok, fl, rc = np.zeros((count, F), np.int64), np.zeros((count, F), np.int64), np.zeros((count, F), np.int32)
        self._check(lib().rg_health_read(self._h, first, count, ok.ctypes.data, fl.ctypes.data, rc.ctypes.data))
        return ok, fl, rc

    def replicate(self, gid=None, heartbeat=None, in_flight=None):
        return _replicate(lambda *a: self._check(lib().rg_replicate(self._h, *a, abi.MEM_HOST)), self.groups, self.cluster,
                          gid, heartbeat, in_flight)

    def timing_enable(self, on=True):
        self._check(lib().rg_timing_enable(self._h, int(on)))

    def timing_read(self, reset=True):
        n, ms = C.c_uint64(), C.c_double()
        self._check(lib().rg_timing_read(self._h, C.byref(n), C.byref(ms), int(reset)))
        return n.value, ms.value

    def timing_begin(self):
        self._check(lib().rg_timing_begin(self._h))

    def timing_end(self):
        ms = C.c_double()
        self._check(lib().rg_timing_end(self._h, C.byref(ms)))
        return ms.value

    def counters(self, reset=False):
        arr = (C.c_uint64 * abi.NUM_COUNTERS)()
        self._check(lib().rg_counters_read(self._h, arr, int(reset)))
        return list(arr)

    def wide_body_workgroups(self, reset=False):
        n = C.c_uint64()
        self._check(lib().rg_wide_body_workgroups(self._h, C.byref(n), int(reset)))
        return n.value

    def copy_bandwidth(self, nbytes=1 << 30, iters=10):
        g = C.c_double()
        self._check(lib().rg_copy_bandwidth(self._h, nbytes, iters, C.byref(g)))
        return g.value
```

Measured before the change: 63.76 billion.

## Chain consecutive compact device submits into one multi-segment kernel launch

```diff
diff --git a/include/raftgpu.h b/include/raftgpu.h
--- a/include/raftgpu.h
+++ b/include/raftgpu.h
@@ -229,6 +229,8 @@
     rg_outcome_t    wide;
 } rg_outcome32_t;
 int rg_submit32c(rg_table_t *t, const rg_batch32_t *in, const rg_outcome32_t *out, int memspace);
+#define RG_SUBMIT_CHAIN_DEFAULT_CAP 4
+int rg_submit_chain_stats(rg_table_t *t, uint64_t *chained_launches, uint64_t *chained_batches, int reset);
 int rg_submit32c_sparse(rg_table_t *t, const rg_batch32_t *in, const rg_outcome32_t *out, int memspace);
 int rg_submit32c_sparse_rounds(rg_table_t *t, const rg_batch32_t *in, const rg_outcome32_t *out, int memspace);
 int rg_outcome32_unpack(const rg_outcome32_t *in, uint32_t rounds, uint32_t count, uint32_t *role_epoch, const rg_outcome_t *out);
diff --git a/rafting_amd/csrc/raftgpu.cpp b/rafting_amd/csrc/raftgpu.cpp
--- a/rafting_amd/csrc/raftgpu.cpp
+++ b/rafting_amd/csrc/raftgpu.cpp
@@ -71,6 +71,10 @@
     hipStream_t s_in = nullptr, s_out = nullptr;
     PipeSlot pipe[RG_PIPELINE_DEPTH];
     uint64_t pipe_head = 0, pipe_tail = 0;
+    int chain_mode = 1;
+    uint32_t chain_cap = RG_SUBMIT_CHAIN_DEFAULT_CAP;
+    rg::ChainParams chain{};
+    uint64_t chained_launches = 0, chained_batches = 0;
     std::string err;
 };
 
@@ -101,9 +105,46 @@
     return 0;
 }
 
-static int bind(rg_table *t, bool drain = true)
-{
+extern "C" { static int launch(rg_table *t, const rg::StepParams &p, bool sparse); }
+
+static int flush_chain(rg_table *t)
+{
+    const uint32_t n = t->chain.nseg;
+    if (n == 0) return 0;
+    t->chain.nseg = 0;
     HIP_TRY(t, hipSetDevice(t->device));
+    if (n == 1) {
+        rg::StepParams p = t->chain.p;
+        const rg::ChainSeg &sg = t->chain.seg[0];
+        p.head = sg.head; p.abcd32 = sg.abcd32; p.out32 = sg.out32; p.persist32 = sg.persist32; p.rounds = sg.rounds;
+        return launch(t, p, false);
+    }
+    rg::ChainParams c = t->chain;
+    c.nseg = n;
+    if (hipError_t e = rg::launch_chain(c, (int)t->F, t->stream); e != hipSuccess)
+        return fail(t, -2, "a chained launch of %u held rg_submit32c batches failed: %s", n, hipGetErrorString(e));
+    t->chained_launches += 1;
+    t->chained_batches += n;
+    return 0;
+}
+
+static bool stream_busy(rg_table *t)
+{
+#ifdef __HIPCC__
+    const hipError_t e = hipStreamQuery(t->stream);
+    (void)hipGetLastError();
+    return e == hipErrorNotReady;
+#else
+    (void)t;
+    return false;
+#endif
+}
+
+static int bind(rg_table *t, bool drain = true, bool flush = true)
+{
+    HIP_TRY(t, hipSetDevice(t->device));
+    if (flush)
+        if (int rc = flush_chain(t)) return rc;
     while (drain && t->pipe_tail != t->pipe_head)
         if (int rc = wait_oldest(t); rc < 0) return rc;
     return 0;
@@ -145,6 +186,7 @@
 int rg_table_option(rg_table_t *t, int option, int value)
 {
     if (!t) return -1;
+    if (int rc = flush_chain(t)) return rc;
     switch (option) {
     case RG_OPT_REQUIRE_FENCED_TIMEOUTS:
         if (t->require_fence != (value != 0)) t->config_gen += 1;
@@ -194,6 +236,7 @@
 {
     if (!t) return 0;
     (void)hipSetDevice(t->device);
+    (void)flush_chain(t);
     if (t->stream) (void)hipStreamSynchronize(t->stream);
     for (struct rg_tick *k : t->ticks) tick_release(k);
     for (struct rg_tick2 *k : t->ticks2) tick2_release(k);
@@ -270,6 +313,8 @@
     if (const char *e = getenv("RG_SPLIT")) t->lanes = atoi(e) != 0 ? 0 : 64;
     if (const char *e = getenv("RG_FAST")) t->fast_paths = atoi(e) != 0;
     if (const char *e = getenv("RG_FORCE_WIDE")) t->force_wide = atoi(e) != 0;
+    if (const char *e = getenv("RG_SUBMIT_CHAIN")) t->chain_mode = strcmp(e, "force") == 0 ? 2 : (strcmp(e, "0") == 0 ? 0 : 1);
+    if (const char *e = getenv("RG_SUBMIT_CHAIN_MAX")) { const int v = atoi(e); t->chain_cap = (uint32_t)(v < 1 ? 1 : (v > rg::CHAIN_CAP ? rg::CHAIN_CAP : v)); }
     t->counter_slots = (G + 63) / 64 + 1;
     CREATE_TRY(hipMalloc((void **)&t->counters, t->counter_slots * RG_NUM_COUNTERS * sizeof(unsigned long long)));
     t->dt.groups = groups;
@@ -683,6 +728,7 @@
     if (!k) return 0;
     if (rg_table *t = k->t) {
         (void)hipSetDevice(t->device);
+        (void)flush_chain(t);
         if (t->stream) (void)hipStreamSynchronize(t->stream);
         t->ticks.erase(std::remove(t->ticks.begin(), t->ticks.end(), k), t->ticks.end());
         tick_release(k);
@@ -793,6 +839,7 @@
     if (!k || !k->t) return -1;
     rg_table *t = k->t;
     HIP_TRY(t, hipSetDevice(t->device));
+    if (int rc = flush_chain(t)) return rc;
     HIP_TRY(t, hipStreamSynchronize(t->stream));
     k->in_flight = false;
     return 0;
@@ -822,6 +869,7 @@
     if (!k) return 0;
     if (rg_table *t = k->t) {
         (void)hipSetDevice(t->device);
+        (void)flush_chain(t);
         if (t->stream) (void)hipStreamSynchronize(t->stream);
         t->ticks2.erase(std::remove(t->ticks2.begin(), t->ticks2.end(), k), t->ticks2.end());
         tick2_release(k);
@@ -987,6 +1035,7 @@
     if (!k || !k->t) return -1;
     rg_table *t = k->t;
     HIP_TRY(t, hipSetDevice(t->device));
+    if (int rc = flush_chain(t)) return rc;
     HIP_TRY(t, hipStreamSynchronize(t->stream));
     k->in_flight = false;
     return 0;
@@ -1014,6 +1063,7 @@
     if (!a) return 0;
     if (rg_table *t = a->t) {
         (void)hipSetDevice(t->device);
+        (void)flush_chain(t);
         if (t->stream) (void)hipStreamSynchronize(t->stream);
         t->assemblers.erase(std::remove(t->assemblers.begin(), t->assemblers.end(), a), t->assemblers.end());
         assembler_release(a);
@@ -1280,6 +1330,7 @@
     if ((uint64_t)first + count > t->G) return fail(t, -1, "rg_index_base_set: groups [%u, %u) of %u", first, first + count, t->G);
     for (uint32_t i = 0; i < count; i++)
         if (base[i] < 0) return fail(t, -1, "rg_index_base_set: base[%u] = %lld is negative", i, (long long)base[i]);
+    if (int rc = flush_chain(t)) return rc;
     for (uint32_t i = 0; i < count; i++)
         if (base[i] != 0 && !t->has_bases) { t->has_bases = 1; t->config_gen += 1; }
     if (count == 0) return 0;
@@ -1369,6 +1420,17 @@
     const rg_outcome_t shape{&dummy_r, &dummy_l, &dummy_p};
     if (int rc = check_batch(t, &wide, &shape, memspace == RG_MEM_HOST, list_rounds)) return rc;
     if (in->count == 0) return 0;
+    const bool chainable = memspace == RG_MEM_DEVICE && !sparse && wides == 0 && in->entry_count == 0 && t->F <= 6 && t->auto_window == 0 && !t->timing &&
+                           t->chain_mode != 0 && t->chain_cap > 1 && in->rounds < (1u << 16) && in->count < (1u << 28);
+    if (chainable) {
+        if (bind(t, true, false)) return -2;
+        if (t->chain.nseg == 0) t->chain.p = step_params(t, &wide);
+        rg::ChainSeg &sg = t->chain.seg[t->chain.nseg++];
+        sg.head = in->head; sg.abcd32 = (const rg::I32x4 *)in->abcd; sg.out32 = (rg::I32x4 *)out->row; sg.persist32 = (rg::I32x4 *)out->persist;
+        sg.rounds = in->rounds; sg.pad = 0;
+        if (t->chain.nseg >= t->chain_cap || (t->chain_mode == 1 && !stream_busy(t))) return flush_chain(t);
+        return 0;
+    }
     if (bind(t)) return -2;
     const size_t rows = (size_t)in->rounds * in->count;
     rg::StepParams p = step_params(t, &wide);
@@ -1952,7 +2014,22 @@
     return 0;
 }
 
-void *rg_stream(rg_table_t *t) { return t ? (void *)t->stream : nullptr; }
+void *rg_stream(rg_table_t *t)
+{
+    if (!t) return nullptr;
+    (void)flush_chain(t);
+    t->chain_mode = 0;
+    return (void *)t->stream;
+}
+
+int rg_submit_chain_stats(rg_table_t *t, uint64_t *chained_launches, uint64_t *chained_batches, int reset)
+{
+    if (!t) return -1;
+    if (chained_launches) *chained_launches = t->chained_launches;
+    if (chained_batches) *chained_batches = t->chained_batches;
+    if (reset) { t->chained_launches = 0; t->chained_batches = 0; }
+    return 0;
+}
 
 
 int rg_timing_enable(rg_table_t *t, int on)
diff --git a/rafting_amd/csrc/rg_device.hpp b/rafting_amd/csrc/rg_device.hpp
--- a/rafting_amd/csrc/rg_device.hpp
+++ b/rafting_amd/csrc/rg_device.hpp
@@ -60,6 +60,19 @@
     uint32_t stride;
 };
 
+constexpr int CHAIN_CAP = 16;
+struct ChainSeg {
+    const rg_ev_head_t *head;
+    const I32x4 *abcd32;
+    I32x4 *out32, *persist32;
+    uint32_t rounds, pad;
+};
+struct ChainParams {
+    StepParams p;
+    uint32_t nseg, pad;
+    ChainSeg seg[CHAIN_CAP];
+};
+
 struct ReplicateParams {
     DevTable t;
     uint32_t count;
@@ -123,6 +136,7 @@
 };
 
 hipError_t launch_step(const StepParams &p, int followers, bool sparse, int shape, hipStream_t s);
+hipError_t launch_chain(const ChainParams &c, int followers, hipStream_t s);
 hipError_t launch_copy(const void *src, void *dst, size_t bytes, hipStream_t s);
 hipError_t launch_replicate(const ReplicateParams &p, int followers, hipStream_t s);
 hipError_t launch_health_update(const HealthParams &p, hipStream_t s);
diff --git a/rafting_amd/csrc/rg_kernels.hip b/rafting_amd/csrc/rg_kernels.hip
--- a/rafting_amd/csrc/rg_kernels.hip
+++ b/rafting_amd/csrc/rg_kernels.hip
@@ -770,7 +770,7 @@
 
 #endif
 
-#define RG_FOLLOWER_LAUNCHERS(X) X(StepLaunch) X(TickLaunch) X(TickSparseLaunch) X(TickTailLaunch)
+#define RG_FOLLOWER_LAUNCHERS(X) X(StepLaunch) X(ChainLaunch) X(TickLaunch) X(TickSparseLaunch) X(TickTailLaunch)
 #if defined(RG_TU) && RG_TU == 1
 #define RG_PER_UNIT(L) extern template hipError_t launch_range<L, 7>(const L &, int); extern template hipError_t launch_range<L, 11>(const L &, int);
 #elif defined(RG_TU)
@@ -782,6 +782,21 @@
 #undef RG_PER_UNIT
 #ifdef RG_TU_MAIN
 hipError_t launch_step(const StepParams &p, int followers, bool sparse, int shape, hipStream_t s) { return launch_followers(StepLaunch{p, sparse, shape, s}, followers); }
+hipError_t launch_chain(const ChainParams &c, int followers, hipStream_t s)
+{
+    if (c.nseg < 1u || c.nseg > (uint32_t)CHAIN_CAP || c.p.count >= (1u << 28) || c.p.gid != nullptr) return hipErrorInvalidValue;
+    ChainParams k = c;
+    uint64_t total = 0;
+    for (uint32_t i = 0; i < k.nseg; i++) {
+        if (k.seg[i].rounds == 0u || !k.seg[i].head || !k.seg[i].abcd32 || !k.seg[i].out32 || !k.seg[i].persist32) return hipErrorInvalidValue;
+        total += k.seg[i].rounds;
+    }
+    if (total > 0xFFFFFFFFull) return hipErrorInvalidValue;
+    k.p.rounds = (uint32_t)total; k.p.stride = k.p.count;
+    k.p.head = k.seg[0].head; k.p.abcd32 = k.seg[0].abcd32; k.p.out32 = k.seg[0].out32; k.p.persist32 = k.seg[0].persist32;
+    k.p.reply = nullptr; k.p.logfx = nullptr; k.p.persist = nullptr;
+    return launch_followers(ChainLaunch{k, s}, followers);
+}
 hipError_t launch_replicate(const ReplicateParams &p, int followers, hipStream_t s) { return launch_followers(ReplicateLaunch{p, s}, followers); }
 hipError_t launch_tick(const StepParams &p, const TickTailParams &tp, int followers, hipStream_t s) { return launch_followers(TickLaunch{p, tp, s}, followers); }
 hipError_t launch_tick_sparse(const StepParams &p, const TickTailParams &tp, const uint32_t *rows_now, int followers, hipStream_t s)
diff --git a/rafting_amd/csrc/rg_step.hpp b/rafting_amd/csrc/rg_step.hpp
--- a/rafting_amd/csrc/rg_step.hpp
+++ b/rafting_amd/csrc/rg_step.hpp
@@ -167,6 +167,17 @@
 {
     return en.same | (((en.t64 != nullptr) | (en.t32 != nullptr)) & ((uint64_t)aux + n <= p.entry_count));
 }
+
+struct SegWalk {
+    uint32_t seg, lo, hi;
+    __device__ __forceinline__ void start(const ChainParams *c) { seg = 0u; lo = 0u; hi = c->seg[0].rounds; }
+    __device__ __forceinline__ bool move_to(const ChainParams *c, uint32_t r)
+    {
+        bool moved = false;
+        while (r >= hi && seg + 1u < c->nseg) { seg += 1u; lo = hi; hi += c->seg[seg].rounds; moved = true; }
+        return moved;
+    }
+};
 
 __device__ __forceinline__ void load_group(const DevTable &t, uint32_t gi, Group &g)
 {
@@ -429,10 +440,11 @@
     static constexpr size_t BYTES = EV32 ? (W_END > N_END ? W_END : N_END) : W_END;
 };
 
-template <int F, bool SPARSE, bool EV32, bool OUT32 = false>
-__device__ __forceinline__ void split_body(const StepParams &p, unsigned char *smem)
+template <int F, bool SPARSE, bool EV32, bool OUT32 = false, bool CHAIN = false>
+__device__ __forceinline__ void split_body(const StepParams &p, unsigned char *smem, const ChainParams *chain = nullptr)
 {
     static_assert(EV32 || !OUT32, "compact outcome rows belong to the compact-row kernels");
+    static_assert(!CHAIN || (!SPARSE && EV32 && OUT32), "chains: dense compact batches with compact outcome rows");
     typedef SplitLds<F, EV32> L;
     int64_t *sh_epoch = reinterpret_cast<int64_t *>(smem + L::W_EPOCH), *sh_next = reinterpret_cast<int64_t *>(smem + L::W_NEXT),
             *sh_match = reinterpret_cast<int64_t *>(smem + L::W_MATCH);
@@ -469,10 +481,34 @@
                 sh_ev[slot][EV_E2][lane] = (uint64_t)t.e2; sh_ev[slot][EV_E3][lane] = (uint64_t)t.e3;
             }
         };
+        SegWalk fw, rw;
+        struct { const rg_ev_head_t *head; const I32x4 *q; I32x4 *out, *per; } cols;
+        if constexpr (CHAIN) {
+            fw.start(chain); rw.start(chain);
+            cols.head = chain->seg[0].head; cols.q = chain->seg[0].abcd32; cols.out = chain->seg[0].out32; cols.per = chain->seg[0].persist32;
+        }
+        auto fetch = [&](uint32_t r, EventRow &e) {
+            if constexpr (CHAIN) {
+                const uint32_t rr = r < p.rounds ? r : last_round;
+                if (fw.move_to(chain, rr)) { cols.head = chain->seg[fw.seg].head; cols.q = chain->seg[fw.seg].abcd32; }
+                const size_t row = (size_t)(rr - fw.lo) * round_rows + ir;
+                const rg_ev_head_t h = nt_load8(cols.head + row);
+                const I32x4 q = nt_load16(cols.q + row);
+                e.hdr = h.hdr; e.aux = h.aux; e.a = q.x; e.b = q.y; e.c = q.z; e.d = q.w;
+            } else {
+                load_event<EV32>(p, row_of(r), e);
+            }
+        };
         Tally tally;
         auto retire = [&](uint32_t r, uint32_t hdr) {
             const uint32_t slot = r & 1u;
-            const size_t row = (size_t)r * round_rows + ir;
+            size_t row;
+            if constexpr (CHAIN) {
+                if (rw.move_to(chain, r)) { cols.out = chain->seg[rw.seg].out32; cols.per = chain->seg[rw.seg].persist32; }
+                row = (size_t)(r - rw.lo) * round_rows + ir;
+            } else {
+                row = (size_t)r * round_rows + ir;
+            }
             const uint64_t fe = sh_out[slot][OUT_FLAGS][lane];
             const uint32_t flags_all = (uint32_t)fe, flags = flags_all & 0xFFFFu, status = RG_F_STATUS(flags_all);
             rg_reply_t rep;
@@ -488,8 +524,13 @@
                 const uint64_t bits = (uint64_t)rep.resp_term | (uint64_t)commit_r | (w_lfx ? (uint64_t)from_r : 0ull) | (w_per ? (uint64_t)per.term : 0ull);
                 const bool wide = bits >= (1ull << 31);
                 if (active) {
+                    if constexpr (CHAIN) {
+                        nt_store16(cols.out + row, I32x4{(int32_t)rep.resp_term, (int32_t)(flags_all | (wide ? RG_F_WIDE_VALUES : 0u)), (int32_t)commit_r, (int32_t)from_r});
+                        if (w_per) nt_store16(cols.per + row, I32x4{(int32_t)per.term, per.voted_for, (int32_t)rep.role_epoch, per.role});
+                    } else {
                     nt_store16(p.out32 + row, I32x4{(int32_t)rep.resp_term, (int32_t)(flags_all | (wide ? RG_F_WIDE_VALUES : 0u)), (int32_t)commit_r, (int32_t)from_r});
                     if (w_per) nt_store16(p.persist32 + row, I32x4{(int32_t)per.term, per.voted_for, (int32_t)rep.role_epoch, per.role});
+                    }
                     if (wide & (p.reply != nullptr)) {
                         nt_store16(p.reply + row, rep);
                         if (w_lfx) nt_store16(p.logfx + row, lfx);
@@ -510,11 +551,15 @@
         {
             EventRow first{};
             EventTail first_t{};
+            if constexpr (CHAIN) {
+                fetch(0, first); fetch(1, n1); fetch(2, n2); fetch(3, n3); fetch(4, n4);
+            } else {
             load_event<EV32>(p, row_of(0), first);
             load_event<EV32>(p, row_of(1), n1);
             load_event<EV32>(p, row_of(2), n2);
             load_event<EV32>(p, row_of(3), n3);
             load_event<EV32>(p, row_of(4), n4);
+            }
             load_event_tail<EV32>(p, row_of(0), first, first_t);
             load_event_tail<EV32>(p, row_of(1), n1, t1);
             load_event_tail<EV32>(p, row_of(2), n2, t2);
@@ -530,7 +575,8 @@
             n2 = n3;
             n3 = n4;
             load_event_tail<EV32>(p, row_of(r + 3u), n2, t2);
-            load_event<EV32>(p, row_of(r + 5u), n4);
+            if constexpr (CHAIN) fetch(r + 5u, n4);
+            else load_event<EV32>(p, row_of(r + 5u), n4);
             lds_barrier();
         }
         retire(last_round, hdr_prev);
@@ -553,7 +599,12 @@
     sh_flush[1] = (active & (p.auto_window != 0)) ? (int64_t)reinterpret_cast<uint64_t>(p.t.ibase + gi) : 0;
     sh_flush[2] = p.auto_window;
     lds_barrier();
+    SegWalk dw;
+    if constexpr (CHAIN) dw.start(chain);
     for (uint32_t r = 0; r < p.rounds; r++) {
+        if constexpr (CHAIN) {
+            if (dw.move_to(chain, r)) blocked = false;
+        }
         const uint32_t slot = r & 1u;
         const uint64_t head = sh_ev[slot][EV_HEAD][lane];
         const uint32_t hdr = (uint32_t)head, aux = (uint32_t)(head >> 32);
@@ -651,10 +702,11 @@
     return ((int32_t)w < 0) ? (w & 0x00FFFFFFu) : fast;
 }
 
-template <int F, bool SPARSE, bool OUT32, int IOW = 1, int RPB = 1>
-__device__ __forceinline__ bool narrow_body(const StepParams &p, unsigned char *smem)
+template <int F, bool SPARSE, bool OUT32, int IOW = 1, int RPB = 1, bool CHAIN = false>
+__device__ __forceinline__ bool narrow_body(const StepParams &p, unsigned char *smem, const ChainParams *chain = nullptr)
 {
     static_assert(RPB == 1 || (RPB == 2 && IOW == 1), "two rounds per hand-over: the two-wavefront workgroup only");
+    static_assert(!CHAIN || (!SPARSE && OUT32 && IOW == 1 && RPB == 1), "chains: dense batches with compact outcome rows, the two-wavefront workgroup, a hand-over per round");
     constexpr int NO = 2 * RPB;
     typedef SplitLds<F, true, NO> L;
     I32x4 *sh_rec = reinterpret_cast<I32x4 *>(smem + L::N_REC);
@@ -688,8 +740,15 @@
         const uint32_t irm = ir & 0x0FFFFFFFu;
         int64_t io_base = 0;
         if constexpr (!OUT32) io_base = (p.has_bases != 0) ? p.t.ibase[SPARSE ? p.gid[ir] : ir] : 0;
+        SegWalk fw, rw;
+        if constexpr (CHAIN) { fw.start(chain); rw.start(chain); }
         auto fetch = [&](uint32_t r, Row32 &x) {
-            const uint64_t rb = (uint64_t)(r < p.rounds ? r : last_round) * round_rows;
+            uint32_t rr = r < p.rounds ? r : last_round;
+            if constexpr (CHAIN) {
+                if (fw.move_to(chain, rr)) { b_head = reinterpret_cast<uint64_t>(chain->seg[fw.seg].head); b_q = reinterpret_cast<uint64_t>(chain->seg[fw.seg].abcd32); }
+                rr -= fw.lo;
+            }
+            const uint64_t rb = (uint64_t)rr * round_rows;
             x.h = nt_load_at<U32x2>(b_head + rb * 8u, irm);
             x.q = nt_load_at<I32x4>(b_q + rb * 16u, irm);
         };
@@ -710,7 +769,12 @@
         Tally tally;
         auto retire = [&](uint32_t r, uint32_t hdr) {
             const uint32_t slot = r & (uint32_t)(NO - 1);
-            const uint64_t rb16 = (uint64_t)r * round_rows * 16u;
+            uint32_t rr = r;
+            if constexpr (CHAIN) {
+                if (rw.move_to(chain, rr)) { b_reply = reinterpret_cast<uint64_t>(chain->seg[rw.seg].out32); b_persist = reinterpret_cast<uint64_t>(chain->seg[rw.seg].persist32); }
+                rr -= rw.lo;
+            }
+            const uint64_t rb16 = (uint64_t)rr * round_rows * 16u;
             const I32x4 o0 = sh_o0[slot][lane], o1 = sh_o1[slot][lane];
             const uint32_t flags_all = expand_by_table(sh_lutm, sh_lute, (uint32_t)o0.y) | ((uint32_t)o1.w << RG_F_ROLE_SHIFT), flags = flags_all & 0xFFFFu, status = RG_F_STATUS(flags_all);
             if constexpr (OUT32) {
@@ -922,7 +986,18 @@
             RG_PROBE_MARK(3);
         }
     };
-    if constexpr (RPB == 2) {
+    if constexpr (CHAIN) {
+        uint32_t r = 0;
+        for (uint32_t s = 0; s < chain->nseg; s++) {
+            if (s != 0u) { blocked = false; g.nallow = FAST ? 0 : -1; g.recache(); }
+            const uint32_t hi = r + chain->seg[s].rounds;
+            for (; r < hi; r++) {
+                round(r);
+                if (bailed) break;
+            }
+            if (bailed) break;
+        }
+    } else if constexpr (RPB == 2) {
         for (uint32_t r = 0; r < p.rounds; r++) {
             round(r);
             if (bailed) break;
@@ -986,6 +1061,19 @@
     }
     lds_barrier();
     split_body<F, SPARSE, true, OUT32>(p, smem);
+}
+
+template <int F, int WAVES>
+__global__ __launch_bounds__(2 * BLOCK) __attribute__((amdgpu_waves_per_eu(WAVES, 8))) void chain32_kernel(const ChainParams c)
+{
+    __shared__ alignas(16) unsigned char smem[SplitLds<F, true, 2>::BYTES];
+    if (narrow_body<F, false, true, 1, 1, true>(c.p, smem, &c)) return;
+    if (threadIdx.x == 0) {
+        for (uint32_t s = 0; s < c.nseg; s++) RG_NOTE_FALLBACK();
+        atomicAdd(c.p.wide_bodies, (unsigned long long)c.nseg);
+    }
+    lds_barrier();
+    split_body<F, false, true, true, true>(c.p, smem, &c);
 }
 
 template <int F, bool SPARSE, int WAVES, bool OUT32>
@@ -1069,6 +1157,26 @@
     }
     return hipGetLastError();
 }
+
+struct ChainLaunch {
+    const ChainParams &c;
+    hipStream_t s;
+    template <int F> hipError_t run() const
+    {
+        if constexpr (F <= 6) {
+            const ChainParams &c = this->c;
+            const hipStream_t s = this->s;
+            const uint32_t blocks = (c.p.count + BLOCK - 1) / BLOCK;
+            if (blocks == 0) return hipSuccess;
+            const dim3 grid(blocks), wg(2 * BLOCK);
+            if (blocks > MANY_BLOCKS) hipLaunchKernelGGL((chain32_kernel<F, WAVES_MANY<F>>), grid, wg, 0, s, c);
+            else                      hipLaunchKernelGGL((chain32_kernel<F, 1>), grid, wg, 0, s, c);
+            return hipGetLastError();
+        } else {
+            return hipErrorInvalidValue;
+        }
+    }
+};
 
 struct StepLaunch {
     const StepParams &p;
diff --git a/rafting_amd/engine.py b/rafting_amd/engine.py
--- a/rafting_amd/engine.py
+++ b/rafting_amd/engine.py
@@ -27,7 +27,7 @@
         "rg_dev_free", "rg_copy_to_device", "rg_copy_to_host", "rg_stream", "rg_replicate", "rg_timers_configure", "rg_timers_update",
         "rg_timers_expired", "rg_timers_expired_epochs", "rg_timers_arm", "rg_timers_read", "rg_health_update", "rg_health_failure", "rg_ready", "rg_health_read", "rg_in_flight_read", "rg_in_flight_set",
         "rg_timing_enable",
-        "rg_timing_read", "rg_timing_begin", "rg_timing_end", "rg_counters_read", "rg_wide_body_workgroups", "rg_copy_bandwidth",
+        "rg_timing_read", "rg_timing_begin", "rg_timing_end", "rg_counters_read", "rg_wide_body_workgroups", "rg_submit_chain_stats", "rg_copy_bandwidth",
     ]
 
 
@@ -152,6 +152,7 @@
         L.rg_timing_end.argtypes = [vp, C.POINTER(C.c_double)]
         L.rg_counters_read.argtypes = [vp, C.POINTER(C.c_uint64), i32]
         L.rg_wide_body_workgroups.argtypes = [vp, C.POINTER(C.c_uint64), i32]
+        L.rg_submit_chain_stats.argtypes = [vp, C.POINTER(C.c_uint64), C.POINTER(C.c_uint64), i32]
         L.rg_copy_bandwidth.argtypes = [vp, C.c_size_t, i32, C.POINTER(C.c_double)]
         if L.rg_abi_version() != abi.ABI_VERSION:
             raise EngineError("libraftgpu.so ABI %d != binding ABI %d" % (L.rg_abi_version(), abi.ABI_VERSION))
@@ -936,6 +937,11 @@
         self._check(lib().rg_wide_body_workgroups(self._h, C.byref(n), int(reset)))
         return n.value
 
+    def submit_chain_stats(self, reset=False):
+        n, b = C.c_uint64(), C.c_uint64()
+        self._check(lib().rg_submit_chain_stats(self._h, C.byref(n), C.byref(b), int(reset)))
+        return n.value, b.value
+
     def copy_bandwidth(self, nbytes=1 << 30, iters=10):
         g = C.c_double()
         self._check(lib().rg_copy_bandwidth(self._h, nbytes, iters, C.byref(g)))
```

Result: slower. 61.67 billion (-3.3%).
